# iosefa/obia

Hardware: AMD Instinct MI355X
Metric: Mpixel/s (SLIC+zonal feats) on 16384²×8-band; achieved HBM GB/s fraction (higher is better)
Workload: dtype f32

## Files before the change

### obia_amd/_lib.py

```python
import ctypes
import os
import subprocess

import numpy as np

_CSRC = os.path.join(os.path.dirname(os.path.abspath(__file__)), "csrc")
LIB_PATH = os.environ.get("OBIA_HIP_LIB") or os.path.join(_CSRC, "libobia_hip.so")

OBIA_OK = 0
MASK_SEEDS_CHUNK = 1024
E_INVALID, E_HIP, E_NOMEM, E_UNSUPPORTED, E_EMPTY, E_NONFINITE = -1, -2, -3, -4, -5, -6


class SlicParams(ctypes.Structure):
    _fields_ = [("compactness", ctypes.c_double), ("min_size_factor", ctypes.c_double),
                ("max_size_factor", ctypes.c_double), ("n_segments", ctypes.c_int32),
                ("max_num_iter", ctypes.c_int32), ("convert2lab", ctypes.c_int32),
                ("enforce_connectivity", ctypes.c_int32), ("slic_zero", ctypes.c_int32),
                ("start_label", ctypes.c_int32), ("normalize_bands", ctypes.c_int32),
                ("exit_on_fixed_point", ctypes.c_int32), ("reserved", ctypes.c_int32),
                ("sigma_zyx", ctypes.c_double * 3), ("spacing_zyx", ctypes.c_double * 3)]


class SlicSeeds(ctypes.Structure):
# ... 43 lines not shown
    "obia_slic_f32_dev": (_I, [_P, _P, _I, _I, _I, _P, ctypes.POINTER(SlicParams), _P, ctypes.POINTER(_I)]),
    "obia_slic_assign_only_f32_dev": (_I, [_P, _P, _I, _I, _I, _P, ctypes.POINTER(SlicParams), _P, ctypes.POINTER(_I)]),
    "obia_slic_seeded_f32_dev": (_I, [_P, _P, _I, _I, _I, _P, ctypes.POINTER(SlicParams), ctypes.POINTER(SlicSeeds), _I, _P,
                                      ctypes.POINTER(_I)]),
    "obia_mask_centroids_dev": (_I, [_P, _P, _I, _I, _P, ctypes.c_int32, _P, ctypes.c_int64, _I, _P, _P]),
    "obia_slic_stages_f32_dev": (_I, [_P, _P, _I, _I, _I, _P, ctypes.POINTER(SlicParams), ctypes.POINTER(SlicSeeds),
                                      ctypes.POINTER(SlicStages)]),
    "obia_enforce_connectivity_i32_dev": (_I, [_P, _P, _I, _I, _I, _I, _I, _P, ctypes.POINTER(_I)]),
    "obia_zonal_stats_f32": (_I, [_P, _P, _P, _I, _I, _I, _P, _I, _I, _I, _P, _P, _P, _P, _P]),
    "obia_zonal_stats_f32_dev": (_I, [_P, _P, _P, _I, _I, _I, _P, _I, _I, _I, _P, _P, _P, _P, _P]),
    "obia_zonal_moments_f32_dev": (_I, [_P, _P, _P, _I, _I, _I, _P, _I, _I, _I, _P, _P, _P, _P]),
    "obia_zonal_moments_f32": (_I, [_P, _P, _P, _I, _I, _I, _P, _I, _I, _I, _P, _P, _P]),
    "obia_texture_stats_f32_dev": (_I, [_P, _P, _P, _I, _I, _I, _P, _I, _I, _I, _P]),
    "obia_label_edges_u8_dev": (_I, [_P, _P, _I, _I, _P, _P]),
    "obia_sample_labels_i32_dev": (_I, [_P, _P, _I, _I, _P, _P, ctypes.c_int64, _I, _P]),
    "obia_cost_bands_f32_dev": (_I, [_P, _P, ctypes.c_int64, _P, _P]),
    "obia_cost_ndvi_f32_dev": (_I, [_P, _P, _P, ctypes.c_int64, _P]),
    "obia_cost_sobel_f32_dev": (_I, [_P, _P, _I, _I, _P]),
    "obia_cost_select_dev": (_I, [_P, _P, _I, ctypes.c_int64, ctypes.c_double, ctypes.c_double, _P, _P]),
    "obia_cost_entropy_f32_dev": (_I, [_P, _P, _I, _I, ctypes.c_double, ctypes.c_double, _P, _P]),
    "obia_cost_normalise_dev": (_I, [_P, _P, _I, ctypes.c_int64, ctypes.c_double, ctypes.c_double, _P]),
    "obia_cost_edge_count_dev": (_I, [_P, _P, _I, _I, _P]),
    "obia_cost_combine_dev": (_I, [_P, _P, _P, _P, _P, _I, _I, _P, _P, _P, _P]),
    "obia_seeds_peaks_dev": (_I, [_P, _P, _I, _I, ctypes.c_double, _I, ctypes.c_float, _P, _P, _P, _P]),
    "obia_seeds_peaks_gather_dev": (_I, [_P, _P, _P, _P, _P, _I, _I, ctypes.c_int64, _P, _P, _P, _P]),
    "obia_seeds_pair_link_dev": (_I, [_P, _P, _P, _I, _P, _I, _I, _P, ctypes.c_double, ctypes.c_double, _I, _P, ctypes.c_double, _I, _P,
                                      ctypes.POINTER(_I)]),
    "obia_seeds_pair_stats_dev": (_I, [_P, _P, _P, _I, _P, _I, _I, _P, ctypes.c_double, ctypes.c_double, _I, _P, _P, _P]),
    "obia_seeds_pair_matrix_dev": (_I, [_P, _P, _P, _I, _P, _I, _I, _P, ctypes.c_double, ctypes.c_double, _I, _P, _P]),
    "obia_polygon_count_i32_dev": (_I, [_P, _P, _I, _I, _I, _P, _P]),
    "obia_polygon_rings_i32_dev": (_I, [_P, _P, _I, _I, _I, ctypes.c_int64, ctypes.c_int64, _P, _P, _P, _P, _P, _P]),
    "obia_rasterize_polygons_dev": (_I, [_P, _P, _P, ctypes.c_int64, _P, _P, ctypes.c_int64, _I, _I, ctypes.c_int32, _P]),
    "obia_rasterize_info": (_I, [ctypes.POINTER(ctypes.c_int64)]),
    "obia_quickshift_f32": (_I, [_P, _P, _I, _I, _I, ctypes.c_double, ctypes.c_double, ctypes.c_double, ctypes.c_double, _I, _P, _I, _P, ctypes.POINTER(_I)]),
    "obia_quickshift_f32_dev": (_I, [_P, _P, _I, _I, _I, ctypes.c_double, ctypes.c_double, ctypes.c_double, ctypes.c_double, _I, _P, _I, _P, ctypes.POINTER(_I)]),
    "obia_quickshift_stages_f32_dev": (_I, [_P, _P, _I, _I, _I, ctypes.c_double, ctypes.c_double, ctypes.c_double, ctypes.c_double, _I, _P, _I, _P,
                                            ctypes.POINTER(_I), _P, _P, _P, _P, _P, _P]),
    "obia_tiled_slic_f32_dev": (_I, [_P, _P, _P, _I, _I, _I, ctypes.POINTER(TilingParams), ctypes.POINTER(SlicParams), _P,
                                     ctypes.POINTER(ctypes.c_int64)]),
    "obia_tiled_slic_f32": (_I, [_P, _P, _P, _I, _I, _I, ctypes.POINTER(TilingParams), ctypes.POINTER(SlicParams), _P,
                                 ctypes.POINTER(ctypes.c_int64)]),
    "obia_tiled_slic_seeded_f32_dev": (_I, [_P, _P, _P, _I, _I, _I, ctypes.POINTER(TilingParams), ctypes.POINTER(SlicParams), _I, PickFn, _P,
                                            _P, ctypes.POINTER(ctypes.c_int64)]),
    "obia_tiled_slic_seeded_f32": (_I, [_P, _P, _P, _I, _I, _I, ctypes.POINTER(TilingParams), ctypes.POINTER(SlicParams), _I, PickFn, _P,
                                        _P, ctypes.POINTER(ctypes.c_int64)]),
    "obia_tiler_set_seeding": (_I, [_P, _I, PickFn, _P]),
    "obia_tiler_create": (_P, [_P, _P, _P, _I, _I, _I, _I, _I, ctypes.POINTER(TilingParams), ctypes.POINTER(SlicParams), _P, _I]),
    "obia_tiler_destroy": (None, [_P]),
    "obia_tiler_run": (_I, [_P, _I, _I, _I, _I]),
    "obia_tiler_next_id": (_I, [_P]),
    "obia_tiler_set_segments": (_I, [_P, _I, _I, _P]),
    "obia_tiler_get_alive": (_I, [_P, _P, _I]),
    "obia_tiler_set_alive": (_I, [_P, _P, _I]),
    "obia_tiler_finalize": (_I, [_P, ctypes.POINTER(ctypes.c_int64)]),
    "obia_tiler_import_seam": (_I, [_P, _P, _I, _I, _I, _P, _I, _P, _P, ctypes.POINTER(ctypes.c_int), ctypes.POINTER(ctypes.c_int),
                                    ctypes.POINTER(ctypes.c_int)]),
    "obia_table_scale_dev": (_I, [_P, _P, ctypes.c_int64, _I, _P, _P, _P]),
    "obia_forest_predict_dev": (_I, [_P, _P, ctypes.c_int64, _I, ctypes.POINTER(Forest), _P, _P, _P, _P]),
    "obia_mlp_predict_dev": (_I, [_P, _P, ctypes.c_int64, _I, ctypes.POINTER(Mlp), _P, _P, _P, _P, _P]),
    "obia_table_scale_f64_dev": (_I, [_P, _P, ctypes.c_int64, _I, _P, _P, _P]),
    "obia_forest_shap_dev": (_I, [_P, _P, ctypes.c_int64, _I, ctypes.POINTER(Forest), _P, _P, _P]),
    "obia_mlp_coalition_dev": (_I, [_P, _P, ctypes.c_int64, _I, ctypes.POINTER(Mlp), _P, ctypes.c_int64, _P, ctypes.c_int64, _P]),
    "obia_shapley_combine_dev": (_I, [_P, _P, ctypes.c_int64, _I, _I, _P, _P]),
    "obia_set_profiling": (_I, [_P, _I]),
    "obia_last_timing": (ctypes.c_double, [_P, _I]),
}
EXPORTED_SYMBOLS = tuple(_SIGNATURES)
_IMAGE_SIGNATURES = {
    "obia_image_stretch_u8_dev": (_I, [_P, _P, _I, ctypes.c_int64, ctypes.c_double, ctypes.c_double, _P]),
    "obia_image_gray_hist_dev": (_I, [_P, _P, _I, ctypes.c_int64, _P, _P]),
    "obia_image_lut_u8_dev": (_I, [_P, _P, ctypes.c_int64, _P, _I, _P]),
    "obia_image_clahe_u8_dev": (_I, [_P, _P, _I, _I, _I, _I, _P]),
    "obia_image_boundaries_dev": (_I, [_P, _P, _I, _I, _P]),
    "obia_image_mark_u8_dev": (_I, [_P, _P, _I, _P, _I, _I, _P, _P, _P]),
}
SHARP_MAX_WIN = 65536
_SHARPNESS_SIGNATURES = {
    "obia_sharp_gray_lap_dev": (_I, [_P, _P, _I, _I, _I, ctypes.POINTER(ctypes.c_int32), _P, _P]),
    "obia_sharp_laplacian_dev": (_I, [_P, _P, _I, _I, _P, _P]),
    "obia_sharp_box_dev": (_I, [_P, _P, _I, _I, _I, _P, _P, _P]),
    "obia_sharp_variance_dev": (_I, [_P, _P, _I, _I, _I, _P, _P]),
    "obia_sharp_stretch_f32_dev": (_I, [_P, _P, ctypes.c_int64, ctypes.c_double, ctypes.c_double, _P]),
}

_lib = None


def build(force=False):
    args = ["make", "-C", _CSRC, "-j8"]
    if force:
        args.append("-B")
    subprocess.check_call(args, stdout=subprocess.DEVNULL)
    return LIB_PATH


def load():
    global _lib
    if _lib is None:
        if not os.path.exists(LIB_PATH):
            raise ImportError(f"{LIB_PATH} not found: build it with `python -c 'import __graft_entry__ as g; g.build()'` "
                              "(hipcc, gfx950). obia_amd has no CPU fallback.")
        lib = ctypes.CDLL(LIB_PATH)
        for name, (res, args) in list(_SIGNATURES.items()) + list(_IMAGE_SIGNATURES.items()) + list(_SHARPNESS_SIGNATURES.items()):
            try:
                fn = getattr(lib, name)
            except AttributeError:
                if os.environ.get("OBIA_HIP_LIB"):
                    continue
                raise
            fn.restype = res
            fn.argtypes = args
        _lib = lib
    return _lib


def last_error():
    return load().obia_last_error().decode("utf-8", "replace")


def check(rc):
    if rc == OBIA_OK:
        return
    msg = last_error()
    if rc in (E_INVALID, E_EMPTY, E_NONFINITE):
        raise ValueError(msg)
    if rc == E_UNSUPPORTED:
        raise NotImplementedError(msg)
    if rc == E_NOMEM:
        raise MemoryError(msg)
    raise RuntimeError(f"obia_hip error {rc}: {msg}")


class Context:

    def __init__(self, device=0, stream=None):
        lib = load()
        if stream is None:
            self._h = lib.obia_create(int(device))
        else:
            self._h = lib.obia_create_on_stream(int(device), ctypes.c_void_p(int(stream)))
        if not self._h:
            raise RuntimeError(f"obia_create failed: {last_error()} (obia_amd needs an AMD GPU; there is no CPU path)")
        self.device = int(device)

    @property
    def handle(self):
        return self._h

    def close(self):
        if getattr(self, "_h", None):
            load().obia_destroy(self._h)
            self._h = None

    def __del__(self):
        try:
            self.close()
        except Exception:
            pass

    def set_profiling(self, on):
        check(load().obia_set_profiling(self._h, int(on)))

    def timing(self):
        lib = load()
        names = ["assign_ms", "sweeps", "features_ms", "connectivity_ms", "zonal_ms", "total_ms", "prepass_ms", "assign_px",
                 "prepass_px", "assign_store_px", "assign_busy_ms", "prepass_busy_ms", "batch_repeats",
                 "prepass_shared_px", "feature_fused_px", "prepass_group_launches"]
        return {n: lib.obia_last_timing(self._h, i) for i, n in enumerate(names)}

    def workspace_bytes(self):
        return int(load().obia_workspace_bytes(self._h))


_default_ctx = {}


def default_context(device=0):
    ctx = _default_ctx.get(device)
    if ctx is None:
        ctx = _default_ctx[device] = Context(device)
    return ctx


def np_ptr(a):
    return None if a is None else ctypes.c_void_p(a.ctypes.data)


def mask_bytes(mask, device=None):
    import torch
    m = torch.as_tensor(mask, device=device)
    if m.dtype == torch.bool:
        m = m.contiguous().view(torch.uint8)
    elif m.dtype != torch.uint8:
        m = (m != 0).view(torch.uint8)
    return m.contiguous()
```

### obia_amd/csrc/api.cpp

```cpp
#include "slic.hpp"

#include <cmath>

using namespace obia;

namespace {

int check_slic_args(const float *img, int H, int W, int C, const obia_slic_params *p) {
    if (!img || !p) { set_error("null image or params"); return OBIA_E_INVALID; }
    if (H <= 0 || W <= 0 || C <= 0) { set_error("bad image shape (%d,%d,%d)", H, W, C); return OBIA_E_INVALID; }
    if ((long long)H * W > 0x7fffffffLL) { set_error("rasters above 2^31 pixels must go through the tiled driver"); return OBIA_E_INVALID; }
    if (C > 16) { set_error("more than 16 bands not supported (got %d)", C); return OBIA_E_UNSUPPORTED; }
    if (p->start_label != 0 && p->start_label != 1) { set_error("start_label should be 0 or 1."); return OBIA_E_INVALID; }
    if (p->convert2lab == 1 && C != 3) { set_error("Lab colorspace conversion requires a RGB image."); return OBIA_E_INVALID; }
    if (!(p->compactness > 0.0)) { set_error("compactness must be positive"); return OBIA_E_INVALID; }
    if (p->n_segments <= 0) { set_error("n_segments must be positive"); return OBIA_E_INVALID; }
    if (p->max_num_iter < 0) { set_error("max_num_iter must be >= 0"); return OBIA_E_INVALID; }
    for (int i = 0; i < 3; ++i) {
        if (!(p->sigma_zyx[i] >= 0.0)) { set_error("sigma must be >= 0"); return OBIA_E_INVALID; }
        if (!(p->spacing_zyx[i] > 0.0) || !(p->spacing_zyx[i] < 1.0e30)) { set_error("spacing must be positive and finite"); return OBIA_E_INVALID; }
    }
    return OBIA_OK;
}

int slic_single(obia_ctx *ctx, const float *img, int H, int W, int C, const uint8_t *mask,
                const obia_slic_params *p, SlicBatch &b, const ExternalSeeds *ext = nullptr, bool prepass_only = false,
                int prepass_iters = 0) {
    Arena &A = ctx->arena;
    slic_batch_settings(b, *p, C, p->normalize_bands, mask != nullptr);
    b.prepass_only = prepass_only && b.masked;
    b.prepass_iter = b.masked ? prepass_iters : 0;
    b.windows.assign(1, SrcWindow{0, 0, H, W, 0, 0, 0});
    OBIA_TRY(slic_batch_layout(b));
    b.d_windows = A.get<SrcWindow>(1);
    b.d_feat = A.get<float>(4 * (size_t)b.total_feat_f4);
    b.d_labels = A.get<int32_t>((size_t)b.total_pix);
    if (!b.d_windows || !b.d_feat || !b.d_labels) return OBIA_E_NOMEM;
    OBIA_HIP_TRY(hipMemcpyAsync(b.d_windows, b.windows.data(), sizeof(SrcWindow), hipMemcpyHostToDevice, ctx->stream));
    b.d_mask = const_cast<uint8_t *>(mask);
    if (b.col_lb) {
        b.d_fbox = A.get<float>((size_t)b.total_boxes * 2 * b.CP);
        if (!b.d_fbox) return OBIA_E_NOMEM;
    }
    OBIA_TRY(slic_prepare_features(ctx, b, img, W));
    std::vector<int> nseg(1, p->n_segments);
    OBIA_TRY(slic_plan_and_seed(ctx, b, nseg, nullptr, ext));
    if (b.probs[0].K <= 0) {
        set_error("mask is empty: nothing to segment");
        return OBIA_E_EMPTY;
    }
    const Arena::Mark sweeps_mk = A.mark();
    OBIA_TRY(slic_run_sweeps(ctx, b));
    OBIA_HIP_TRY(hipStreamSynchronize(ctx->stream));
    bool repeat = false;
    OBIA_TRY(slic_sweeps_settle(ctx, &repeat));
    if (repeat) {
        A.rewind(sweeps_mk);
        b.d_mask4 = nullptr;
        OBIA_TRY(slic_rerun_storing(ctx, b));
    }
    return OBIA_OK;
}

}

extern "C" {

static int check_seeds(const obia_slic_seeds *seeds, int H, int W, ExternalSeeds &ext) {
    if (!seeds) { set_error("null seeds"); return OBIA_E_INVALID; }
    if (!seeds->yx || seeds->n < 1) { set_error("seeds: need at least one (y, x) pair"); return OBIA_E_INVALID; }
    for (int i = 0; i < seeds->n; ++i) {
        const double y = seeds->yx[2 * (size_t)i], x = seeds->yx[2 * (size_t)i + 1];
        if (!(y >= 0.0 && y <= (double)(H - 1) && x >= 0.0 && x <= (double)(W - 1))) {
            set_error("seed %d = (%g, %g) lies outside the (%d, %d) raster", i, y, x, H, W);
            return OBIA_E_INVALID;
        }
    }
    double st = seeds->steps_zyx[0];
    if (seeds->steps_zyx[1] > st) st = seeds->steps_zyx[1];
    if (seeds->steps_zyx[2] > st) st = seeds->steps_zyx[2];
    if (!(st > 0.0) || !(st < 1e9)) { set_error("seeds: steps must be positive and finite"); return OBIA_E_INVALID; }
    ext.yx = seeds->yx; ext.n = seeds->n; ext.step = st;
    return OBIA_OK;
}

static int slic_stages_impl(obia_ctx *ctx, const float *img, int H, int W, int C, const uint8_t *mask,
                            const obia_slic_params *params, const ExternalSeeds *ext, obia_slic_stages *st) {
    OBIA_TRY(check_slic_args(img, H, W, C, params));
    if (!st) { set_error("null output"); return OBIA_E_INVALID; }
    if (st->prepass_iters < 0) { set_error("prepass_iters must be >= 0"); return OBIA_E_INVALID; }
    if (st->centroids && params->max_num_iter < 1) { set_error("centroids: no sweep ran (max_num_iter = 0)"); return OBIA_E_INVALID; }
    SlicBatch b;
    OBIA_TRY(call_frame(ctx, FRAME_TOTAL, [&] {
        int rc = slic_single(ctx, img, H, W, C, mask, params, b, ext, st->prepass_only != 0, st->prepass_iters);
        if (rc == OBIA_OK && (st->seeds_yx || st->centroids) && b.probs[0].K > st->centroid_capacity) {
            set_error("%d centroids, room for %d", b.probs[0].K, st->centroid_capacity);
            rc = OBIA_E_INVALID;
        }
        if (rc == OBIA_OK && st->labels_pre) {
            hipError_t e = hipMemcpyAsync(st->labels_pre, b.d_labels, sizeof(int32_t) * (size_t)H * W, hipMemcpyDeviceToDevice, ctx->stream);
            if (e != hipSuccess) { set_error("copy failed: %s", hipGetErrorString(e)); rc = OBIA_E_HIP; }
        }
        if (rc == OBIA_OK && (st->features || st->seeds_yx || st->centroids))
            rc = slic_stage_outputs(ctx, b, st->features, st->seeds_yx, st->centroids);
        return rc;
    }));
    st->K = b.probs[0].K;
    st->step = (double)b.step[0];
    st->prescale = (double)b.prescale;
    st->fscale = b.fscale * (double)b.prescale;
    return OBIA_OK;
}

static int slic_assign_only_impl(obia_ctx *ctx, const float *img, int H, int W, int C, const uint8_t *mask,
                                 const obia_slic_params *params, const ExternalSeeds *ext, int32_t *labels_pre_out,
                                 int *n_centroids_out) {
    if (!labels_pre_out) { set_error("null output"); return OBIA_E_INVALID; }
    obia_slic_stages st{};
    st.labels_pre = labels_pre_out;
    OBIA_TRY(slic_stages_impl(ctx, img, H, W, C, mask, params, ext, &st));
    if (n_centroids_out) *n_centroids_out = st.K;
    return OBIA_OK;
}

static int slic_full_impl(obia_ctx *ctx, const float *img, int H, int W, int C, const uint8_t *mask,
                          const obia_slic_params *params, const ExternalSeeds *ext, int32_t *labels_out, int *n_labels_out) {
    OBIA_TRY(check_slic_args(img, H, W, C, params));
    if (!labels_out) { set_error("null output"); return OBIA_E_INVALID; }
    SlicBatch b;
    int n_labels = 0;
    OBIA_TRY(call_frame(ctx, FRAME_TOTAL, [&]() -> int {
        OBIA_TRY(slic_single(ctx, img, H, W, C, mask, params, b, ext));
        if (params->enforce_connectivity) {
            const auto [min_size, max_size] = slic_cc_sizes(params->min_size_factor, params->max_size_factor, b.probs[0].n_valid, b.probs[0].K);
            return enforce_connectivity_dev(ctx, b.d_labels, H, W, min_size, max_size, params->start_label, labels_out, &n_labels);
        }
        hipError_t e = hipMemcpyAsync(labels_out, b.d_labels, sizeof(int32_t) * (size_t)H * W, hipMemcpyDeviceToDevice, ctx->stream);
        if (e != hipSuccess) { set_error("copy failed: %s", hipGetErrorString(e)); return OBIA_E_HIP; }
        n_labels = b.probs[0].K;
        return OBIA_OK;
    }));
    if (n_labels_out) *n_labels_out = n_labels;
// ... 160 lines not shown
```

### obia_amd/csrc/cc.hip

```cpp
#include "slic.hpp"

#include <cstdlib>

namespace obia {

__device__ __forceinline__ int find_prob(const CcProblem *__restrict__ probs, int nprob, long long g) {
    int lo = 0, hi = nprob - 1;
    while (lo < hi) {
        const int mid = (lo + hi + 1) >> 1;
        if (probs[mid].pix_off <= g) lo = mid; else hi = mid - 1;
    }
    return lo;
}

__device__ __forceinline__ int ld_agent(const int *p) {
    return __hip_atomic_load(p, __ATOMIC_RELAXED, __HIP_MEMORY_SCOPE_AGENT);
}

__device__ __forceinline__ int find_root(const int *parent, int i) {
    int p;
    while ((p = ld_agent(&parent[i])) != i) i = p;
    return i;
}

// ... 642 lines not shown
        n = ccur[s];
        if (o + n > cap) n = cap - o;
    }
    if (n > 0 && n <= SETTLE_COOP) {
        int m = T_NEVER;
        for (int e = 0; e < n; ++e) m = min(m, settle_entry_min(px_cn[o + e], settle));
        int t = T_NEVER;
        if (m != T_NEVER)
            for (int e = 0; e < n; ++e) { const int g = px_g[o + e]; if (g > m && g < t) t = g; }
        if (settle[s] != t) {
            settle[s] = t;
            for (int e = 0; e < n; ++e) push_neighbours(px_cn[o + e]);
        }
    }
    unsigned long long coop = __ballot(n > SETTLE_COOP);
    while (coop) {
        const int src = __builtin_ctzll(coop);
        coop &= coop - 1;
        const int sb = __shfl(s, src), ob = __shfl(o, src), nb = __shfl(n, src);
        int m = T_NEVER;
        for (int e = lane; e < nb; e += 64) m = min(m, settle_entry_min(px_cn[ob + e], settle));
        m = wave_min_i32(m);
        int t = T_NEVER;
        if (m != T_NEVER)
            for (int e = lane; e < nb; e += 64) { const int g = px_g[ob + e]; if (g > m && g < t) t = g; }
        t = wave_min_i32(t);
        const int old = settle[sb];
        if (old != t) {
            if (lane == 0) settle[sb] = t;
            for (int e = lane; e < nb; e += 64) push_neighbours(px_cn[ob + e]);
        }
    }
    int inc = npush;
#pragma unroll
    for (int off = 1; off < 64; off <<= 1) { const int v = __shfl_up(inc, off); if ((int)threadIdx.x >= off) inc += v; }
    const int total = __shfl(inc, 63);
    if (total == 0) return;
    int base_slot = 0;
    if (threadIdx.x == 63) base_slot = atomicAdd(work_cnt, total);
    base_slot = __shfl(base_slot, 63);
    for (int j = 0; j < npush; ++j) work_out[base_slot + inc - npush + j] = s_push[threadIdx.x][j];
}
__global__ __launch_bounds__(64) void cc_small_target_kernel(const CcProblem *__restrict__ probs, int nprob, const int *__restrict__ code,
                                                             const int *__restrict__ newlab, const int *__restrict__ small_list,
                                                             const int *__restrict__ small_qoff, const int *__restrict__ settle,
                                                             int *__restrict__ queue, int32_t *__restrict__ out, int *__restrict__ target, int n_small) {
    const int s = blockIdx.x * blockDim.x + threadIdx.x;
    if (s >= n_small) return;
    const int st = settle[s];
    if (st == T_NEVER) { target[s] = -1; return; }
    const CcProblem P = probs[find_prob(probs, nprob, small_list[s])];
    int *q = queue + small_qoff[s];
    int csize = 0, ms = 0;
    const int adjacent = replay_bfs<true>(code, newlab, settle, -(s + 2), st, P.H, P.W, (int)P.pix_off, q, out, &csize, &ms, nullptr);
    for (int i = 0; i < csize; ++i) out[q[i]] = 0;
    target[s] = adjacent;
}

__global__ void cc_settle_init_kernel(const int *__restrict__ small_list, int n_small, int *__restrict__ settle, int from_above) {
    const int s = blockIdx.x * blockDim.x + threadIdx.x;
    if (s < n_small) settle[s] = from_above ? 0x7fffffff : small_list[s];
}

__global__ void cc_small_final_kernel(const int *__restrict__ parent, const int *__restrict__ newlab, const int *__restrict__ target,
                                      int n_small, int max_hops, int *__restrict__ small_final) {
    const int s = blockIdx.x * blockDim.x + threadIdx.x;
    if (s >= n_small) return;
    int nl = -(s + 2), hops = 0;
    while (nl < 0) {
        const int t = target[-nl - 2];
        if (t < 0 || ++hops > max_hops) { nl = -1; break; }
        nl = newlab[parent[parent[t]]];
    }
    small_final[s] = nl;
}

__global__ __launch_bounds__(256) void cc_relabel_kernel(const CcResolve R, long long n, int32_t *__restrict__ out) {
    for (long long i = (long long)blockIdx.x * blockDim.x + threadIdx.x; i < n; i += (long long)gridDim.x * blockDim.x)
        out[i] = cc_resolve_label(R, i);
}

int enforce_connectivity_batch(obia_ctx *ctx, const std::vector<CcProblem> &probs, const int32_t *labels_in,
                               long long total_pix, int start_label, int32_t *labels_out, int *h_n_labels_out,
                               CcResolve *deferred) {
    ScopedSpan span(ctx, T_CC);
    Arena &A = ctx->arena;
    const long long n = total_pix;
    const int np = (int)probs.size();
    if (np <= 0 || n <= 0 || n > 0x7fffffffLL) { set_error("label batch of %lld pixels not supported", n); return OBIA_E_INVALID; }
    const int mask_label = start_label - 1;
    CcProblem *d_probs = A.get<CcProblem>(np);
    int *parent = A.get<int>(n), *size = A.get<int>(n), *newlab = A.get<int>(n);
    const int nb = cdiv(n, SCAN_CHUNK);
    int *block_sums = A.get<int>(3 * (size_t)nb);
    unsigned long long *rootbits = A.get<unsigned long long>((size_t)((n + 63) / 64));
    if (!rootbits) return OBIA_E_NOMEM;
    unsigned long long *lrbits_block = A.get<unsigned long long>((size_t)((n + 63) / 64) + 4);
    if (!lrbits_block) return OBIA_E_NOMEM;
    unsigned long long *lrbits = lrbits_block + 4;
    const unsigned long long *rb = rootbits;
    int *counters = reinterpret_cast<int *>(lrbits_block);
    if (!d_probs || !parent || !size || !newlab || !block_sums) return OBIA_E_NOMEM;
    OBIA_TRY(upload_async(ctx, d_probs, probs.data(), sizeof(CcProblem) * np));
    OBIA_HIP_TRY(hipMemsetAsync(lrbits_block, 0, sizeof(unsigned long long) * ((size_t)((n + 63) / 64) + 4), ctx->stream));
    int gs = cdiv(n, 256 * 4);
    if (gs > 65535 * 4) gs = 65535 * 4;
    {
        int max_tiles = 1;
        long long max_seam = 1;
        for (auto &P : probs) {
            const int t = cdiv(P.W, CT_W) * cdiv(P.H, CT_H);
            if (t > max_tiles) max_tiles = t;
            const long long sm = (long long)((P.H - 1) / CT_H) * P.W + (long long)((P.W - 1) / CT_W) * P.H;
            if (sm > max_seam) max_seam = sm;
        }
        hipLaunchKernelGGL(cc_tile_kernel, dim3(max_tiles, np), dim3(256), 0, ctx->stream, d_probs, labels_in, parent, size, mask_label, lrbits);
        int sg = cdiv(max_seam, 256);
        if (sg > 65535) sg = 65535;
        hipLaunchKernelGGL(cc_seam_kernel, dim3(sg, np), dim3(256), 0, ctx->stream, d_probs, labels_in, parent, mask_label);
    }
    debug_sync(ctx, "cc: tile + seam");
    hipLaunchKernelGGL(cc_roots_kernel, dim3(cdiv((n + 63) / 64, 64)), dim3(64), 0, ctx->stream, parent, size, n, lrbits, rootbits);
    debug_sync(ctx, "cc: roots");
    hipLaunchKernelGGL(cc_rank_blocksum_bits_kernel, dim3(nb), dim3(64), 0, ctx->stream, d_probs, np, size, n, block_sums, counters, rootbits);
    hipLaunchKernelGGL(cc_rank_scan_kernel, dim3(3), dim3(1024), 0, ctx->stream, block_sums, nb, counters);
    int hc[8];
    OBIA_TRY(read_back(ctx, hc, counters, sizeof(hc)));
    if (hc[6] > 0) {
        const int n_big = hc[6];
        int *big_root = A.get<int>(n_big), *big_qoff = A.get<int>(n_big), *big_box = A.get<int>(4 * (size_t)n_big);
        if (!big_root || !big_qoff || !big_box) return OBIA_E_NOMEM;
        OBIA_HIP_TRY(hipMemsetAsync(counters, 0, sizeof(int) * 8, ctx->stream));
        hipLaunchKernelGGL(cc_flatten_all_kernel, dim3(gs), dim3(256), 0, ctx->stream, parent, n);
        hipLaunchKernelGGL(cc_big_list_kernel, dim3(cdiv(n, 256)), dim3(256), 0, ctx->stream, d_probs, np, parent, size, n, newlab,
                           big_root, big_qoff, big_box, counters);
        int hb[8];
        OBIA_TRY(read_back(ctx, hb, counters, sizeof(hb)));
        int *bqueue = A.get<int>(hb[7] > 0 ? hb[7] : 1);
        if (!bqueue) return OBIA_E_NOMEM;
        hipLaunchKernelGGL(cc_big_mark_kernel, dim3(cdiv(n, 256)), dim3(256), 0, ctx->stream, d_probs, np, parent, size, n, newlab, big_box);
        hipLaunchKernelGGL(cc_split_kernel, dim3(cdiv(n_big, 64)), dim3(64), 0, ctx->stream, d_probs, np, parent, size, big_root, big_qoff,
                           big_box, n_big, bqueue);
        OBIA_HIP_TRY(hipMemsetAsync(counters, 0, sizeof(int) * 8, ctx->stream));
        rb = nullptr;
        hipLaunchKernelGGL(cc_rank_blocksum_kernel, dim3(nb), dim3(SCAN_NT), 0, ctx->stream, d_probs, np, parent, size, n, block_sums, counters, rb);
        hipLaunchKernelGGL(cc_rank_scan_kernel, dim3(3), dim3(1024), 0, ctx->stream, block_sums, nb, counters);
        OBIA_TRY(read_back(ctx, hc, counters, sizeof(hc)));
    }
    const int n_small = hc[0], small_px = hc[1], n_surv = hc[2];
    int *small_list = A.get<int>(n_small > 0 ? n_small : 1);
    int *small_qoff = A.get<int>(n_small > 0 ? n_small : 1);
    int *target = A.get<int>(n_small > 0 ? n_small : 1);
    int *queue = A.get<int>(small_px > 0 ? small_px : 1);
    if (!small_list || !small_qoff || !target || !queue) return OBIA_E_NOMEM;
    debug_sync(ctx, "cc: rank counts");
    if (rb)
        hipLaunchKernelGGL(cc_rank_apply_bits_kernel, dim3(nb), dim3(64), 0, ctx->stream, d_probs, np, size, n, block_sums, newlab,
                           small_list, small_qoff, rb);
    else
        hipLaunchKernelGGL(cc_rank_apply_kernel, dim3(nb), dim3(SCAN_NT), 0, ctx->stream, d_probs, np, parent, size, n, block_sums,
                           newlab, small_list, small_qoff, counters, rb);
    int *settle_arr = nullptr;
    int32_t *visited = nullptr;
    if (n_small > 0) {
        int *settle = settle_arr = A.get<int>(n_small), *work_a = A.get<int>(n_small), *work_b = A.get<int>(n_small), *tag = A.get<int>(n_small);
        static const long long code_div = std::getenv("OBIA_CC_CODE_DIV") ? atoll(std::getenv("OBIA_CC_CODE_DIV")) : 64;
        const bool use_code = (long long)n_small * code_div >= n;
        constexpr int RING = 64;
        int *ring = A.get<int>(RING);
        if (!ring) return OBIA_E_NOMEM;
        OBIA_HIP_TRY(hipMemsetAsync(ring, 0, sizeof(int) * RING, ctx->stream));
        long long ring_pos = 0;
        int *code = use_code ? A.get<int>(n) : parent;
        if (!settle || !work_a || !work_b || !tag || !code) return OBIA_E_NOMEM;
        if ((size_t)n > ctx->cc_visited_px || ctx->cc_visited_dirty) {
            if ((size_t)n > ctx->cc_visited_px) {
                OBIA_HIP_TRY(hipStreamSynchronize(ctx->stream));
                if (ctx->cc_visited) (void)hipFree(ctx->cc_visited);
                ctx->cc_visited = nullptr; ctx->cc_visited_px = 0;
                const size_t want = (size_t)n + (size_t)n / 8;
                if (hipMalloc(&ctx->cc_visited, want * sizeof(int32_t)) != hipSuccess) { (void)hipGetLastError(); set_error("out of device memory (visited map of %zu pixels)", want); return OBIA_E_NOMEM; }
                ctx->cc_visited_px = want;
            }
            OBIA_HIP_TRY(hipMemsetAsync(ctx->cc_visited, 0, sizeof(int32_t) * ctx->cc_visited_px, ctx->stream));
        }
        ctx->cc_visited_dirty = true;
        visited = ctx->cc_visited;
        if (use_code) hipLaunchKernelGGL(cc_code_kernel, dim3(gs), dim3(256), 0, ctx->stream, parent, newlab, n, code);
        constexpr int ROUNDS_FROM_BELOW = 5;
        bool converged = false;
        const bool dense = use_code && start_label == 1 && !std::getenv("OBIA_CC_WORKLIST");
        if (dense) {
            int *px_g = A.get<int>(small_px), *ccur = A.get<int>(n_small);
            int4 *px_cn = A.get<int4>(small_px);
            if (!px_g || !ccur || !px_cn) return OBIA_E_NOMEM;
            int maxh = 1;
            for (auto &P : probs) maxh = std::max(maxh, P.H);
            OBIA_HIP_TRY(hipMemsetAsync(ccur, 0, sizeof(int) * (size_t)n_small, ctx->stream));
            hipLaunchKernelGGL(cc_small_pixels_kernel, dim3(maxh, np), dim3(256), 0, ctx->stream, d_probs, code, small_qoff, ccur, px_g, px_cn, small_px);
            for (int side = (n_small > 8 * (long long)n_surv ? 1 : 0); side < 2 && !converged; ++side) {
                OBIA_HIP_TRY(hipMemsetAsync(tag, 0, sizeof(int) * (size_t)n_small, ctx->stream));
                hipLaunchKernelGGL(cc_settle_init_kernel, dim3(cdiv(n_small, 256)), dim3(256), 0, ctx->stream, small_list, n_small, settle, side);
                int n_items = n_small;
                const int *work_in = nullptr;
                const long long max_rounds = side == 0 ? ROUNDS_FROM_BELOW : (long long)small_px + 2;
                for (long long round = 0; round <= max_rounds; ++round) {
                    if (std::getenv("OBIA_DEBUG_CC")) fprintf(stderr, "[obia cc]   (lists) side %d round %lld: %d items\n", side, round, n_items);
                    int *cnt = ring + (ring_pos++ % RING);
                    if (ring_pos > RING && (ring_pos - 1) % RING == 0) OBIA_HIP_TRY(hipMemsetAsync(ring, 0, sizeof(int) * RING, ctx->stream));
                    hipLaunchKernelGGL(cc_settle_eval_kernel, dim3(cdiv(n_items, 64)), dim3(64), 0, ctx->stream, small_qoff, ccur, px_g, px_cn, small_px,
                                       settle, work_in, n_items, work_a, cnt, tag, (int)(round & 0x3fffffff));
                    int n_next = 0;
                    OBIA_TRY(read_back(ctx, &n_next, cnt, sizeof(int)));
                    if (n_next == 0) { converged = true; break; }
                    work_in = work_a;
                    std::swap(work_a, work_b);
                    n_items = n_next;
                }
            }
            if (converged)
                hipLaunchKernelGGL(cc_small_target_kernel, dim3(cdiv(n_small, 64)), dim3(64), 0, ctx->stream, d_probs, np, code, newlab, small_list,
                                   small_qoff, settle, queue, visited, target, n_small);
        }
        for (int side = (n_small > 8 * (long long)n_surv ? 1 : 0); !dense && side < 2 && !converged; ++side) {
            OBIA_HIP_TRY(hipMemsetAsync(tag, 0, sizeof(int) * (size_t)n_small, ctx->stream));
            hipLaunchKernelGGL(cc_settle_init_kernel, dim3(cdiv(n_small, 256)), dim3(256), 0, ctx->stream, small_list, n_small, settle, side);
            int n_items = n_small;
            const int *work_in = nullptr;
            const long long max_rounds = side == 0 ? ROUNDS_FROM_BELOW : (long long)small_px + 2;
            for (long long round = 0; round <= max_rounds; ++round) {
                if (std::getenv("OBIA_DEBUG_CC")) fprintf(stderr, "[obia cc]   side %d round %lld: %d items\n", side, round, n_items);
                int *cnt = ring + (ring_pos++ % RING);
                if (ring_pos > RING && (ring_pos - 1) % RING == 0) OBIA_HIP_TRY(hipMemsetAsync(ring, 0, sizeof(int) * RING, ctx->stream));
                if (use_code)
                    hipLaunchKernelGGL(HIP_KERNEL_NAME(cc_small_bfs_kernel<true>), dim3(cdiv(n_items, 64)), dim3(64), 0, ctx->stream, d_probs, np, code,
                                       newlab, small_list, small_qoff, start_label, settle, queue, visited, target, work_in, n_items, work_a,
                                       cnt, tag, (int)(round & 0x3fffffff));
                else
                    hipLaunchKernelGGL(HIP_KERNEL_NAME(cc_small_bfs_kernel<false>), dim3(cdiv(n_items, 64)), dim3(64), 0, ctx->stream, d_probs, np, code,
                                       newlab, small_list, small_qoff, start_label, settle, queue, visited, target, work_in, n_items, work_a,
                                       cnt, tag, (int)(round & 0x3fffffff));
                int n_next = 0;
                OBIA_TRY(read_back(ctx, &n_next, cnt, sizeof(int)));
                if (n_next == 0) { converged = true; break; }
                work_in = work_a;
                std::swap(work_a, work_b);
                n_items = n_next;
            }
        }
        if (!converged) { set_error("connectivity enforcement: settle rounds did not converge (%d small components)", n_small); return OBIA_E_INVALID; }
        ctx->cc_visited_dirty = false;
    }
    if (std::getenv("OBIA_DEBUG_CC"))
        fprintf(stderr, "[obia cc] %lld px, %d problems: %d surviving, %d small components (%d px)\n", n, np, n_surv, n_small, small_px);
    debug_sync(ctx, "cc: rank apply + small components");
    if (n_small > 0)
        hipLaunchKernelGGL(cc_small_final_kernel, dim3(cdiv(n_small, 256)), dim3(256), 0, ctx->stream, parent, newlab, target, n_small, n_small + 1, settle_arr);
    const CcResolve R{parent, newlab, settle_arr, start_label, mask_label};
    if (deferred) *deferred = R;
    else hipLaunchKernelGGL(cc_relabel_kernel, dim3(gs), dim3(256), 0, ctx->stream, R, n, labels_out);
    OBIA_HIP_TRY(hipGetLastError());
    if (h_n_labels_out) *h_n_labels_out = n_surv;
    return OBIA_OK;
}

int enforce_connectivity_dev(obia_ctx *ctx, const int32_t *labels_in, int H, int W, int min_size, int max_size,
                             int start_label, int32_t *labels_out, int *h_n_labels_out) {
    std::vector<CcProblem> probs(1, CcProblem{H, W, 0, min_size, max_size > 0 ? max_size : 1});
    return enforce_connectivity_batch(ctx, probs, labels_in, (long long)H * W, start_label, labels_out, h_n_labels_out);
}

}
```

### obia_amd/csrc/common.hpp

```cpp
#pragma once
#include <hip/hip_runtime.h>
#include <algorithm>
#include <cstdint>
#include <cstdio>
#include <cstring>
#include <string>
#include <vector>

#include "../../include/obia_hip.h"

namespace obia {

void set_error(const char *fmt, ...);

#define OBIA_HIP_TRY(expr)                                                                       \
    do {                                                                                         \
        hipError_t e__ = (expr);                                                                 \
        if (e__ != hipSuccess) {                                                                 \
            obia::set_error("%s:%d: %s -> %s", __FILE__, __LINE__, #expr, hipGetErrorString(e__)); \
            return OBIA_E_HIP;                                                                   \
        }                                                                                        \
    } while (0)

#define OBIA_TRY(expr)            \
    do {                          \
        int rc__ = (expr);        \
        if (rc__ != OBIA_OK) return rc__; \
    } while (0)

class Arena {
  public:
    ~Arena() { release(); }
    void *alloc(size_t bytes);
    template <typename T> T *get(size_t n) { return static_cast<T *>(alloc(n * sizeof(T))); }
    void reset();
    void release();
    struct Mark { size_t block, used, total; };
    Mark mark() const;
    void rewind(const Mark &m);
    size_t capacity() const;
    bool failed() const { return failed_; }

  private:
    struct Block { char *p; size_t size; size_t used; };
    std::vector<Block> blocks_;
    size_t high_water_ = 0, cur_total_ = 0, cur_ = 0;
    bool failed_ = false;
};

struct Timing {
    double assign_ms = 0, prepass_ms = 0, feat_ms = 0, cc_ms = 0, zonal_ms = 0, total_ms = 0;
    double assign_px = 0, prepass_px = 0;
    double prepass_shared_px = 0;
    double assign_store_px = 0;
    double feat_fused_px = 0;
    int sweeps = 0;
    int prepass_group_launches = 0;
    int batch_repeats = 0;
    double assign_busy_ms = 0, prepass_busy_ms = 0;
};

}

struct obia_ctx {
    int device = 0;
    hipStream_t stream = nullptr;
    bool own_stream = false;
    obia::Arena arena;
    void *pinned = nullptr;
    size_t pinned_bytes = 0;
    unsigned long long *defer_buf = nullptr;
    bool defer_pending = false;
    double defer_shared_px = 0;
    int32_t *cc_visited = nullptr;
    size_t cc_visited_px = 0;
    bool cc_visited_dirty = false;
    char *up_buf = nullptr;
    size_t up_bytes = 0, up_used = 0;
    int profiling = 0;
    obia::Timing timing;
    struct Span { int kind; hipEvent_t a, b; };
    std::vector<Span> spans;
    std::vector<hipEvent_t> event_pool;
    size_t events_used = 0;
    hipStream_t side = nullptr;
    hipEvent_t aux_fork = nullptr, aux_join = nullptr;
    hipEvent_t grp_fork = nullptr, grp_join = nullptr;
    int spatial_residency[4] = {0, 0, 0, 0};
};

namespace obia {

enum TimeKind { T_ASSIGN = 0, T_FEAT = 2, T_CC = 3, T_ZONAL = 4, T_TOTAL = 5, T_PREPASS = 6 };

struct ScopedSpan {
    obia_ctx *ctx; bool on; size_t idx;
    ScopedSpan(obia_ctx *c, int kind);
    ~ScopedSpan();
};
struct KernelSpan {
    hipEvent_t a = nullptr, b = nullptr;
    KernelSpan(obia_ctx *c, int kind);
};
void begin_timing(obia_ctx *ctx);
void resolve_timing(obia_ctx *ctx);

int read_back(obia_ctx *ctx, void *host_dst, const void *dev_src, size_t bytes);
int upload_async(obia_ctx *ctx, void *dev_dst, const void *host_src, size_t bytes);
int side_stream(obia_ctx *ctx);
void debug_sync(obia_ctx *ctx, const char *stage);

static inline int cdiv(long long a, long long b) { return (int)((a + b - 1) / b); }
static inline unsigned flat_grid(long long n) { return (unsigned)std::max<long long>(1, std::min<long long>(cdiv(n, 256), 8192)); }


int enter(obia_ctx *ctx);

int quiesce(obia_ctx *ctx, int rc);

enum FrameOpts : unsigned { FRAME_PLAIN = 0, FRAME_TIMING = 1, FRAME_TOTAL = 2 | FRAME_TIMING };
void frame_begin(obia_ctx *ctx, unsigned opts);
int frame_end(obia_ctx *ctx, unsigned opts, int rc);
template <typename Body> int call_frame(obia_ctx *ctx, unsigned opts, Body &&body) {
    frame_begin(ctx, opts);
    int rc;
    if ((opts & FRAME_TOTAL) == FRAME_TOTAL) {
        ScopedSpan total(ctx, T_TOTAL);
        rc = body();
    } else {
        rc = body();
    }
    return frame_end(ctx, opts, rc);
}

class Staging {
  public:
    explicit Staging(obia_ctx *ctx) : ctx_(ctx) {}
    ~Staging() { (void)finish(); }
    Staging(const Staging &) = delete;
    Staging &operator=(const Staging &) = delete;
    template <typename T> T *in(const T *host, size_t n) { return static_cast<T *>(upload(host, n * sizeof(T))); }
    template <typename T> T *out(size_t n) { return static_cast<T *>(alloc(n * sizeof(T))); }
    template <typename T> void fetch(T *host, const T *dev, size_t n) { download(host, dev, n * sizeof(T)); }
    bool ok() const { return rc_ == OBIA_OK; }
    template <typename Call> void run(Call &&call) { if (ok()) rc_ = call(); }
    int finish();
  private:
    void *alloc(size_t bytes);
    void *upload(const void *host, size_t bytes);
    void download(void *host, const void *dev, size_t bytes);
    obia_ctx *ctx_;
    int rc_ = OBIA_OK;
    bool open_ = true;
    std::vector<void *> bufs_;
};

#if defined(__HIPCC__)
typedef float obia_v4f __attribute__((ext_vector_type(4)));
__device__ __forceinline__ float4 ld_stream_f4(const void *p) {
    const obia_v4f t = __builtin_nontemporal_load(reinterpret_cast<const obia_v4f *>(p));
    return make_float4(t.x, t.y, t.z, t.w);
}
#endif

}
```

### obia_amd/csrc/context.cpp

```cpp
#include "common.hpp"

#include <algorithm>
#include <cstdlib>
#include <utility>

#include <cstdarg>

namespace obia {

static thread_local std::string g_last_error;

void set_error(const char *fmt, ...) {
    char buf[1024];
    va_list ap;
    va_start(ap, fmt);
    vsnprintf(buf, sizeof(buf), fmt, ap);
    va_end(ap);
    g_last_error = buf;
}

void *Arena::alloc(size_t bytes) {
    bytes = (bytes + 255) & ~size_t(255);
    if (bytes == 0) bytes = 256;
    for (; cur_ < blocks_.size(); ++cur_) {
        Block &b = blocks_[cur_];
        if (b.size - b.used >= bytes) {
            void *p = b.p + b.used;
            b.used += bytes;
            cur_total_ += bytes;
            if (cur_total_ > high_water_) high_water_ = cur_total_;
            return p;
        }
    }
    size_t want = bytes;
    size_t grow = blocks_.empty() ? (size_t(64) << 20) : 2 * blocks_.back().size;
    if (grow > (size_t(4) << 30)) grow = size_t(4) << 30;
    if (want < grow) want = grow;
    void *p = nullptr;
    if (hipMalloc(&p, want) != hipSuccess) {
        if (want == bytes || hipMalloc(&p, bytes) != hipSuccess) {
            failed_ = true;
            set_error("workspace hipMalloc of %zu bytes failed", bytes);
            return nullptr;
        }
        want = bytes;
    }
    blocks_.push_back(Block{static_cast<char *>(p), want, bytes});
    cur_ = blocks_.size() - 1;
    cur_total_ += bytes;
    if (cur_total_ > high_water_) high_water_ = cur_total_;
    return p;
}

Arena::Mark Arena::mark() const {
    Mark m;
    m.block = cur_ < blocks_.size() ? cur_ : blocks_.size();
    m.used = m.block < blocks_.size() ? blocks_[m.block].used : 0;
    m.total = cur_total_;
    return m;
}

void Arena::rewind(const Mark &m) {
    for (size_t i = m.block + 1; i < blocks_.size(); ++i) blocks_[i].used = 0;
    if (m.block < blocks_.size()) blocks_[m.block].used = m.used;
    cur_ = m.block;
    cur_total_ = m.total;
}

void Arena::reset() {
    failed_ = false;
    cur_total_ = 0;
    cur_ = 0;
    if (blocks_.size() > 1) {
        size_t total = 0;
        for (auto &b : blocks_) total += b.size;
        for (auto &b : blocks_) (void)hipFree(b.p);
        blocks_.clear();
        void *p = nullptr;
        if (hipMalloc(&p, high_water_ + (high_water_ >> 3)) == hipSuccess) blocks_.push_back(Block{static_cast<char *>(p), high_water_ + (high_water_ >> 3), 0});
        (void)total;
    } else if (!blocks_.empty()) {
        blocks_[0].used = 0;
    }
// ... 17 lines not shown
        ctx->event_pool.push_back(e);
    }
    return ctx->event_pool[ctx->events_used++];
}

ScopedSpan::ScopedSpan(obia_ctx *c, int kind) : ctx(c), on(c->profiling == 1 || (c->profiling == 2 && kind == T_ASSIGN)), idx(0) {
    if (!on) return;
    obia_ctx::Span s{kind, get_event(ctx), get_event(ctx)};
    (void)hipEventRecord(s.a, ctx->stream);
    idx = ctx->spans.size();
    ctx->spans.push_back(s);
}
ScopedSpan::~ScopedSpan() {
    if (on) (void)hipEventRecord(ctx->spans[idx].b, ctx->stream);
}

int side_stream(obia_ctx *ctx) {
    if (!ctx->aux_fork) OBIA_HIP_TRY(hipEventCreateWithFlags(&ctx->aux_fork, hipEventDisableTiming));
    if (!ctx->aux_join) OBIA_HIP_TRY(hipEventCreateWithFlags(&ctx->aux_join, hipEventDisableTiming));
    if (!ctx->grp_fork) OBIA_HIP_TRY(hipEventCreateWithFlags(&ctx->grp_fork, hipEventDisableTiming));
    if (!ctx->grp_join) OBIA_HIP_TRY(hipEventCreateWithFlags(&ctx->grp_join, hipEventDisableTiming));
    if (!ctx->side) OBIA_HIP_TRY(hipStreamCreateWithFlags(&ctx->side, hipStreamNonBlocking));
    return OBIA_OK;
}

KernelSpan::KernelSpan(obia_ctx *c, int kind) {
    if (!(c->profiling == 1 || (c->profiling == 2 && kind == T_ASSIGN))) return;
    a = get_event(c);
    b = get_event(c);
    c->spans.push_back(obia_ctx::Span{kind, a, b});
}

void begin_timing(obia_ctx *ctx) {
    ctx->spans.clear();
    ctx->events_used = 0;
    ctx->timing = Timing();
}

void resolve_timing(obia_ctx *ctx) {
    if (!ctx->profiling) return;
    (void)hipStreamSynchronize(ctx->stream);
    std::vector<std::pair<double, double>> iv[2];
    hipEvent_t ref = nullptr;
    for (auto &s : ctx->spans) {
        float ms = 0;
        if (hipEventElapsedTime(&ms, s.a, s.b) != hipSuccess) { (void)hipGetLastError(); continue; }
        if (s.kind == T_ASSIGN || s.kind == T_PREPASS) {
            if (!ref) ref = s.a;
            float end = 0;
            if (hipEventElapsedTime(&end, ref, s.b) == hipSuccess) iv[s.kind == T_ASSIGN ? 0 : 1].emplace_back((double)end - ms, (double)end);
            else (void)hipGetLastError();
        }
        switch (s.kind) {
            case T_ASSIGN: ctx->timing.assign_ms += ms; ctx->timing.sweeps += 1; break;
            case T_FEAT: ctx->timing.feat_ms += ms; break;
            case T_CC: ctx->timing.cc_ms += ms; break;
            case T_ZONAL: ctx->timing.zonal_ms += ms; break;
            case T_TOTAL: ctx->timing.total_ms += ms; break;
            case T_PREPASS: ctx->timing.prepass_ms += ms; break;
            default: break;
        }
    }
    for (int c = 0; c < 2; ++c) {
        std::sort(iv[c].begin(), iv[c].end());
        double busy = 0, lo = 0, hi = -1;
        for (auto &x : iv[c]) {
            if (hi < lo || x.first > hi) { if (hi > lo) busy += hi - lo; lo = x.first; hi = x.second; }
            else if (x.second > hi) hi = x.second;
        }
        if (hi > lo) busy += hi - lo;
        (c == 0 ? ctx->timing.assign_busy_ms : ctx->timing.prepass_busy_ms) += busy;
    }
    ctx->spans.clear();
}

int read_back(obia_ctx *ctx, void *host_dst, const void *dev_src, size_t bytes) {
    if (bytes > ctx->pinned_bytes) {
        if (ctx->pinned) (void)hipHostFree(ctx->pinned);
        ctx->pinned = nullptr;
        size_t want = bytes < 4096 ? 4096 : bytes;
        OBIA_HIP_TRY(hipHostMalloc(&ctx->pinned, want, hipHostMallocDefault));
        ctx->pinned_bytes = want;
    }
    OBIA_HIP_TRY(hipMemcpyAsync(ctx->pinned, dev_src, bytes, hipMemcpyDeviceToHost, ctx->stream));
    OBIA_HIP_TRY(hipStreamSynchronize(ctx->stream));
    ctx->up_used = 0;
    memcpy(host_dst, ctx->pinned, bytes);
    return OBIA_OK;
}

void debug_sync(obia_ctx *ctx, const char *stage) {
    static const bool on = std::getenv("OBIA_DEBUG_SYNC") != nullptr;
    if (!on) return;
    const hipError_t e = hipStreamSynchronize(ctx->stream);
    fprintf(stderr, "[obia debug] %s: %s\n", stage, e == hipSuccess ? "ok" : hipGetErrorString(e));
    fflush(stderr);
}

int upload_async(obia_ctx *ctx, void *dev_dst, const void *host_src, size_t bytes) {
    if (bytes == 0) return OBIA_OK;
    constexpr size_t RING = 8u << 20;
    if (!ctx->up_buf) {
        void *p = nullptr;
        OBIA_HIP_TRY(hipHostMalloc(&p, RING, hipHostMallocDefault));
        ctx->up_buf = static_cast<char *>(p);
        ctx->up_bytes = RING;
        ctx->up_used = 0;
    }
    if (bytes > ctx->up_bytes) {
        OBIA_HIP_TRY(hipMemcpyAsync(dev_dst, host_src, bytes, hipMemcpyHostToDevice, ctx->stream));
        OBIA_HIP_TRY(hipStreamSynchronize(ctx->stream));
        ctx->up_used = 0;
        return OBIA_OK;
    }
    if (ctx->up_used + bytes > ctx->up_bytes) {
        OBIA_HIP_TRY(hipStreamSynchronize(ctx->stream));
        ctx->up_used = 0;
    }
    char *slot = ctx->up_buf + ctx->up_used;
    memcpy(slot, host_src, bytes);
    OBIA_HIP_TRY(hipMemcpyAsync(dev_dst, slot, bytes, hipMemcpyHostToDevice, ctx->stream));
    ctx->up_used += (bytes + 63) & ~(size_t)63;
    return OBIA_OK;
}

int enter(obia_ctx *ctx) {
    if (!ctx) { set_error("null context"); return OBIA_E_INVALID; }
    if (hipSetDevice(ctx->device) != hipSuccess) { set_error("hipSetDevice(%d) failed", ctx->device); return OBIA_E_HIP; }
    return OBIA_OK;
}

int quiesce(obia_ctx *ctx, int rc) {
    (void)hipStreamSynchronize(ctx->stream);
    if (ctx->side) (void)hipStreamSynchronize(ctx->side);
    return rc;
}

void frame_begin(obia_ctx *ctx, unsigned opts) {
    ctx->arena.reset();
    if (opts & FRAME_TIMING) begin_timing(ctx);
}

int frame_end(obia_ctx *ctx, unsigned opts, int rc) {
    if (rc != OBIA_OK) return quiesce(ctx, rc);
    OBIA_HIP_TRY(hipStreamSynchronize(ctx->stream));
    if (opts & FRAME_TIMING) resolve_timing(ctx);
    return OBIA_OK;
}

void *Staging::alloc(size_t bytes) {
    if (!ok()) return nullptr;
    void *p = nullptr;
    if (hipMalloc(&p, bytes) != hipSuccess) {
        set_error("device allocation for host-pointer call failed");
        rc_ = OBIA_E_NOMEM;
        return nullptr;
    }
    bufs_.push_back(p);
    return p;
}

void *Staging::upload(const void *host, size_t bytes) {
    if (!host) return nullptr;
    void *p = alloc(bytes);
    if (p && hipMemcpyAsync(p, host, bytes, hipMemcpyHostToDevice, ctx_->stream) != hipSuccess) {
        set_error("host->device copy failed in a host-pointer call");
        rc_ = OBIA_E_HIP;
    }
    return p;
}

void Staging::download(void *host, const void *dev, size_t bytes) {
    if (ok() && hipMemcpyAsync(host, dev, bytes, hipMemcpyDeviceToHost, ctx_->stream) != hipSuccess) {
        set_error("device->host copy failed in a host-pointer call");
        rc_ = OBIA_E_HIP;
    }
}

int Staging::finish() {
    if (open_) {
        open_ = false;
        (void)hipStreamSynchronize(ctx_->stream);
        for (void *p : bufs_) (void)hipFree(p);
        bufs_.clear();
    }
    return rc_;
}

}

using namespace obia;

extern "C" {

int obia_abi_version(void) { return OBIA_ABI_VERSION; }

const char *obia_last_error(void) { return g_last_error.c_str(); }

static obia_ctx *create_impl(int device_id, void *stream, bool own) {
    int n = 0;
    if (hipGetDeviceCount(&n) != hipSuccess || n <= 0) {
        set_error("no HIP device available");
        return nullptr;
    }
    if (device_id < 0 || device_id >= n) {
        set_error("device_id %d out of range (%d devices)", device_id, n);
        return nullptr;
    }
    if (hipSetDevice(device_id) != hipSuccess) {
        set_error("hipSetDevice(%d) failed", device_id);
        return nullptr;
    }
    obia_ctx *ctx = new obia_ctx();
    ctx->device = device_id;
    if (own) {
        if (hipStreamCreateWithFlags(&ctx->stream, hipStreamNonBlocking) != hipSuccess) {
            set_error("hipStreamCreate failed");
            delete ctx;
            return nullptr;
        }
        ctx->own_stream = true;
    } else {
        ctx->stream = static_cast<hipStream_t>(stream);
    }
    return ctx;
}

obia_ctx *obia_create(int device_id) { return create_impl(device_id, nullptr, true); }
obia_ctx *obia_create_on_stream(int device_id, void *hip_stream) { return create_impl(device_id, hip_stream, false); }

void obia_destroy(obia_ctx *ctx) {
    if (!ctx) return;
    (void)hipSetDevice(ctx->device);
    (void)hipStreamSynchronize(ctx->stream);
    ctx->arena.release();
    if (ctx->up_buf) (void)hipHostFree(ctx->up_buf);
    if (ctx->pinned) (void)hipHostFree(ctx->pinned);
    if (ctx->defer_buf) (void)hipHostFree(ctx->defer_buf);
    if (ctx->cc_visited) (void)hipFree(ctx->cc_visited);
    for (auto e : ctx->event_pool) (void)hipEventDestroy(e);
    if (ctx->side) (void)hipStreamDestroy(ctx->side);
    if (ctx->aux_fork) (void)hipEventDestroy(ctx->aux_fork);
    if (ctx->aux_join) (void)hipEventDestroy(ctx->aux_join);
    if (ctx->grp_fork) (void)hipEventDestroy(ctx->grp_fork);
    if (ctx->grp_join) (void)hipEventDestroy(ctx->grp_join);
    if (ctx->own_stream) (void)hipStreamDestroy(ctx->stream);
    delete ctx;
}

int obia_synchronize(obia_ctx *ctx) {
    if (!ctx) { set_error("null context"); return OBIA_E_INVALID; }
    OBIA_HIP_TRY(hipStreamSynchronize(ctx->stream));
    return OBIA_OK;
}

int64_t obia_workspace_bytes(obia_ctx *ctx) { return ctx ? (int64_t)ctx->arena.capacity() : 0; }

void obia_slic_default_params(obia_slic_params *p) {
    if (!p) return;
    p->n_segments = 100;
    p->compactness = 10.0;
    p->max_num_iter = 10;
    p->convert2lab = -1;
    p->enforce_connectivity = 1;
    p->min_size_factor = 0.5;
    p->max_size_factor = 3.0;
    p->slic_zero = 0;
    p->start_label = 1;
    p->normalize_bands = 0;
    p->exit_on_fixed_point = 0;
    p->reserved = 0;
    p->sigma_zyx[0] = p->sigma_zyx[1] = p->sigma_zyx[2] = 0.0;
    p->spacing_zyx[0] = p->spacing_zyx[1] = p->spacing_zyx[2] = 1.0;
}

int obia_set_profiling(obia_ctx *ctx, int enabled) {
    if (!ctx) { set_error("null context"); return OBIA_E_INVALID; }
    ctx->profiling = enabled < 0 ? 0 : (enabled > 2 ? 1 : enabled);
    return OBIA_OK;
}

double obia_last_timing(obia_ctx *ctx, int what) {
    if (!ctx) return -1.0;
    switch (what) {
        case 0: return ctx->timing.assign_ms;
        case 1: return (double)ctx->timing.sweeps;
        case 2: return ctx->timing.feat_ms;
        case 3: return ctx->timing.cc_ms;
        case 4: return ctx->timing.zonal_ms;
        case 5: return ctx->timing.total_ms;
        case 6: return ctx->timing.prepass_ms;
        case 7: return ctx->timing.assign_px;
        case 8: return ctx->timing.prepass_px;
        case 9: return ctx->timing.assign_store_px;
        case 10: return ctx->timing.assign_busy_ms;
        case 11: return ctx->timing.prepass_busy_ms;
        case 12: return (double)ctx->timing.batch_repeats;
        case 13: return ctx->timing.prepass_shared_px;
        case 14: return ctx->timing.feat_fused_px;
        case 15: return (double)ctx->timing.prepass_group_launches;
        default: return -1.0;
    }
}

}
```

### obia_amd/csrc/slic.hip

```cpp
#include "slic.hpp"
#include "slic_features.hpp"

#include <cmath>
#include <cstdlib>

namespace obia {

void regular_grid_hw(long long H, long long W, long long n, long long out[4]) {
    long long dims[3] = {1, H, W};
    int order[3] = {0, 1, 2};
    for (int i = 0; i < 3; ++i)
        for (int j = i + 1; j < 3; ++j)
            if (dims[order[j]] < dims[order[i]]) std::swap(order[i], order[j]);
    double sd[3];
    for (int i = 0; i < 3; ++i) sd[i] = (double)dims[order[i]];
    double space = sd[0] * sd[1] * sd[2];
    if (space <= (double)n) { out[0] = out[1] = out[2] = out[3] = 0; return; }
    double st[3];
    for (int i = 0; i < 3; ++i) st[i] = std::pow(space / (double)n, 1.0 / 3.0);
    auto all_ge = [&]() { return sd[0] >= st[0] && sd[1] >= st[1] && sd[2] >= st[2]; };
    if (!all_ge()) {
        for (int d = 0; d < 3; ++d) {
            st[d] = sd[d];
            double sp = 1.0;
// ... 612 lines not shown
            bal[u] = __ballot(keep[u]);
            if (lane == 0) s_wave[it & 1][u][wv] = __popcll(bal[u]);
        }
        __syncthreads();
        int run = base;
#pragma unroll
        for (int u = 0; u < U; ++u) {
            int before = 0, total = 0;
#pragma unroll
            for (int w = 0; w < 4; ++w) { const int c = s_wave[it & 1][u][w]; total += c; if (w < wv) before += c; }
            if (keep[u]) {
                const int rank = run + before + __popcll(bal[u] & ((1ull << lane) - 1ull));
                seed[2 * (size_t)(g.cent_off + rank)] = (float)y[u];
                seed[2 * (size_t)(g.cent_off + rank) + 1] = (float)x[u];
                cent_prob[g.cent_off + rank] = p;
            }
            run += total;
        }
        base = run;
    }
    __syncthreads();
    int K = base;
    if (K == 0 && g.slots > 0) {
        const long long npix = (long long)P.H * P.W;
        unsigned long long best = ~0ull;
        for (long long i = tid; i < npix; i += 256)
            if (mask[P.pix_off + i]) { best = (unsigned long long)i; break; }
        atomicMin(&s_first, best);
        __syncthreads();
        if (tid == 0 && s_first != ~0ull) {
            seed[2 * (size_t)g.cent_off] = (float)(s_first / P.W);
            seed[2 * (size_t)g.cent_off + 1] = (float)(s_first % P.W);
            cent_prob[g.cent_off] = p;
        }
        K = (s_first != ~0ull) ? 1 : 0;
    }
    if (tid == 0) K_out[p] = K;
}

__global__ __launch_bounds__(256) void count_valid_kernel(const SlicProblem *__restrict__ probs,
                                                          const uint8_t *__restrict__ mask, int *__restrict__ out) {
    const int p = blockIdx.y;
    const SlicProblem P = probs[p];
    const long long npix = (long long)P.H * P.W;
    const uint8_t *m = mask + P.pix_off;
    int c = 0;
    const long long head = ((16 - (reinterpret_cast<uintptr_t>(m) & 15)) & 15);
    const long long h0 = head < npix ? head : npix;
    const long long nvec = (npix - h0) / 16;
    const uint4 *mv = reinterpret_cast<const uint4 *>(m + h0);
    auto popnz = [](const uint4 &t) {
        int n = 0;
        const unsigned wds[4] = {t.x, t.y, t.z, t.w};
#pragma unroll
        for (int q = 0; q < 4; ++q) {
            unsigned nz = wds[q] | (wds[q] >> 4);
            nz |= nz >> 2; nz |= nz >> 1;
            n += __popc(nz & 0x01010101u);
        }
        return n;
    };
    const long long stride = (long long)gridDim.x * blockDim.x;
    long long i = (long long)blockIdx.x * blockDim.x + threadIdx.x;
    for (; i + 3 * stride < nvec; i += 4 * stride) {
        const uint4 t0 = mv[i], t1 = mv[i + stride], t2 = mv[i + 2 * stride], t3 = mv[i + 3 * stride];
        c += popnz(t0) + popnz(t1) + popnz(t2) + popnz(t3);
    }
    for (; i < nvec; i += stride) c += popnz(mv[i]);
    if (blockIdx.x == 0) {
        for (long long j = threadIdx.x; j < h0; j += blockDim.x) c += m[j] != 0;
        for (long long j = h0 + nvec * 16 + threadIdx.x; j < npix; j += blockDim.x) c += m[j] != 0;
    }
    __shared__ int s_c[4];
#pragma unroll
    for (int off = 32; off > 0; off >>= 1) c += __shfl_xor(c, off);
    if ((threadIdx.x & 63) == 0) s_c[threadIdx.x >> 6] = c;
    __syncthreads();
    if (threadIdx.x == 0) {
        const int tot = s_c[0] + s_c[1] + s_c[2] + s_c[3];
        if (tot) atomicAdd(&out[p], tot);
    }
}

int slic_count_valid(obia_ctx *ctx, SlicBatch &b, std::vector<int> &nvalid) {
    const int np = b.nprob;
    Arena &A = ctx->arena;
    nvalid.assign(np, 0);
    if (!b.d_probs) b.d_probs = A.get<SlicProblem>(np);
    if (!b.d_probs) return OBIA_E_NOMEM;
    if (b.masked) {
        OBIA_TRY(upload_async(ctx, b.d_probs, b.probs.data(), sizeof(SlicProblem) * np));
        int *d_cnt = A.get<int>(np);
        if (!d_cnt) return OBIA_E_NOMEM;
        OBIA_HIP_TRY(hipMemsetAsync(d_cnt, 0, sizeof(int) * np, ctx->stream));
        int blocks = cdiv(b.maxpix, 256 * 16 * 32);
        if (blocks < 1) blocks = 1;
        hipLaunchKernelGGL(count_valid_kernel, dim3(blocks, np), dim3(256), 0, ctx->stream, b.d_probs, b.d_mask, d_cnt);
        OBIA_TRY(read_back(ctx, nvalid.data(), d_cnt, sizeof(int) * np));
    } else {
        for (int p = 0; p < np; ++p) nvalid[p] = b.probs[p].H * b.probs[p].W;
    }
    return OBIA_OK;
}

int slic_plan_and_seed(obia_ctx *ctx, SlicBatch &b, const std::vector<int> &n_segments, const std::vector<int> *nvalid_in,
                       const ExternalSeeds *ext) {
    const int np = b.nprob;
    if (ext)
        for (int p = 0; p < np; ++p)
            if (ext[p].n < 0 || (ext[p].n > 0 && !ext[p].yx && !ext[p].d_yx)) { set_error("external seeds of problem %d: bad set", p); return OBIA_E_INVALID; }
    Arena &A = ctx->arena;
    if (!b.d_probs) b.d_probs = A.get<SlicProblem>(np);
    if (!b.d_probs) return OBIA_E_NOMEM;
    std::vector<int> nvalid;
    if (nvalid_in) nvalid = *nvalid_in;
    else OBIA_TRY(slic_count_valid(ctx, b, nvalid));
    if (ext && np == 1 && ext->n > 0 && nvalid[0] <= 0) { set_error("the mask has no valid pixel"); return OBIA_E_EMPTY; }
    std::vector<SeedGrid> grids(np);
    std::vector<double> stepmax(np);
    b.step.assign(np, 1.0f);
    b.grid_n.assign(np, 0);
    int cent_off = 0;
    for (int p = 0; p < np; ++p) {
        SlicProblem &P = b.probs[p];
        P.n_valid = nvalid[p];
        SeedGrid &g = grids[p];
        g.cent_off = cent_off; g.slots = 0;
        if (ext && ext[p].n > 0 && nvalid[p] > 0) {
            if ((long long)cent_off + ext[p].n > 0x7fff0000LL) { set_error("too many centroids in one batch"); return OBIA_E_INVALID; }
            g.start_y = g.start_x = 0; g.step_y = g.step_x = 1; g.ny = 1; g.nx = ext[p].n;
            stepmax[p] = ext[p].step < 1.0 ? 1.0 : ext[p].step;
            P.cent_off = cent_off;
            cent_off += ext[p].n;
            continue;
        }
        if (ext || nvalid[p] <= 0 || n_segments[p] <= 0) {
            g.start_y = g.start_x = 0; g.step_y = g.step_x = 1; g.ny = g.nx = 0;
            stepmax[p] = 1.0;
            P.cent_off = cent_off;
            continue;
        }
        long long n_eff = n_segments[p];
        if (b.masked) {
            double ne = std::nearbyint((double)n_segments[p] * ((double)P.H * (double)P.W) / (double)nvalid[p]);
            n_eff = ne < 1.0 ? 1 : (long long)ne;
        }
        b.grid_n[p] = n_eff;
        long long gr[4];
        regular_grid_hw(P.H, P.W, n_eff, gr);
        g.start_y = (int)gr[0]; g.step_y = gr[1] ? (int)gr[1] : 1; g.ny = (int)slice_len(P.H, gr[0], gr[1]);
        g.start_x = (int)gr[2]; g.step_x = gr[3] ? (int)gr[3] : 1; g.nx = (int)slice_len(P.W, gr[2], gr[3]);
        double sy = gr[1] ? (double)gr[1] : 1.0, sx = gr[3] ? (double)gr[3] : 1.0;
        stepmax[p] = sy > sx ? sy : sx;
        if (stepmax[p] < 1.0) stepmax[p] = 1.0;
        P.cent_off = cent_off;
        long long Kg = (long long)g.ny * g.nx;
        if (Kg < 1) Kg = 1;
        if (cent_off + Kg > 0x7fff0000LL) { set_error("too many centroids in one batch"); return OBIA_E_INVALID; }
        g.slots = (int)Kg;
        cent_off += (int)Kg;
    }
    b.total_cent = cent_off > 0 ? cent_off : 1;
    b.d_seed = A.get<float>((size_t)b.total_cent * 2);
    b.d_cent_prob = A.get<int>(b.total_cent);
    SeedGrid *d_grids = A.get<SeedGrid>(np);
    if (!b.d_seed || !b.d_cent_prob || !d_grids) return OBIA_E_NOMEM;
    OBIA_HIP_TRY(hipMemsetAsync(b.d_cent_prob, 0xff, sizeof(int) * b.total_cent, ctx->stream));
    OBIA_TRY(upload_async(ctx, d_grids, grids.data(), sizeof(SeedGrid) * np));
    std::vector<int> K(np);
    if (ext) {
        std::vector<int> hp((size_t)b.total_cent, 0);
        std::vector<float> hs;
        for (int p = 0; p < np; ++p) {
            K[p] = grids[p].ny * grids[p].nx;
            if (K[p] <= 0) continue;
            float *dst = b.d_seed + 2 * (size_t)grids[p].cent_off;
            for (int k = 0; k < K[p]; ++k) hp[(size_t)grids[p].cent_off + k] = p;
            if (ext[p].d_yx) {
                OBIA_HIP_TRY(hipMemcpyAsync(dst, ext[p].d_yx, sizeof(float) * 2 * (size_t)K[p], hipMemcpyDeviceToDevice, ctx->stream));
            } else {
                hs.resize((size_t)K[p] * 2);
                for (size_t i = 0; i < hs.size(); ++i) hs[i] = (float)ext[p].yx[i];
                OBIA_TRY(upload_async(ctx, dst, hs.data(), sizeof(float) * hs.size()));
            }
        }
        OBIA_TRY(upload_async(ctx, b.d_cent_prob, hp.data(), sizeof(int) * hp.size()));
    } else if (b.masked) {
        int *d_K = A.get<int>(np);
        if (!d_K) return OBIA_E_NOMEM;
        hipLaunchKernelGGL(seed_masked_kernel, dim3(np), dim3(256), 0, ctx->stream, d_grids, b.d_probs, b.d_mask,
                           b.d_seed, b.d_cent_prob, d_K);
        OBIA_TRY(read_back(ctx, K.data(), d_K, sizeof(int) * np));
        for (int p = 0; p < np; ++p) if (nvalid[p] <= 0 || n_segments[p] <= 0) K[p] = 0;
    } else {
        int maxK = 1;
        for (int p = 0; p < np; ++p) { K[p] = grids[p].ny * grids[p].nx; if (K[p] > maxK) maxK = K[p]; }
        hipLaunchKernelGGL(seed_grid_kernel, dim3(cdiv(maxK, 256), np), dim3(256), 0, ctx->stream, d_grids, np,
                           b.d_seed, b.d_cent_prob);
    }
    int cell_off = 0, tile_max = 0;
    long long tiles_all = 0;
    for (int p = 0; p < np; ++p) {
        SlicProblem &P = b.probs[p];
        P.K = K[p];
        long long gr[4] = {0, 0, 0, 0};
        if (P.K > 0) regular_grid_hw(P.H, P.W, P.K, gr);
        P.sy = gr[1] ? (int)gr[1] : 1;
        P.sx = gr[3] ? (int)gr[3] : 1;
        P.ncy = cdiv(P.H, P.sy);
        P.ncx = cdiv(P.W, P.sx);
        const float stepf = (float)stepmax[p];
        b.step[p] = stepf;
        P.spatial_w = (float)(1.0 / ((double)stepf * (double)stepf)) * (b.prescale * b.prescale);
        P.sp_y = (float)b.spacing[1]; P.sp_x = (float)b.spacing[2];
        P.direct = b.direct ? 1 : 0;
        P.cell_off = cell_off;
        long long nc = (long long)P.ncy * P.ncx;
        if (cell_off + nc > 0x7fff0000LL) { set_error("too many bins in one batch"); return OBIA_E_INVALID; }
        cell_off += (int)nc;
        P.tiles_x = cdiv(P.W, SWEEP_TW);
        P.tiles_y = cdiv(P.H, SWEEP_TH);
        const int nt = P.tiles_x * P.tiles_y;
        P.tile_off = (int)tiles_all;
        tiles_all += nt;
        if (nt > tile_max) tile_max = nt;
    }
    b.total_tiles_all = tiles_all > 0 ? tiles_all : 1;
    {
        std::vector<int> tp((size_t)b.total_tiles_all, 0);
        for (int p = 0; p < np; ++p)
            for (int t = 0; t < b.probs[p].tiles_x * b.probs[p].tiles_y; ++t) tp[(size_t)b.probs[p].tile_off + t] = p;
        b.d_tile_prob = A.get<int>(tp.size());
        if (!b.d_tile_prob) return OBIA_E_NOMEM;
        OBIA_TRY(upload_async(ctx, b.d_tile_prob, tp.data(), sizeof(int) * tp.size()));
    }
    b.total_cells = cell_off > 0 ? cell_off : 1;
    b.total_tiles = tile_max;
    OBIA_TRY(upload_async(ctx, b.d_probs, b.probs.data(), sizeof(SlicProblem) * np));
    const int RS = CENT_REC + b.CP;
    b.d_cent = A.get<float>((size_t)b.total_cent * RS);
    b.d_head = A.get<int>((size_t)b.total_cells * 2);
    const size_t acc_q = (size_t)b.total_cent * acc_record_qwords(b.CP);
    b.d_acc = A.get<unsigned long long>(acc_q);
    if (!b.d_cent || !b.d_head || !b.d_acc) return OBIA_E_NOMEM;
    OBIA_HIP_TRY(hipMemsetAsync(b.d_acc, 0, sizeof(unsigned long long) * acc_q, ctx->stream));
    return OBIA_OK;
}

__global__ __launch_bounds__(256) void stage_features_kernel(const float *__restrict__ feat, SlicProblem P, int C, int CP, float inv_prescale,
                                                             float *__restrict__ out) {
    const long long n = (long long)P.H * P.W * C;
    for (long long i = (long long)blockIdx.x * blockDim.x + threadIdx.x; i < n; i += (long long)gridDim.x * blockDim.x) {
        const int c = (int)(i % C);
        const long long pix = i / C;
        const int y = (int)(pix / P.W), x = (int)(pix % P.W);
        const long long f4 = P.feat_off + (((long long)(y >> 2) * P.XB + (x >> 4)) * CP + c) * 16 + (x & 15);
        out[i] = feat[4 * f4 + (y & 3)] * inv_prescale;
    }
}

__global__ void stage_centroids_kernel(const float *__restrict__ cent, int cent_off, int K, int C, int CP, float inv_prescale,
                                       float *__restrict__ out) {
    const long long i = (long long)blockIdx.x * blockDim.x + threadIdx.x;
    if (i >= (long long)K * (2 + C)) return;
    const int k = (int)(i / (2 + C)), f = (int)(i % (2 + C));
    const float *rec = cent + (size_t)(cent_off + k) * (CENT_REC + CP);
    out[i] = f < 2 ? rec[f] : rec[CENT_REC + f - 2] * inv_prescale;
}

int slic_stage_outputs(obia_ctx *ctx, const SlicBatch &b, float *features, float *seeds_yx, float *centroids) {
    if (b.nprob != 1 || !b.feat_planes) { set_error("stage outputs: one raster in the plane layout"); return OBIA_E_INVALID; }
    const SlicProblem &P = b.probs[0];
    const float inv_prescale = 1.0f / b.prescale;
    if (features) {
        const long long n = (long long)P.H * P.W * b.C;
        long long blocks = (n + 255) / 256;
        if (blocks > 65535) blocks = 65535;
        hipLaunchKernelGGL(stage_features_kernel, dim3((unsigned)blocks), dim3(256), 0, ctx->stream, b.d_feat, P, b.C, b.CP, inv_prescale, features);
    }
    if (seeds_yx && P.K > 0)
        OBIA_HIP_TRY(hipMemcpyAsync(seeds_yx, b.d_seed + 2 * (size_t)P.cent_off, sizeof(float) * 2 * (size_t)P.K, hipMemcpyDeviceToDevice, ctx->stream));
    if (centroids && P.K > 0)
        hipLaunchKernelGGL(stage_centroids_kernel, dim3(cdiv((long long)P.K * (2 + b.C), 256)), dim3(256), 0, ctx->stream, b.d_cent, P.cent_off,
                           P.K, b.C, b.CP, inv_prescale, centroids);
    OBIA_HIP_TRY(hipGetLastError());
    return OBIA_OK;
}

}
```

### obia_amd/csrc/slic.hpp

```cpp
#pragma once
#include "common.hpp"

namespace obia {

struct SlicProblem {
    int H, W;
    int K;
    int sy, sx;
    int ncy, ncx;
    float spatial_w;
    int cent_off;
    int cell_off;
    int tile_off;
    int tiles_x, tiles_y;
    long long pix_off;
    long long feat_off;
    int XB;
    int n_valid;
    long long fb_off;
    float sp_y, sp_x;
    int direct;
    int m4_off;
};

// ... 51 lines not shown
    double sigma[3] = {0.0, 0.0, 0.0};
    double spacing[3] = {1.0, 1.0, 1.0};
    long long total_feat_f4 = 0;
    uint8_t *d_mask = nullptr;
    unsigned *d_mask4 = nullptr;
    long long total_m4 = 0;
    int32_t *d_labels = nullptr;
    float *d_seed = nullptr;
    int *d_cent_prob = nullptr;
    int *d_tile_prob = nullptr;
    float *d_cent = nullptr;
    int *d_head = nullptr;
    int *d_head_cur = nullptr;
    unsigned long long *d_acc = nullptr;
    int *d_tl_k = nullptr;
    unsigned *d_tl_fp = nullptr;
    int *d_tl_meta = nullptr;
    int *d_tl_req = nullptr;
    float *d_ref = nullptr;
    double fscale = 1.0;
    float prescale = 1.0f;
    bool exit_on_fixed_point = false;
    bool slic_zero = false;
    bool prepass_only = false;
    int prepass_iter = 0;
    std::vector<float> step;
    std::vector<long long> grid_n;
};

inline int slic_prepass_classes(const std::vector<SlicProblem> &probs, const std::vector<long long> &grid_n, std::vector<int> &rep) {
    const int np = (int)probs.size();
    rep.resize(np);
    std::vector<int> reps;
    int members = 0;
    for (int p = 0; p < np; ++p) {
        const SlicProblem &P = probs[p];
        rep[p] = p;
        if ((int)grid_n.size() != np || grid_n[p] <= 0 || P.K <= 0 || P.direct) continue;
        if ((long long)P.n_valid != (long long)P.H * (long long)P.W) continue;
        bool found = false;
        for (int r : reps) {
            const SlicProblem &R = probs[r];
            if (R.H == P.H && R.W == P.W && R.K == P.K && grid_n[r] == grid_n[p] && R.sy == P.sy && R.sx == P.sx && R.ncy == P.ncy &&
                R.ncx == P.ncx && R.tiles_x == P.tiles_x && R.tiles_y == P.tiles_y && R.spatial_w == P.spatial_w && R.sp_y == P.sp_y &&
                R.sp_x == P.sp_x) {
                rep[p] = r; ++members; found = true;
                break;
            }
        }
        if (!found) reps.push_back(p);
    }
    return members;
}

struct SmoothSpec {
    double sigma[3] = {0.0, 0.0, 0.0};
    float *tmp_a = nullptr, *tmp_b = nullptr;
    double *d_w[3] = {nullptr, nullptr, nullptr};
    int radius[3] = {0, 0, 0};
    unsigned *d_scratch = nullptr;
    bool on() const { return sigma[0] > 1e-15 || sigma[1] > 1e-15 || sigma[2] > 1e-15; }
};
int smooth_prepare(obia_ctx *ctx, SmoothSpec &sm, long long total_pix, int CP, int np);
int gaussian_weights_host(double sigma, bool sigma_is_f32, std::vector<double> &w);
int slic_features_launch(hipStream_t stream, const SlicBatch &b, const float *src, int Ws, unsigned *d_keys, const SmoothSpec *smooth = nullptr,
                         bool minmax_only = false);
bool slic_fuse_features(const SlicBatch &b, const float *src, int Ws);
double slic_fscale(float maxabs);
int slic_features_finish(SlicBatch &b, const unsigned *keys, const unsigned *nonfinite, const unsigned *maxabs_bits, std::vector<int> *skip);
int slic_prepare_features(obia_ctx *ctx, SlicBatch &b, const float *src, int Ws, std::vector<int> *skip = nullptr);
float slic_prescale(float ratio, int normalize, int to_lab, bool slic_zero);
bool slic_use_colour_bound(float ratio, bool to_lab = false);
void slic_batch_settings(SlicBatch &b, const obia_slic_params &p, int C, int normalize_bands, bool masked);
int slic_batch_layout(SlicBatch &b);
inline std::pair<int, int> slic_cc_sizes(double min_size_factor, double max_size_factor, int n_valid, int K) {
    const double segment_size = K > 0 ? (double)n_valid / (double)K : 1.0;
    const double mxd = max_size_factor * segment_size;
    return {(int)(min_size_factor * segment_size), mxd >= 2147483647.0 ? 2147483647 : (mxd >= 1.0 ? (int)mxd : 1)};
}

struct ExternalSeeds { const double *yx; int n; double step; const float *d_yx = nullptr; };
int slic_plan_and_seed(obia_ctx *ctx, SlicBatch &b, const std::vector<int> &n_segments,
                       const std::vector<int> *nvalid = nullptr, const ExternalSeeds *ext = nullptr);
int slic_count_valid(obia_ctx *ctx, SlicBatch &b, std::vector<int> &nvalid);

int slic_run_sweeps(obia_ctx *ctx, SlicBatch &b);
int slic_sweeps_settle(obia_ctx *ctx, bool *repeat);
int slic_rerun_storing(obia_ctx *ctx, SlicBatch &b);

int slic_stage_outputs(obia_ctx *ctx, const SlicBatch &b, float *features, float *seeds_yx, float *centroids);

int mask_centroids_dev(obia_ctx *ctx, const uint8_t *mask, int H, int W, const int64_t *picks, int K, const int64_t *dense, long long n_dense,
                       int iters, double *centroids_yx_out, double *steps_zyx_out);
int mask_centroids_queue(obia_ctx *ctx, const uint8_t *mask, int h, int w, long long n_valid, const int64_t *picks, int K, const int64_t *dense,
                         long long n_dense, int iters, float *seeds_out_dev, double *steps_out_dev);

struct CcProblem { int H, W; long long pix_off; int min_size; int max_size; };
struct CcResolve { const int *parent; const int *newlab; const int *small_final; int start_label; int mask_label; };
#if defined(__HIPCC__)
__device__ __forceinline__ int cc_resolve_label(const CcResolve &R, long long i) {
    const int p = R.parent[i];
    if (p < 0) return R.mask_label;
    const int r = R.parent[p];
    int nl = R.newlab[r];
    if (nl < 0) nl = R.small_final[-nl - 2];
    return (nl >= 0) ? nl + R.start_label : 0;
}
#endif
int enforce_connectivity_batch(obia_ctx *ctx, const std::vector<CcProblem> &probs, const int32_t *labels_in,
                               long long total_pix, int start_label, int32_t *labels_out, int *h_n_labels_out,
                               CcResolve *deferred = nullptr);

int enforce_connectivity_dev(obia_ctx *ctx, const int32_t *labels_in, int H, int W, int min_size,
                             int max_size, int start_label, int32_t *labels_out, int *d_n_labels_out);

int zonal_stats_dev(obia_ctx *ctx, const float *raw, const int32_t *labels, int H, int W, int C,
                    const int32_t *bands_host, int n_bands, int n_labels, int start_label,
                    int64_t *count, double *mean, double *var, float *mn, float *mx);
int zonal_moments_dev(obia_ctx *ctx, const float *raw, const int32_t *labels, int H, int W, int C,
                      const int32_t *bands_host, int n_bands, int n_labels, int start_label, const double *mean,
                      double *skew, double *kurt, double *var );

}
```

### obia_amd/csrc/slic_sweep.hip

```cpp
#include "slic.hpp"
#include "slic_features.hpp"

#include <type_traits>
#include <hip/hip_ext.h>

#include <cstdlib>

namespace obia {

#ifdef OBIA_STAMP
__device__ unsigned long long g_tl[65536 * 4 * 24];
#define STAMP_DECL unsigned long long st_t = clock64(), st_t0 = st_t, st_r0 = __builtin_amdgcn_s_memrealtime(), st_acc[12] = {0, 0, 0, 0, 0, 0, 0, 0, 0, 0, 0, 0}, st_cnt[6] = {0, 0, 0, 0, 0, 0};
#define STAMP_COUNT(i, v) st_cnt[i] += (v);
#define STAMP(i) { const unsigned long long st_n = clock64(); st_acc[i] += st_n - st_t; st_t = st_n; }
#ifndef OBIA_STAMP_KIND
#define OBIA_STAMP_KIND 0
#endif
#define STAMP_FLUSH if (accumulate && (LEAN ? 1 : 0) == OBIA_STAMP_KIND && (threadIdx.x & 63) == 0 && gtile < 65536) { unsigned long long *st_o = g_tl + ((size_t)gtile * 4 + (threadIdx.x >> 6)) * 24; for (int st_i = 0; st_i < 12; ++st_i) st_o[st_i] = st_acc[st_i]; st_o[12] = st_t0; st_o[13] = clock64(); st_o[14] = st_r0; st_o[15] = __builtin_amdgcn_s_memrealtime(); for (int st_i = 0; st_i < 6; ++st_i) st_o[16 + st_i] = st_cnt[st_i]; }
#else
#define STAMP_DECL
#define STAMP(i)
#define STAMP_COUNT(i, v)
#define STAMP_FLUSH
#endif
// ... 1247 lines not shown
                for (int j = 0; j < 4; ++j) {
                    const int y = 4 * q + j;
                    if (y < P.H) w |= (unsigned)(mb[(long long)y * W + x] != 0) << (8 * j);
                }
                out[(long long)q * W + x] = w;
            }
        }
    }
}

__global__ void fill_i32_kernel(int32_t *p, long long n, int32_t v) {
    for (long long i = (long long)blockIdx.x * blockDim.x + threadIdx.x; i < n; i += (long long)gridDim.x * blockDim.x) p[i] = v;
}

static void fill_labels(obia_ctx *ctx, SlicBatch &b) {
    const long long n = b.total_pix;
    int blocks = cdiv(n, 256 * 8);
    if (blocks > 65535) blocks = 65535;
    if (blocks < 1) blocks = 1;
    hipLaunchKernelGGL(fill_i32_kernel, dim3(blocks), dim3(256), 0, ctx->stream, b.d_labels, n, b.start_label - 1);
}

static void fold_counters(obia_ctx *ctx, const unsigned long long *h, double shared_px) {
    if (ctx->profiling) {
        for (int i = 0; i < 256; ++i) { ctx->timing.assign_px += (double)h[i]; ctx->timing.prepass_px += (double)h[256 + i]; }
        ctx->timing.prepass_px += shared_px;
        ctx->timing.prepass_shared_px += shared_px;
    }
}

static int spatial_residency(obia_ctx *ctx, int CP) {
    int &r = ctx->spatial_residency[CP / 4 - 1];
    if (r > 0) return r;
    int per_cu = 0, cus = 0;
    hipError_t e = hipErrorInvalidValue;
    switch (CP) {
        case 8: e = hipOccupancyMaxActiveBlocksPerMultiprocessor(&per_cu, slic_spatial_kernel<8>, NT, 0); break;
#ifndef OBIA_ONLY_CP8
        case 4: e = hipOccupancyMaxActiveBlocksPerMultiprocessor(&per_cu, slic_spatial_kernel<4>, NT, 0); break;
        case 12: e = hipOccupancyMaxActiveBlocksPerMultiprocessor(&per_cu, slic_spatial_kernel<12>, NT, 0); break;
        case 16: e = hipOccupancyMaxActiveBlocksPerMultiprocessor(&per_cu, slic_spatial_kernel<16>, NT, 0); break;
#endif
        default: break;
    }
    if (e == hipSuccess) e = hipDeviceGetAttribute(&cus, hipDeviceAttributeMultiprocessorCount, ctx->device);
    if (e != hipSuccess || per_cu <= 0 || cus <= 0) { (void)hipGetLastError(); return 0x7fffffff; }
    r = per_cu * cus;
    return r;
}

static int queue_sweeps(obia_ctx *ctx, SlicBatch &b, bool repeat, unsigned long long **d_px_out, double *shared_px_out) {
    *d_px_out = nullptr;
    *shared_px_out = 0.0;
    if (std::getenv("OBIA_DEBUG_SYNC"))
        for (size_t p = 0; p < b.probs.size(); ++p) {
            const SlicProblem &P = b.probs[p];
            fprintf(stderr, "[obia debug]   problem %zu: %dx%d K %d steps %d %d bins %dx%d cell_off %d cent_off %d tiles %dx%d tile_off %d n_valid %d (total_cent %d total_cells %d tiles_all %lld)\n",
                    p, P.H, P.W, P.K, P.sy, P.sx, P.ncy, P.ncx, P.cell_off, P.cent_off, P.tiles_y, P.tiles_x, P.tile_off, P.n_valid,
                    b.total_cent, b.total_cells, b.total_tiles_all);
        }
    if (b.total_tiles <= 0 || b.max_iter <= 0) { fill_labels(ctx, b); return OBIA_OK; }
    for (auto &P : b.probs)
        if (P.W >= (1 << 22)) { set_error("rasters / tile windows wider than 4194303 pixels are not supported (got %d)", P.W); return OBIA_E_UNSUPPORTED; }
    const int passes = (b.masked && !b.prepass_only) ? 2 : 1;
    if (b.fuse_features && (!b.masked || b.exit_on_fixed_point || b.slic_zero || b.direct || b.col_lb || b.C != b.CP || b.CP > 12 || !b.raw_src || !b.d_keys)) {
        set_error("fused feature pass on a batch that cannot take it");
        return OBIA_E_INVALID;
    }
    const int pre_iter = (b.masked && b.prepass_iter > 0) ? b.prepass_iter : b.max_iter;
    const int total_sweeps = b.masked ? pre_iter + (passes - 1) * b.max_iter : b.max_iter;
    const int RQ = acc_record_qwords(b.CP);
    Arena &A = ctx->arena;
    unsigned long long *d_px = A.get<unsigned long long>(513);
    if (!d_px) return OBIA_E_NOMEM;
    int *d_orphan = reinterpret_cast<int *>(d_px + 512);
    FixedPointState fp;
    if (b.exit_on_fixed_point) {
        const size_t nt = (size_t)b.total_tiles_all;
        fp.bin_stamp = A.get<int>((size_t)b.total_cells);
        fp.tile_lp = A.get<int>(nt);
        fp.cache_k = A.get<int>(nt * (MAXC + 1));
        fp.cache_q = A.get<unsigned long long>(nt * MAXC * (size_t)(b.CP + 3));
        if (!fp.bin_stamp || !fp.tile_lp || !fp.cache_k || !fp.cache_q) return OBIA_E_NOMEM;
        OBIA_HIP_TRY(hipMemsetAsync(fp.bin_stamp, 0, sizeof(int) * (size_t)b.total_cells, ctx->stream));
        OBIA_HIP_TRY(hipMemsetAsync(fp.tile_lp, 0, sizeof(int) * nt, ctx->stream));
    }
    {
        const size_t nt = (size_t)b.total_tiles_all;
        b.d_tl_k = A.get<int>(nt * MAXC);
        b.d_tl_fp = A.get<unsigned>(nt * NT);
        b.d_tl_meta = A.get<int>(nt * 3);
        b.d_tl_req = b.d_tl_meta ? b.d_tl_meta + nt * 2 : nullptr;
        b.d_ref = A.get<float>((size_t)b.total_cent * 2);
        if (!b.d_tl_k || !b.d_tl_fp || !b.d_tl_meta || !b.d_tl_req || !b.d_ref) return OBIA_E_NOMEM;
    }
    int maxh_z = 1, kmax = 1;
    for (auto &P : b.probs) { if (P.H > maxh_z) maxh_z = P.H; if (P.K > kmax) kmax = P.K; }
    if (b.masked && b.d_mask && !b.d_mask4) {
        b.d_mask4 = A.get<unsigned>((size_t)b.total_m4);
        if (!b.d_mask4) return OBIA_E_NOMEM;
        int gq = (maxh_z + 3) / 4;
        if (gq > 16384) gq = 16384;
        hipLaunchKernelGGL(mask_pack4_kernel, dim3(gq, b.nprob), dim3(256), 0, ctx->stream, b.d_probs, b.d_mask, b.d_mask4);
    }
    if (maxh_z > 4096) maxh_z = 4096;

    const bool store_all = repeat || b.exit_on_fixed_point || b.slic_zero;
    if (store_all || total_sweeps <= 1) {
        fill_labels(ctx, b);
        debug_sync(ctx, "sweeps: label fill");
    }
    if (repeat) OBIA_HIP_TRY(hipMemsetAsync(b.d_acc, 0, sizeof(unsigned long long) * (size_t)b.total_cent * RQ, ctx->stream));
    const bool prep_grouped = std::getenv("OBIA_PREP_GROUPED") != nullptr;
    const bool prepass_visits = std::getenv("OBIA_PREPASS_VISITS") != nullptr;
    std::vector<int> share_rep;
    int n_shared = 0;
    {
        const char *e = std::getenv("OBIA_PREPASS_SHARE");
        const bool off = e && e[0] == '0';
        if (!off && b.masked && passes == 2 && pre_iter >= 2 && b.prepass_iter <= 0 && !store_all && !b.direct && !prep_grouped)
            n_shared = slic_prepass_classes(b.probs, b.grid_n, share_rep);
    }
    TileSubset act_tiles;
    const int *d_act_probs = nullptr;
    const int *d_member_rep = nullptr;
    int act_p_base = 0, n_act = b.nprob, kmax_act = kmax, kmax_mem = 1;
    if (n_shared > 0) {
        std::vector<int> ap, at, mr;
        double spx = 0.0;
        kmax_act = 1;
        for (int p = 0; p < b.nprob; ++p) {
            const SlicProblem &P = b.probs[p];
            if (share_rep[p] == p) {
                ap.push_back(p);
                for (int t = 0; t < P.tiles_x * P.tiles_y; ++t) at.push_back(P.tile_off + t);
                if (P.K > kmax_act) kmax_act = P.K;
            } else {
                mr.push_back(p); mr.push_back(share_rep[p]);
                if (P.K > kmax_mem) kmax_mem = P.K;
                spx += (double)P.H * (double)P.W * (double)(pre_iter - 1);
            }
        }
        n_act = (int)ap.size();
        act_p_base = ap.front();
        const bool span = ap.back() - ap.front() + 1 == n_act;
        int *d_mr = A.get<int>(mr.size());
        if (!d_mr) return OBIA_E_NOMEM;
        OBIA_TRY(upload_async(ctx, d_mr, mr.data(), sizeof(int) * mr.size()));
        d_member_rep = d_mr;
        if (span) {
            act_tiles.base = b.probs[ap.front()].tile_off;
            act_tiles.end = b.probs[ap.back()].tile_off + b.probs[ap.back()].tiles_x * b.probs[ap.back()].tiles_y;
        } else {
            int *d_ap = A.get<int>(ap.size()), *d_at = A.get<int>(at.size() ? at.size() : 1);
            if (!d_ap || !d_at) return OBIA_E_NOMEM;
            OBIA_TRY(upload_async(ctx, d_ap, ap.data(), sizeof(int) * ap.size()));
            if (!at.empty()) OBIA_TRY(upload_async(ctx, d_at, at.data(), sizeof(int) * at.size()));
            d_act_probs = d_ap;
            act_tiles.table = d_at; act_tiles.base = 0; act_tiles.end = (int)at.size();
        }
        *shared_px_out = spx;
    }
    int grp_split = 0;
    {
        const char *e = std::getenv("OBIA_PREPASS_GROUPS");
        const int mode = !e ? 1 : (e[0] == '0' ? 0 : (e[0] == '2' ? 2 : 1));
        if (mode != 0 && n_shared == 0 && b.masked && pre_iter >= 2 && !store_all && !prepass_visits && !prep_grouped && !b.direct &&
            b.nprob >= 2 && !std::getenv("OBIA_DEBUG_SYNC")) {
            long long best = -1;
            for (int p = 1; p < b.nprob; ++p) {
                const long long t0 = b.probs[p].tile_off, t1 = b.total_tiles_all - t0, d = t0 > t1 ? t0 - t1 : t1 - t0;
                if (t0 > 0 && t1 > 0 && (best < 0 || d <= best)) { best = d; grp_split = p; }
            }
            if (grp_split > 0 && mode != 2) {
                const long long t0 = b.probs[grp_split].tile_off, t1 = b.total_tiles_all - t0;
                if ((t0 < t1 ? t0 : t1) < (long long)spatial_residency(ctx, b.CP)) grp_split = 0;
            }
            if (grp_split > 0) OBIA_TRY(side_stream(ctx));
        }
    }
    OBIA_HIP_TRY(hipMemsetAsync(d_px, 0, sizeof(unsigned long long) * 513, ctx->stream));
    OBIA_HIP_TRY(hipMemsetAsync(b.d_head, 0xff, sizeof(int) * (size_t)b.total_cells, ctx->stream));
    OBIA_HIP_TRY(hipMemsetAsync(b.d_tl_meta, 0xff, sizeof(int) * 3 * (size_t)b.total_tiles_all, ctx->stream));
    debug_sync(ctx, "sweeps: memsets");
    bool first = true;
    int sweep_no = 0;
    for (int pass = 0; pass < passes; ++pass) {
        const int ignore_color = (b.masked && pass == 0) ? 1 : 0;
        const bool last_pass = (pass == passes - 1);
        if (pass > 0 && store_all) {
            fill_labels(ctx, b);
            if (fp.tile_lp) OBIA_HIP_TRY(hipMemsetAsync(fp.tile_lp, 0, sizeof(int) * (size_t)b.total_tiles_all, ctx->stream));
        }
        const int iters = ignore_color ? pre_iter : b.max_iter;
        for (int it = 0; it < iters; ++it) {
            int *head_cur = b.d_head + (size_t)(sweep_no & 1) * b.total_cells;
            int *head_nxt = b.d_head + (size_t)((sweep_no + 1) & 1) * b.total_cells;
            ++sweep_no;
            const int zmode = (b.slic_zero && !ignore_color) ? (it == 0 ? 2 : 1) : 0;
            const bool shared_sweep = n_shared > 0 && ignore_color && it < iters - 1;
            if (n_shared > 0 && ignore_color && it == iters - 1) {
                hipLaunchKernelGGL(slic_prepass_broadcast_kernel, dim3(cdiv(kmax_mem, 64), n_shared), dim3(64), 0, ctx->stream, b.d_probs,
                                   d_member_rep, b.CP, RQ, b.d_acc, b.d_cent, b.d_ref);
                debug_sync(ctx, "sweeps: pre-pass broadcast");
            }
            const dim3 prep_grid(cdiv(shared_sweep ? kmax_act : kmax, 64), shared_sweep ? n_act : b.nprob);
            const int prep_base = shared_sweep ? act_p_base : 0;
            const int *prep_table = shared_sweep ? d_act_probs : nullptr;
#define LAUNCH_PREP_LANE(CPV)                                                                                         \
    hipLaunchKernelGGL(HIP_KERNEL_NAME(slic_prep_lane_kernel<CPV>), pgrid, dim3(64), 0, stream, \
                       b.d_probs, p_base, first ? 1 : 0, zmode, b.d_seed, b.d_acc, RQ, 1.0 / b.fscale, b.d_cent, head_cur, head_nxt, \
                       cell_end, fp.bin_stamp, sweep_no, cell_base, b.d_ref, b.d_tl_req, table)
            auto prep_lane = [&](hipStream_t stream, dim3 pgrid, int p_base, const int *table, int cell_base, int cell_end) {
                switch (b.CP) {
                    case 4: LAUNCH_PREP_LANE(4); break;
                    case 8: LAUNCH_PREP_LANE(8); break;
                    case 12: LAUNCH_PREP_LANE(12); break;
                    default: LAUNCH_PREP_LANE(16); break;
                }
            };
#undef LAUNCH_PREP_LANE
            if (grp_split > 0 && ignore_color && it < iters - 1) {
                hipError_t he = hipSuccess;
                if (it == 0) {
                    he = hipEventRecord(ctx->grp_fork, ctx->stream);
                    if (he == hipSuccess) he = hipStreamWaitEvent(ctx->side, ctx->grp_fork, 0);
                }
                for (int g = 0; g < 2 && he == hipSuccess; ++g) {
                    const int p0 = g ? grp_split : 0, p1 = g ? b.nprob : grp_split;
                    int kmax_g = 1;
                    for (int p = p0; p < p1; ++p) if (b.probs[p].K > kmax_g) kmax_g = b.probs[p].K;
                    const hipStream_t st = g ? ctx->side : ctx->stream;
                    prep_lane(st, dim3(cdiv(kmax_g, 64), p1 - p0), p0, nullptr, b.probs[p0].cell_off, g ? b.total_cells : b.probs[p1].cell_off);
                    KernelSpan span(ctx, T_PREPASS);
                    TileSubset sub;
                    sub.base = b.probs[p0].tile_off;
                    sub.end = g ? (int)b.total_tiles_all : b.probs[p1].tile_off;
                    unsigned long long *pxc = ctx->profiling ? d_px + 256 : nullptr;
                    switch (b.CP) {
                        case 8: launch_assign<8>(ctx, b, 1, 1, 0, 0, d_orphan, fp, sweep_no, 1, pxc, span, head_cur, false, sub, false, &st); break;
#ifndef OBIA_ONLY_CP8
                        case 4: launch_assign<4>(ctx, b, 1, 1, 0, 0, d_orphan, fp, sweep_no, 1, pxc, span, head_cur, false, sub, false, &st); break;
                        case 12: launch_assign<12>(ctx, b, 1, 1, 0, 0, d_orphan, fp, sweep_no, 1, pxc, span, head_cur, false, sub, false, &st); break;
                        case 16: launch_assign<16>(ctx, b, 1, 1, 0, 0, d_orphan, fp, sweep_no, 1, pxc, span, head_cur, false, sub, false, &st); break;
#endif
                        default: he = hipErrorInvalidValue; break;
                    }
                    ctx->timing.prepass_group_launches += 1;
                }
                if (he == hipSuccess && it == iters - 2) {
                    he = hipEventRecord(ctx->grp_join, ctx->side);
                    if (he == hipSuccess) he = hipStreamWaitEvent(ctx->stream, ctx->grp_join, 0);
                }
                if (he != hipSuccess) {
                    (void)hipStreamSynchronize(ctx->side);
                    set_error("grouped pre-pass: %s", hipGetErrorString(he));
                    return OBIA_E_HIP;
                }
                b.d_head_cur = head_cur;
                first = false;
                continue;
            }
            if (!prep_grouped) prep_lane(ctx->stream, prep_grid, prep_base, prep_table, 0, b.total_cells);
            else if (RQ == 16)
                hipLaunchKernelGGL(HIP_KERNEL_NAME(slic_prep_kernel<16>), dim3(cdiv(b.total_cent * 16LL, 256)), dim3(256), 0,
                                   ctx->stream, b.d_probs, b.d_cent_prob, b.total_cent, b.CP, first ? 1 : 0, zmode, b.d_seed, b.d_acc,
                                   1.0 / b.fscale, b.d_cent, head_cur, head_nxt, b.total_cells, fp.bin_stamp, sweep_no, 0, 0, b.d_ref, b.d_tl_req);
            else
                hipLaunchKernelGGL(HIP_KERNEL_NAME(slic_prep_kernel<32>), dim3(cdiv(b.total_cent * 32LL, 256)), dim3(256), 0,
                                   ctx->stream, b.d_probs, b.d_cent_prob, b.total_cent, b.CP, first ? 1 : 0, zmode, b.d_seed, b.d_acc,
                                   1.0 / b.fscale, b.d_cent, head_cur, head_nxt, b.total_cells, fp.bin_stamp, sweep_no, 0, 0, b.d_ref, b.d_tl_req);
            b.d_head_cur = head_cur;
            debug_sync(ctx, "sweeps: prep");
            first = false;
            if (zmode == 1) {
                dim3 zg(maxh_z, b.nprob);
#define LAUNCH_MAXDIST(CPV)                                                                                           \
    do {                                                                                                              \
        if (b.masked) hipLaunchKernelGGL(HIP_KERNEL_NAME(slic_maxdist_kernel<CPV, true>), zg, dim3(256), 0, ctx->stream, b.d_probs, \
                                         b.d_feat, b.d_mask, b.d_labels, b.d_cent, b.start_label, b.C);            \
        else hipLaunchKernelGGL(HIP_KERNEL_NAME(slic_maxdist_kernel<CPV, false>), zg, dim3(256), 0, ctx->stream, b.d_probs, \
                                b.d_feat, b.d_mask, b.d_labels, b.d_cent, b.start_label, b.C);                     \
    } while (0)
                switch (b.CP) {
                    case 4: LAUNCH_MAXDIST(4); break;
                    case 8: LAUNCH_MAXDIST(8); break;
                    case 12: LAUNCH_MAXDIST(12); break;
                    default: LAUNCH_MAXDIST(16); break;
                }
#undef LAUNCH_MAXDIST
            }
            const bool very_last = last_pass && it == iters - 1;
            const int accumulate = very_last ? 0 : 1;
            const int accum_color = (!ignore_color || it == iters - 1) ? 1 : 0;
            const int store_labels = store_all ? 2 : (very_last ? 1 : 0);
            const int use_cache = (ignore_color && it == iters - 1) ? 0 : 1;
            const bool rawin = b.fuse_features && !repeat && ignore_color && it == iters - 1;
            {
                KernelSpan span(ctx, ignore_color ? T_PREPASS : T_ASSIGN);
                const TileSubset sub = shared_sweep ? act_tiles : TileSubset();
                unsigned long long *pxc = ctx->profiling ? d_px + (ignore_color ? 256 : 0) : nullptr;
                if (ctx->profiling && !ignore_color && store_labels) ctx->timing.assign_store_px += (double)b.total_pix;
                switch (b.CP) {
                    case 8: launch_assign<8>(ctx, b, ignore_color, accumulate, accum_color, store_labels, d_orphan, fp, sweep_no, use_cache, pxc, span, head_cur, prepass_visits, sub, rawin); break;
#ifndef OBIA_ONLY_CP8
                    case 4: launch_assign<4>(ctx, b, ignore_color, accumulate, accum_color, store_labels, d_orphan, fp, sweep_no, use_cache, pxc, span, head_cur, prepass_visits, sub, rawin); break;
                    case 12: launch_assign<12>(ctx, b, ignore_color, accumulate, accum_color, store_labels, d_orphan, fp, sweep_no, use_cache, pxc, span, head_cur, prepass_visits, sub, rawin); break;
                    case 16: launch_assign<16>(ctx, b, ignore_color, accumulate, accum_color, store_labels, d_orphan, fp, sweep_no, use_cache, pxc, span, head_cur, prepass_visits, sub); break;
#endif
                    default: set_error("bad CP"); return OBIA_E_INVALID;
                }
            }
            debug_sync(ctx, ignore_color ? "sweeps: pre-pass sweep" : "sweeps: colour sweep");
        }
    }
    OBIA_HIP_TRY(hipGetLastError());
    *d_px_out = d_px;
    return OBIA_OK;
}

int slic_run_sweeps(obia_ctx *ctx, SlicBatch &b) {
    ctx->defer_pending = false;
    unsigned long long *d_px = nullptr;
    ctx->defer_shared_px = 0.0;
    OBIA_TRY(queue_sweeps(ctx, b, false, &d_px, &ctx->defer_shared_px));
    if (!d_px) return OBIA_OK;
    if (!ctx->defer_buf) OBIA_HIP_TRY(hipHostMalloc(reinterpret_cast<void **>(&ctx->defer_buf), sizeof(unsigned long long) * 513, hipHostMallocDefault));
    OBIA_HIP_TRY(hipMemcpyAsync(ctx->defer_buf, d_px, sizeof(unsigned long long) * 513, hipMemcpyDeviceToHost, ctx->stream));
    ctx->defer_pending = true;
    return OBIA_OK;
}

int slic_sweeps_settle(obia_ctx *ctx, bool *repeat) {
    *repeat = false;
    if (!ctx->defer_pending) return OBIA_OK;
    ctx->defer_pending = false;
    const unsigned long long *h = ctx->defer_buf;
    if ((h[512] & 0xffffffffull) != 0ull) { *repeat = true; return OBIA_OK; }
    fold_counters(ctx, h, ctx->defer_shared_px);
    return OBIA_OK;
}

int slic_rerun_storing(obia_ctx *ctx, SlicBatch &b) {
    ctx->timing.batch_repeats += 1;
    unsigned long long *d_px = nullptr;
    double shared_px = 0.0;
    OBIA_TRY(queue_sweeps(ctx, b, true, &d_px, &shared_px));
    if (!d_px) return OBIA_OK;
    unsigned long long h[513];
    OBIA_TRY(read_back(ctx, h, d_px, sizeof(h)));
    fold_counters(ctx, h, shared_px);
    return OBIA_OK;
}

}
```

### obia_amd/csrc/tiling.hip

```cpp
#include "slic.hpp"

#include <cmath>
#include <cstdlib>

namespace obia {

struct TileWin { int y0, x0, h, w; long long pix_off; int cly, clx; int cly_in, clx_in, cly_any, clx_any; int m4_off; };

__device__ __forceinline__ void wave_hist_add(unsigned *hist, int key, bool active) {
    bool todo = active;
    while (true) {
        const unsigned long long act = __ballot(todo);
        if (!act) break;
        const int leader = __ffsll((long long)act) - 1;
        const int kk = __shfl(key, leader);
        const unsigned long long same = __ballot(todo && key == kk);
        if ((int)(threadIdx.x & 63) == leader) atomicAdd(&hist[kk], (unsigned)__popcll(same));
        if (key == kk) todo = false;
    }
}

__device__ __forceinline__ bool in_corner(const TileWin &t, int y, int x) {
    return (y >= t.h - t.cly) && (x < t.clx || x >= t.w - t.clx);
}
// ... 217 lines not shown
    for (int q = 0; q < 16; ++q)
        if (i0 + q < n_ids) { if (f[q]) { run += 1; newid[i0 + q] = run; } else newid[i0 + q] = 0; }
    if (blockIdx.x == gridDim.x - 1 && tid == 1023) *total = before + inc;
}

__global__ __launch_bounds__(256) void ids_apply_kernel(int32_t *__restrict__ G, long long n, const int *__restrict__ newid) {
    const long long n4 = ((reinterpret_cast<uintptr_t>(G) & 15) == 0) ? n / 4 : 0;
    int4 *G4 = reinterpret_cast<int4 *>(G);
    for (long long i = (long long)blockIdx.x * blockDim.x + threadIdx.x; i < n4; i += (long long)gridDim.x * blockDim.x) {
        int4 g = G4[i];
        g.x = g.x > 0 ? newid[g.x] : 0;
        g.y = g.y > 0 ? newid[g.y] : 0;
        g.z = g.z > 0 ? newid[g.z] : 0;
        g.w = g.w > 0 ? newid[g.w] : 0;
        G4[i] = g;
    }
    for (long long i = n4 * 4 + (long long)blockIdx.x * blockDim.x + threadIdx.x; i < n; i += (long long)gridDim.x * blockDim.x) {
        const int g = G[i];
        G[i] = g > 0 ? newid[g] : 0;
    }
}

struct TileState {
    int H, W, C;
    int Hg, row0;
    const float *img;
    const uint8_t *inmask;
    int32_t *G;
    unsigned *seg_size, *inside;
    uint8_t *alive;
    int *newid;
    long long *d_total;
    int id_cap, next_id;
    int clx, cly, clx_in, cly_in, clx_any, cly_any;
    obia_tiling_params tp;
    obia_slic_params sp;
    SlicBatch settings;
    int seeding = OBIA_SEEDING_GRID;
    obia_pick_fn pick_fn = nullptr;
    void *pick_user = nullptr;
    struct PreFeat {
        bool ready = false;
        bool planned = false;
        bool fused = false;
        SlicBatch b;
        std::vector<unsigned> host;
        unsigned *d_keys = nullptr;
        bool launched = false;
        bool on_side = false;
        size_t cursor = 0;
    } pf;
};


static int grid_rows(const std::vector<TileWin> &wins) {
    int g = 1;
    for (auto &t : wins) if (t.h > g) g = t.h;
    return g > 8192 ? 8192 : g;
}

#ifndef OBIA_PREFETCH_BESIDE
#define OBIA_PREFETCH_BESIDE 0
#endif
static int prefetch_white_launch(obia_ctx *ctx, TileState &S, bool beside = false);

static int seed_tiles_skimage(obia_ctx *ctx, TileState &S, const SlicBatch &b, const std::vector<int> &nvalid, std::vector<int> &nseg,
                              std::vector<ExternalSeeds> &ext) {
    const int np = b.nprob;
    if (!S.pick_fn) { set_error("seeding = skimage needs a pick function"); return OBIA_E_INVALID; }
    Arena &A = ctx->arena;
    ext.assign(np, ExternalSeeds{nullptr, 0, 1.0, nullptr});
    std::vector<long long> off(np, 0);
    long long total = 0;
    for (int p = 0; p < np; ++p) {
        if (nseg[p] < 2 || nvalid[p] < 2) { nseg[p] = 0; continue; }
        off[p] = total;
        total += std::min(nseg[p], nvalid[p]);
    }
    if (total == 0) return OBIA_OK;
    if (total > 0x7fff0000LL) { set_error("too many centroids in one batch"); return OBIA_E_INVALID; }
    float *d_seeds = A.get<float>(2 * (size_t)total);
    double *d_steps = A.get<double>(2 * (size_t)np);
    if (!d_seeds || !d_steps) return OBIA_E_NOMEM;
    OBIA_HIP_TRY(hipMemsetAsync(d_steps, 0, sizeof(double) * 2 * (size_t)np, ctx->stream));
    auto ascending_below = [](const int64_t *v, long long n, long long bound) {
        if (v[0] < 0 || v[n - 1] >= bound) return false;
        for (long long i = 1; i < n; ++i) if (v[i] <= v[i - 1]) return false;
        return true;
    };
    for (int p = 0; p < np; ++p) {
        if (nseg[p] == 0) continue;
        const int K = std::min(nseg[p], nvalid[p]);
        const int64_t *idx = nullptr, *dense = nullptr;
        int32_t n_idx = 0;
        int64_t n_dense = 0;
        if (S.pick_fn(S.pick_user, (int64_t)nvalid[p], (int32_t)nseg[p], &idx, &n_idx, &dense, &n_dense) != 0) {
            set_error("the pick function failed for a tile with %d valid pixels and n_segments = %d", nvalid[p], nseg[p]);
            return OBIA_E_INVALID;
        }
        if (!idx || n_idx != K || !ascending_below(idx, K, nvalid[p]) ||
            (dense && (n_dense < 1 || n_dense > nvalid[p] || !ascending_below(dense, n_dense, nvalid[p])))) {
            set_error("the pick function returned bad picks for a tile with %d valid pixels and n_segments = %d: %d strictly ascending ranks below the "
                      "valid count are needed", nvalid[p], nseg[p], K);
            return OBIA_E_INVALID;
        }
        const SlicProblem &P = b.probs[p];
        OBIA_TRY(mask_centroids_queue(ctx, b.d_mask + P.pix_off, P.H, P.W, nvalid[p], idx, K, dense, dense ? (long long)n_dense : 0, 5,
                                      d_seeds + 2 * off[p], d_steps + 2 * (size_t)p));
        ext[p].n = K;
        ext[p].d_yx = d_seeds + 2 * off[p];
    }
    std::vector<double> steps(2 * (size_t)np);
    OBIA_TRY(read_back(ctx, steps.data(), d_steps, sizeof(double) * steps.size()));
    for (int p = 0; p < np; ++p) {
        if (ext[p].n == 0) continue;
        const double st = std::max(steps[2 * (size_t)p], steps[2 * (size_t)p + 1]);
        if (!(st >= 0.0) || !(st < 1e9)) { set_error("tile seeding: steps are not finite"); return OBIA_E_INVALID; }
        ext[p].step = st;
    }
    return OBIA_OK;
}

static int run_tile_batch(obia_ctx *ctx, TileState &S, std::vector<TileWin> &wins, bool white) {
    const int np = (int)wins.size();
    if (np == 0) return OBIA_OK;
    Arena &A = ctx->arena;
    const Arena::Mark mk = A.mark();
    SlicBatch b = S.settings;
    for (auto &t : wins) b.windows.push_back(SrcWindow{t.y0, t.x0, t.h, t.w, 0, 0, 0});
    OBIA_TRY(slic_batch_layout(b));
    for (int p = 0; p < np; ++p) { wins[p].pix_off = b.probs[p].pix_off; wins[p].m4_off = b.probs[p].m4_off; }
    TileWin *d_wins = A.get<TileWin>(np);
    b.d_windows = A.get<SrcWindow>(np);
    b.d_mask = A.get<uint8_t>((size_t)b.total_pix);
    unsigned *d_mask4 = A.get<unsigned>((size_t)b.total_m4);
    if (!d_mask4) return OBIA_E_NOMEM;
    const bool pre = white && S.pf.ready;
    if (pre) {
        const SlicBatch &pb = S.pf.b;
        if (S.pf.cursor + np > pb.windows.size()) { set_error("white batch beyond the prefetched windows"); return OBIA_E_INVALID; }
        const SrcWindow *a = &pb.windows[S.pf.cursor];
        for (int p = 0; p < np; ++p)
            if (a[p].y0 != wins[p].y0 || a[p].x0 != wins[p].x0 || a[p].h != wins[p].h || a[p].w != wins[p].w) { set_error("white batch does not match the prefetched windows"); return OBIA_E_INVALID; }
        if (S.pf.fused) {
            b.d_feat = A.get<float>(4 * (size_t)b.total_feat_f4);
            b.fuse_features = true;
            b.raw_src = S.img; b.raw_ws = S.W;
            b.d_keys = S.pf.d_keys + S.pf.cursor * (size_t)S.C * 2;
        } else {
            b.d_feat = pb.d_feat + 4 * (size_t)a[0].feat_off;
            if (b.col_lb) b.d_fbox = pb.d_fbox + (size_t)a[0].fb_off * 2 * b.CP;
        }
    } else {
        b.d_feat = A.get<float>(4 * (size_t)b.total_feat_f4);
        if (b.col_lb) {
            b.d_fbox = A.get<float>((size_t)b.total_boxes * 2 * b.CP);
            if (!b.d_fbox) return OBIA_E_NOMEM;
        }
    }
    b.d_labels = A.get<int32_t>((size_t)b.total_pix);
    if (!d_wins || !b.d_windows || !b.d_mask || !b.d_feat || !b.d_labels) return OBIA_E_NOMEM;
    OBIA_TRY(upload_async(ctx, d_wins, wins.data(), sizeof(TileWin) * np));
    OBIA_TRY(upload_async(ctx, b.d_windows, b.windows.data(), sizeof(SrcWindow) * np));
    int *d_tile_any = A.get<int>(np);
    if (!d_tile_any) return OBIA_E_NOMEM;
    if (white) {
        OBIA_HIP_TRY(hipMemsetAsync(S.inside, 0, sizeof(unsigned) * (size_t)S.next_id, ctx->stream));
        OBIA_HIP_TRY(hipMemsetAsync(d_tile_any, 0, sizeof(int) * (size_t)np, ctx->stream));
        hipLaunchKernelGGL(tile_count_inside_kernel, dim3(grid_rows(wins), np), dim3(256), 0, ctx->stream, d_wins, S.G, S.W, S.inside, d_tile_any);
    }
    {
        bool vec4 = (S.W % 4 == 0) && (reinterpret_cast<uintptr_t>(S.inmask) % 4 == 0) && (reinterpret_cast<uintptr_t>(S.G) % 16 == 0) &&
                    (reinterpret_cast<uintptr_t>(b.d_mask) % 4 == 0) && (reinterpret_cast<uintptr_t>(d_mask4) % 16 == 0);
        for (auto &t : wins) vec4 = vec4 && (t.x0 % 4 == 0) && (t.w % 4 == 0) && (t.pix_off % 4 == 0);
        if (vec4) {
            hipLaunchKernelGGL(HIP_KERNEL_NAME(tile_mask_kernel<true>), dim3((grid_rows(wins) + 3) / 4, np), dim3(256), 0, ctx->stream, d_wins, S.inmask,
                               S.G, S.W, white ? 1 : 0, S.inside, S.seg_size, S.alive, b.d_mask, d_tile_any, d_mask4);
            b.d_mask4 = d_mask4;
        } else {
            hipLaunchKernelGGL(HIP_KERNEL_NAME(tile_mask_kernel<false>), dim3(grid_rows(wins), np), dim3(256), 0, ctx->stream, d_wins, S.inmask,
                               S.G, S.W, white ? 1 : 0, S.inside, S.seg_size, S.alive, b.d_mask, d_tile_any, d_mask4);
        }
    }
    std::vector<int> skip;
    if (pre) {
        const size_t NP = S.pf.b.windows.size(), nkeys = NP * (size_t)S.C * 2;
        const unsigned *h = S.pf.host.data();
        OBIA_TRY(slic_features_finish(b, h + S.pf.cursor * (size_t)S.C * 2, h + nkeys + S.pf.cursor, h + nkeys + NP + S.pf.cursor, &skip));
        S.pf.cursor += np;
    } else {
        OBIA_TRY(slic_prepare_features(ctx, b, S.img, S.W, &skip));
    }
    std::vector<int> nvalid;
    debug_sync(ctx, "tiler: mask + features");
    OBIA_TRY(slic_count_valid(ctx, b, nvalid));
    debug_sync(ctx, "tiler: count_valid");
    std::vector<int> nseg(np);
    const double pixel_area = S.tp.pixel_width * S.tp.pixel_height;
    const double crown_area = M_PI * S.tp.crown_radius * S.tp.crown_radius;
    for (int p = 0; p < np; ++p) {
        double n;
        if (S.sp.n_segments > 0)
            n = std::nearbyint((double)S.sp.n_segments * (double)nvalid[p] / ((double)S.tp.tile_size * S.tp.tile_size));
        else
            n = std::nearbyint((double)nvalid[p] * pixel_area / crown_area);
        nseg[p] = (skip[p] || n < 1.0) ? 0 : (n > 2.0e9 ? 2000000000 : (int)n);
    }
    std::vector<ExternalSeeds> ext;
    if (S.seeding == OBIA_SEEDING_SKIMAGE) OBIA_TRY(seed_tiles_skimage(ctx, S, b, nvalid, nseg, ext));
    OBIA_TRY(slic_plan_and_seed(ctx, b, nseg, &nvalid, ext.empty() ? nullptr : ext.data()));
    debug_sync(ctx, "tiler: plan_and_seed");
    if (!white && S.pf.planned && !S.pf.launched)
        OBIA_TRY(prefetch_white_launch(ctx, S, OBIA_PREFETCH_BESIDE != 0 || b.exit_on_fixed_point || b.slic_zero));
    const Arena::Mark sweeps_mk = A.mark();
    unsigned *const mask4 = b.d_mask4;
    OBIA_TRY(slic_run_sweeps(ctx, b));
    debug_sync(ctx, "tiler: sweeps");
    int n_new = 0;
    CcResolve resolve{};
    if (S.sp.enforce_connectivity) {
        std::vector<CcProblem> cps(np);
        for (int p = 0; p < np; ++p) {
            const SlicProblem &P = b.probs[p];
            const auto [min_size, max_size] = slic_cc_sizes(S.sp.min_size_factor, S.sp.max_size_factor, P.n_valid, P.K);
            cps[p] = CcProblem{P.H, P.W, P.pix_off, min_size, max_size};
        }
        OBIA_TRY(enforce_connectivity_batch(ctx, cps, b.d_labels, b.total_pix, 1, nullptr, &n_new, &resolve));
        bool repeat = false;
        OBIA_TRY(slic_sweeps_settle(ctx, &repeat));
        if (repeat) {
            A.rewind(sweeps_mk);
            b.d_mask4 = mask4;
            OBIA_TRY(slic_rerun_storing(ctx, b));
            OBIA_TRY(enforce_connectivity_batch(ctx, cps, b.d_labels, b.total_pix, 1, nullptr, &n_new, &resolve));
        }
        debug_sync(ctx, "tiler: connectivity");
    } else {
        set_error("the tiled driver needs enforce_connectivity=True (segments must be connected pixel sets)");
        return OBIA_E_UNSUPPORTED;
    }
    if (S.next_id + n_new > S.id_cap) { set_error("segment id capacity exceeded (%d + %d > %d)", S.next_id, n_new, S.id_cap); return OBIA_E_NOMEM; }
    if (n_new > 0) {
        int sblocks = 1;
        for (auto &t : wins) sblocks = std::max(sblocks, cdiv(t.w, 64) * cdiv(t.h, 64));
        hipLaunchKernelGGL(tile_scatter_kernel, dim3(sblocks, np), dim3(64), 0, ctx->stream, d_wins, resolve, S.G, S.W,
                           S.next_id - 1, S.seg_size);
        OBIA_HIP_TRY(hipMemsetAsync(S.alive + S.next_id, 1, (size_t)n_new, ctx->stream));
        S.next_id += n_new;
    }
    OBIA_HIP_TRY(hipGetLastError());
    A.rewind(mk);
    return OBIA_OK;
}

__global__ __launch_bounds__(256) void seam_mark_kernel(const int32_t *__restrict__ codes, int n, int me, int owner, int32_t *__restrict__ fmap,
                                                        int cap, int *__restrict__ new_list, int *__restrict__ ctr, int32_t *__restrict__ ids) {
    int tmax = 0;
    for (int i = blockIdx.x * blockDim.x + threadIdx.x; i < n; i += gridDim.x * blockDim.x) {
        const int c = codes[i];
        int id = 0;
        if (c > 0) {
            const int o = (c >> 24) - 1, t = c & 0xffffff;
            if (o == me) id = t;
            else if (o == owner) {
                tmax = max(tmax, t);
                if (t > 0 && t < cap) {
                    const int f = fmap[t];
                    if (f > 0) id = f;
                    else if (f == 0 && atomicCAS(&fmap[t], 0, -1) == 0) new_list[atomicAdd(&ctr[0], 1)] = t;
                }
            }
        }
        ids[i] = id;
    }
    for (int off = 32; off > 0; off >>= 1) tmax = max(tmax, __shfl_xor(tmax, off));
    if ((threadIdx.x & 63) == 0 && tmax > 0) atomicMax(&ctr[1], tmax);
}
constexpr int SEAM_SORT = 16384;
__global__ __launch_bounds__(1024) void seam_assign_sort_kernel(int *__restrict__ new_list, int m, int first, int owner,
                                                                int32_t *__restrict__ fmap, int32_t *__restrict__ code_of) {
    __shared__ int s[SEAM_SORT];
    int np2 = 1;
    while (np2 < m) np2 <<= 1;
    for (int i = threadIdx.x; i < np2; i += 1024) s[i] = i < m ? new_list[i] : 0x7fffffff;
    __syncthreads();
    for (int k = 2; k <= np2; k <<= 1)
        for (int j = k >> 1; j > 0; j >>= 1) {
            for (int i = threadIdx.x; i < np2; i += 1024) {
                const int ixj = i ^ j;
                if (ixj > i) {
                    const int a = s[i], b = s[ixj];
                    if (((i & k) == 0) ? (a > b) : (a < b)) { s[i] = b; s[ixj] = a; }
                }
            }
            __syncthreads();
        }
    for (int i = threadIdx.x; i < m; i += 1024) {
        const int t = s[i];
        fmap[t] = first + i;
        code_of[first + i] = t | ((owner + 1) << 24);
    }
}
__global__ __launch_bounds__(256) void seam_assign_count_kernel(const int *__restrict__ new_list, int m, int first, int owner,
                                                                int32_t *__restrict__ fmap, int32_t *__restrict__ code_of) {
    for (int i = blockIdx.x * blockDim.x + threadIdx.x; i < m; i += gridDim.x * blockDim.x) {
        const int t = new_list[i];
        int rank = 0;
        for (int j = 0; j < m; ++j) rank += new_list[j] < t;
        fmap[t] = first + rank;
        code_of[first + rank] = t | ((owner + 1) << 24);
    }
}
__global__ __launch_bounds__(256) void seam_translate_kernel(const int32_t *__restrict__ codes, int n, int owner,
                                                             const int32_t *__restrict__ fmap, int cap, int32_t *__restrict__ ids) {
    for (int i = blockIdx.x * blockDim.x + threadIdx.x; i < n; i += gridDim.x * blockDim.x) {
        if (ids[i] != 0) continue;
        const int c = codes[i];
        if (c <= 0 || (c >> 24) - 1 != owner) continue;
        const int t = c & 0xffffff;
        if (t > 0 && t < cap) ids[i] = fmap[t];
    }
}
__global__ void seam_register_kernel(unsigned *__restrict__ seg_size, uint8_t *__restrict__ alive, int first, int count) {
    const int i = blockIdx.x * blockDim.x + threadIdx.x;
    if (i < count) { seg_size[first + i] = 0xffffffffu; alive[first + i] = 1; }
}

static int tiler_check(const float *img, int H, int W, int C, int Hg, int row0, const obia_tiling_params *tp,
                       const obia_slic_params *sp, const int32_t *labels) {
    if (!img || !tp || !sp || !labels) { set_error("null argument"); return OBIA_E_INVALID; }
    if (H <= 0 || W <= 0 || C <= 0 || C > 16) { set_error("bad raster shape (%d,%d,%d)", H, W, C); return OBIA_E_INVALID; }
    if (row0 < 0 || row0 + H > Hg) { set_error("local rows [%d,%d) outside the global raster of %d rows", row0, row0 + H, Hg); return OBIA_E_INVALID; }
    if ((long long)H * W > 0x7fffffffLL) { set_error("raster above 2^31 pixels: shard it across GPUs"); return OBIA_E_INVALID; }
    if (tp->tile_size <= 0 || tp->buffer < 0) { set_error("tile_size must be positive and buffer non-negative"); return OBIA_E_INVALID; }
    if (!(sp->compactness > 0.0) || sp->max_num_iter < 0) { set_error("bad SLIC parameters"); return OBIA_E_INVALID; }
    for (int i = 0; i < 3; ++i) {
        if (!(sp->sigma_zyx[i] >= 0.0)) { set_error("sigma must be >= 0"); return OBIA_E_INVALID; }
        if (!(sp->spacing_zyx[i] > 0.0) || !(sp->spacing_zyx[i] < 1.0e30)) { set_error("spacing must be positive and finite"); return OBIA_E_INVALID; }
    }
    if (!sp->enforce_connectivity) { set_error("the tiled driver needs enforce_connectivity=True (segments must be connected pixel sets)"); return OBIA_E_UNSUPPORTED; }
    if (sp->n_segments <= 0 && !(tp->crown_radius > 0.0 && tp->pixel_width > 0.0 && tp->pixel_height > 0.0)) {
        set_error("crown_radius and pixel size must be positive when n_segments is not given");
        return OBIA_E_INVALID;
    }
    return OBIA_OK;
}

static int tiler_init(obia_ctx *ctx, TileState &S, const float *img, const uint8_t *mask, int H, int W, int C, int Hg,
                      int row0, const obia_tiling_params *tp, const obia_slic_params *sp, int32_t *labels, int extra_ids) {
    OBIA_TRY(tiler_check(img, H, W, C, Hg, row0, tp, sp, labels));
    const int T = tp->tile_size, B = tp->buffer;
    Arena &A = ctx->arena;
    const int ntx = cdiv(W, T), nty = cdiv(H, T) + 2;
    const double pixel_area = tp->pixel_width * tp->pixel_height;
    const double crown_area = M_PI * tp->crown_radius * tp->crown_radius;
    const long long wh = (long long)(T + 2 * B) * (T + 2 * B);
    double n = sp->n_segments > 0 ? (double)sp->n_segments * (double)wh / ((double)T * T) : (double)wh * pixel_area / crown_area;
    if (n < 1) n = 1;
    long long cap = (long long)(n * 1.5 + 64.0) * (long long)ntx * nty + 16 + extra_ids;
    if (cap > 0x7ffffff0LL) { set_error("too many segments for int32 ids"); return OBIA_E_INVALID; }
    S.H = H; S.W = W; S.C = C; S.Hg = Hg; S.row0 = row0; S.img = img; S.inmask = mask; S.G = labels; S.tp = *tp; S.sp = *sp;
    S.id_cap = (int)cap; S.next_id = 1;
    slic_batch_settings(S.settings, *sp, C, 1, true);
    S.settings.start_label = 1;
    S.seg_size = A.get<unsigned>((size_t)cap);
    S.inside = A.get<unsigned>((size_t)cap);
    S.alive = A.get<uint8_t>((size_t)cap);
    S.newid = A.get<int>((size_t)cap);
    S.d_total = A.get<long long>(1);
    if (!S.seg_size || !S.inside || !S.alive || !S.newid || !S.d_total) return OBIA_E_NOMEM;
    OBIA_HIP_TRY(hipMemsetAsync(S.seg_size, 0, sizeof(unsigned) * (size_t)cap, ctx->stream));
    OBIA_HIP_TRY(hipMemsetAsync(S.alive, 0, (size_t)cap, ctx->stream));
    S.clx = S.cly = S.clx_in = S.cly_in = S.clx_any = S.cly_any = 0;
    if (B > 0) {
        const double cl = (double)B / 2.0;
        auto count = [](double px, double cl, int kind) {
            if (!(px > 0.0)) px = 1.0;
            long long k = (long long)std::floor(cl / px) + 2;
            if (k < 0) k = 0;
            auto holds = [&](long long i) { return kind == 0 ? (i + 0.5) * px < cl : (kind == 1 ? (i + 1.0) * px <= cl : i * px < cl); };
            while (k > 0 && !holds(k - 1)) --k;
            return (int)std::min<long long>(k, 0x3fffffff);
        };
        S.clx = count(tp->pixel_width, cl, 0);  S.cly = count(tp->pixel_height, cl, 0);
        S.clx_in = count(tp->pixel_width, cl, 1);  S.cly_in = count(tp->pixel_height, cl, 1);
        S.clx_any = count(tp->pixel_width, cl, 2);  S.cly_any = count(tp->pixel_height, cl, 2);
    }
    return OBIA_OK;
}

static TileWin white_window(const TileState &S, int tj, int ti) {
    const int T = S.tp.tile_size, B = S.tp.buffer;
    const int y0 = std::max(0, tj * T - B), y1 = std::min(S.Hg, tj * T + T + B);
    const int x0 = std::max(0, ti * T - B), x1 = std::min(S.W, ti * T + T + B);
    const int h = y1 - y0, w = x1 - x0;
    return TileWin{y0 - S.row0, x0, h, w, 0, std::min(S.cly, h), std::min(S.clx, w), std::min(S.cly_in, h), std::min(S.clx_in, w),
                   std::min(S.cly_any, h), std::min(S.clx_any, w), 0};
}

static int prefetch_white_plan(obia_ctx *ctx, TileState &S, int white_order) {
    const int T = S.tp.tile_size;
    const int ntx = cdiv(S.W, T), nty = cdiv(S.Hg, T);
    TileState::PreFeat &pf = S.pf;
    pf = TileState::PreFeat();
    if (S.sp.sigma_zyx[0] > 0.0 || S.sp.sigma_zyx[1] > 0.0 || S.sp.sigma_zyx[2] > 0.0) return OBIA_OK;
    SlicBatch b = S.settings;
    for (int cls = 0; cls < (white_order == 1 ? 2 : 1); ++cls)
        for (int tj = 0; tj < nty; ++tj) {
            if (white_order == 1 && (tj & 1) != cls) continue;
            for (int ti = 0; ti < ntx; ++ti) {
                if ((ti + tj) % 2 == 0) continue;
                const TileWin t = white_window(S, tj, ti);
                if (t.h <= 0 || t.w <= 0) continue;
                if (t.y0 < 0 || t.y0 + t.h > S.H) return OBIA_OK;
                b.windows.push_back(SrcWindow{t.y0, t.x0, t.h, t.w, 0, 0, 0});
            }
        }
    const size_t NP = b.windows.size();
    if (NP == 0) return OBIA_OK;
    if (slic_batch_layout(b) != OBIA_OK) return OBIA_OK;
    pf.fused = slic_fuse_features(b, S.img, S.W);
    if (!pf.fused && (double)b.total_feat_f4 * 16.0 > 32.0 * 1024 * 1024 * 1024) return OBIA_OK;
    Arena &A = ctx->arena;
    const size_t ntot = NP * (size_t)S.C * 2 + 2 * NP;
    b.d_windows = A.get<SrcWindow>(NP);
    pf.d_keys = A.get<unsigned>(ntot);
    if (!pf.fused) b.d_feat = A.get<float>(4 * (size_t)b.total_feat_f4);
    if (!b.d_windows || !pf.d_keys || (!pf.fused && !b.d_feat)) return OBIA_E_NOMEM;
    if (b.col_lb) {
        b.d_fbox = A.get<float>((size_t)b.total_boxes * 2 * b.CP);
        if (!b.d_fbox) return OBIA_E_NOMEM;
    }
    pf.host.resize(ntot);
    pf.b = std::move(b);
    pf.planned = true;
    return OBIA_OK;
}

static int prefetch_white_launch(obia_ctx *ctx, TileState &S, bool beside) {
    TileState::PreFeat &pf = S.pf;
    if (pf.launched || !pf.planned) return OBIA_OK;
    pf.launched = true;
    if (pf.fused) beside = false;
    OBIA_TRY(upload_async(ctx, pf.b.d_windows, pf.b.windows.data(), sizeof(SrcWindow) * pf.b.windows.size()));
    if (beside) {
        OBIA_TRY(side_stream(ctx));
        hipStream_t side = ctx->side;
        OBIA_HIP_TRY(hipEventRecord(ctx->aux_fork, ctx->stream));
        OBIA_HIP_TRY(hipStreamWaitEvent(side, ctx->aux_fork, 0));
        OBIA_TRY(slic_features_launch(side, pf.b, S.img, S.W, pf.d_keys, nullptr, false));
        OBIA_HIP_TRY(hipEventRecord(ctx->aux_join, side));
        pf.on_side = true;
        return OBIA_OK;
    }
    ScopedSpan span(ctx, T_FEAT);
    OBIA_TRY(slic_features_launch(ctx->stream, pf.b, S.img, S.W, pf.d_keys, nullptr, pf.fused));
    return OBIA_OK;
}

static int prefetch_white_fetch(obia_ctx *ctx, TileState &S) {
    if (!S.pf.planned) return OBIA_OK;
    OBIA_TRY(prefetch_white_launch(ctx, S));
    if (S.pf.on_side) { OBIA_HIP_TRY(hipStreamWaitEvent(ctx->stream, ctx->aux_join, 0)); S.pf.on_side = false; }
    OBIA_TRY(read_back(ctx, S.pf.host.data(), S.pf.d_keys, S.pf.host.size() * sizeof(unsigned)));
    S.pf.ready = true;
    S.pf.cursor = 0;
    return OBIA_OK;
}

static int tiler_run(obia_ctx *ctx, TileState &S, bool white, int tr_lo, int tr_hi, int parity) {
    const int T = S.tp.tile_size, B = S.tp.buffer;
    const int ntx = cdiv(S.W, T), nty = cdiv(S.Hg, T);
    if (tr_lo < 0) tr_lo = 0;
    if (tr_hi > nty) tr_hi = nty;
    const bool per_row = !(parity >= 0 && T > 2 * B);
    const bool per_tile = white && T <= 2 * B;
    std::vector<TileWin> wins;
    auto flush = [&]() -> int {
        for (auto &t : wins)
            if (t.y0 < 0 || t.y0 + t.h > S.H) { set_error("tile window rows [%d,%d) (local) outside the %d local rows: halo too small", t.y0, t.y0 + t.h, S.H); return OBIA_E_INVALID; }
        int rc = run_tile_batch(ctx, S, wins, white);
        wins.clear();
        return rc;
    };
    for (int tj = tr_lo; tj < tr_hi; ++tj) {
        if (parity >= 0 && (tj & 1) != parity) continue;
        for (int ti = 0; ti < ntx; ++ti) {
            const bool is_white = (ti + tj) % 2 != 0;
            if (is_white != white) continue;
            if (!white) {
                TileWin t{tj * T - S.row0, ti * T, std::min(T, S.Hg - tj * T), std::min(T, S.W - ti * T), 0, 0, 0, 0, 0, 0, 0, 0};
                if (t.h > 0 && t.w > 0) wins.push_back(t);
            } else {
                const TileWin t = white_window(S, tj, ti);
                if (t.h > 0 && t.w > 0) wins.push_back(t);
                if (per_tile && !wins.empty()) OBIA_TRY(flush());
            }
        }
        if (white && per_row) OBIA_TRY(flush());
    }
    if (!wins.empty()) OBIA_TRY(flush());
    return OBIA_OK;
}

static int tiler_finalize(obia_ctx *ctx, TileState &S, int64_t *n_segments_out) {
    const int nchunks = cdiv(S.next_id, IDS_CHUNK);
    int *d_partial = ctx->arena.get<int>((size_t)nchunks);
    if (!d_partial) return OBIA_E_NOMEM;
    hipLaunchKernelGGL(ids_count_kernel, dim3(nchunks), dim3(1024), 0, ctx->stream, S.alive, S.next_id, d_partial);
    hipLaunchKernelGGL(ids_scan_kernel, dim3(nchunks), dim3(1024), 0, ctx->stream, S.alive, S.next_id, d_partial, S.newid, S.d_total);
    int g = cdiv((long long)S.H * S.W, 256 * 16);
    if (g > 65535) g = 65535;
    hipLaunchKernelGGL(ids_apply_kernel, dim3(g), dim3(256), 0, ctx->stream, S.G, (long long)S.H * S.W, S.newid);
    OBIA_HIP_TRY(hipGetLastError());
    long long total = 0;
    OBIA_TRY(read_back(ctx, &total, S.d_total, sizeof(long long)));
    if (n_segments_out) *n_segments_out = total;
    return OBIA_OK;
}

static int check_seeding(int seeding, obia_pick_fn picks) {
    if (seeding != OBIA_SEEDING_GRID && seeding != OBIA_SEEDING_SKIMAGE) { set_error("seeding must be OBIA_SEEDING_GRID or OBIA_SEEDING_SKIMAGE (got %d)", seeding); return OBIA_E_INVALID; }
    if (seeding == OBIA_SEEDING_SKIMAGE && !picks) { set_error("seeding = skimage needs a pick function"); return OBIA_E_INVALID; }
    return OBIA_OK;
}

static int tiled_slic_dev(obia_ctx *ctx, const float *img, const uint8_t *mask, int H, int W, int C,
                          const obia_tiling_params *tp, const obia_slic_params *sp, int seeding, obia_pick_fn picks, void *picks_user,
                          int32_t *labels_out, int64_t *n_segments_out) {
    TileState S;
    OBIA_TRY(check_seeding(seeding, picks));
    OBIA_TRY(tiler_init(ctx, S, img, mask, H, W, C, H, 0, tp, sp, labels_out, 0));
    S.seeding = seeding; S.pick_fn = picks; S.pick_user = picks_user;
    OBIA_HIP_TRY(hipMemsetAsync(labels_out, 0, sizeof(int32_t) * (size_t)H * W, ctx->stream));
    const int nty = cdiv(H, tp->tile_size);
    OBIA_TRY(prefetch_white_plan(ctx, S, tp->white_order));
    OBIA_TRY(tiler_run(ctx, S, false, 0, nty, -1));
    if (std::getenv("OBIA_DEBUG_FAIL_AFTER_BLACK")) {
        set_error("debug: forced failure after the black pass");
        return OBIA_E_INVALID;
    }
    OBIA_TRY(prefetch_white_fetch(ctx, S));
    if (tp->white_order == 1) {
        OBIA_TRY(tiler_run(ctx, S, true, 0, nty, 0));
        OBIA_TRY(tiler_run(ctx, S, true, 0, nty, 1));
    } else {
        OBIA_TRY(tiler_run(ctx, S, true, 0, nty, -1));
    }
    return tiler_finalize(ctx, S, n_segments_out);
}

}

struct obia_tiler {
    obia_ctx *ctx;
    obia::TileState S;
    int *seam_buf = nullptr;
    size_t seam_cap = 0;
};

using namespace obia;

static int enter(obia_tiler *t) {
    if (!t) { set_error("null tiler"); return OBIA_E_INVALID; }
    return enter(t->ctx);
}

extern "C" {

obia_tiler *obia_tiler_create(obia_ctx *ctx, const float *img_local, const uint8_t *mask_local, int H_local, int W, int C,
                              int H_global, int row0, const obia_tiling_params *tiling, const obia_slic_params *params,
                              int32_t *labels_local, int extra_ids) {
    if (enter(ctx) != OBIA_OK) return nullptr;
    frame_begin(ctx, FRAME_TIMING);
    obia_tiler *t = new obia_tiler();
    t->ctx = ctx;
    if (tiler_init(ctx, t->S, img_local, mask_local, H_local, W, C, H_global, row0, tiling, params, labels_local,
                   extra_ids < 0 ? 0 : extra_ids) != OBIA_OK) { delete t; return nullptr; }
    return t;
}

void obia_tiler_destroy(obia_tiler *t) {
    if (!t) return;
    (void)enter(t->ctx);
    (void)quiesce(t->ctx, 0);
    if (t->seam_buf) (void)hipFree(t->seam_buf);
    resolve_timing(t->ctx);
    delete t;
}

int obia_tiler_run(obia_tiler *t, int white, int tile_row_lo, int tile_row_hi, int row_parity) {
    OBIA_TRY(enter(t));
    const int rc = tiler_run(t->ctx, t->S, white != 0, tile_row_lo, tile_row_hi, row_parity);
    if (rc != OBIA_OK) return quiesce(t->ctx, rc);
    OBIA_HIP_TRY(hipStreamSynchronize(t->ctx->stream));
    return OBIA_OK;
}

int obia_tiler_next_id(obia_tiler *t) { return t ? t->S.next_id : -1; }

int obia_tiler_set_seeding(obia_tiler *t, int seeding, obia_pick_fn picks, void *picks_user) {
    OBIA_TRY(enter(t));
    OBIA_TRY(check_seeding(seeding, picks));
    t->S.seeding = seeding; t->S.pick_fn = picks; t->S.pick_user = picks_user;
    return OBIA_OK;
}

int obia_tiler_set_segments(obia_tiler *t, int first_id, int count, const uint32_t *sizes_dev) {
    OBIA_TRY(enter(t));
    if (!sizes_dev || first_id < 1 || count < 0) { set_error("bad arguments"); return OBIA_E_INVALID; }
    if (first_id + count > t->S.id_cap) { set_error("segment id capacity exceeded (%d + %d > %d)", first_id, count, t->S.id_cap); return OBIA_E_NOMEM; }
    if (count == 0) return OBIA_OK;
    OBIA_HIP_TRY(hipMemcpyAsync(t->S.seg_size + first_id, sizes_dev, sizeof(uint32_t) * (size_t)count, hipMemcpyDeviceToDevice, t->ctx->stream));
    OBIA_HIP_TRY(hipMemsetAsync(t->S.alive + first_id, 1, (size_t)count, t->ctx->stream));
    if (first_id + count > t->S.next_id) t->S.next_id = first_id + count;
    OBIA_HIP_TRY(hipStreamSynchronize(t->ctx->stream));
    return OBIA_OK;
}

int obia_tiler_get_alive(obia_tiler *t, uint8_t *alive_out_dev, int count) {
    OBIA_TRY(enter(t));
    if (!alive_out_dev || count < 0 || count > t->S.id_cap) { set_error("bad arguments"); return OBIA_E_INVALID; }
    OBIA_HIP_TRY(hipMemcpyAsync(alive_out_dev, t->S.alive, (size_t)count, hipMemcpyDeviceToDevice, t->ctx->stream));
    OBIA_HIP_TRY(hipStreamSynchronize(t->ctx->stream));
    return OBIA_OK;
}

int obia_tiler_set_alive(obia_tiler *t, const uint8_t *alive_in_dev, int count) {
    OBIA_TRY(enter(t));
    if (!alive_in_dev || count < 0 || count > t->S.id_cap) { set_error("bad arguments"); return OBIA_E_INVALID; }
    OBIA_HIP_TRY(hipMemcpyAsync(t->S.alive, alive_in_dev, (size_t)count, hipMemcpyDeviceToDevice, t->ctx->stream));
    OBIA_HIP_TRY(hipStreamSynchronize(t->ctx->stream));
    return OBIA_OK;
}

int obia_tiler_import_seam(obia_tiler *t, const int32_t *codes_dev, int n, int my_rank, int owner_rank,
                           int32_t *fmap_dev, int fmap_cap, int32_t *code_of_dev, int32_t *ids_out_dev,
                           int *first_new_out, int *n_new_out, int *max_owner_id_out) {
    OBIA_TRY(enter(t));
    if (!codes_dev || !fmap_dev || !code_of_dev || !ids_out_dev || n < 0 || fmap_cap < 1 || my_rank < 0 || owner_rank < 0 ||
        my_rank > 126 || owner_rank > 126 || !first_new_out || !n_new_out || !max_owner_id_out) { set_error("bad arguments"); return OBIA_E_INVALID; }
    obia_ctx *ctx = t->ctx;
    *first_new_out = t->S.next_id; *n_new_out = 0; *max_owner_id_out = 0;
    if (n == 0) return OBIA_OK;
    if (t->seam_cap < (size_t)n + 2) {
        if (t->seam_buf) (void)hipFree(t->seam_buf);
        t->seam_buf = nullptr; t->seam_cap = 0;
        if (hipMalloc(&t->seam_buf, sizeof(int) * ((size_t)n + 2)) != hipSuccess) { set_error("seam scratch allocation failed"); return OBIA_E_NOMEM; }
        t->seam_cap = (size_t)n + 2;
    }
    int *ctr = t->seam_buf, *new_list = t->seam_buf + 2;
    OBIA_HIP_TRY(hipMemsetAsync(ctr, 0, sizeof(int) * 2, ctx->stream));
    const int blocks = std::min(cdiv(n, 256), 2048);
    hipLaunchKernelGGL(seam_mark_kernel, dim3(blocks), dim3(256), 0, ctx->stream, codes_dev, n, my_rank, owner_rank, fmap_dev, fmap_cap, new_list, ctr,
                       ids_out_dev);
    int h[2] = {0, 0};
    OBIA_TRY(read_back(ctx, h, ctr, sizeof(h)));
    *max_owner_id_out = h[1];
    const int n_new = h[0];
    if (t->S.next_id + n_new > t->S.id_cap) { set_error("segment id capacity exceeded (%d + %d > %d)", t->S.next_id, n_new, t->S.id_cap); return OBIA_E_NOMEM; }
    if (n_new > 0) {
        if (n_new <= SEAM_SORT)
            hipLaunchKernelGGL(seam_assign_sort_kernel, dim3(1), dim3(1024), 0, ctx->stream, new_list, n_new, t->S.next_id, owner_rank, fmap_dev, code_of_dev);
        else
            hipLaunchKernelGGL(seam_assign_count_kernel, dim3(256), dim3(256), 0, ctx->stream, new_list, n_new, t->S.next_id, owner_rank, fmap_dev, code_of_dev);
        hipLaunchKernelGGL(seam_translate_kernel, dim3(blocks), dim3(256), 0, ctx->stream, codes_dev, n, owner_rank, fmap_dev, fmap_cap, ids_out_dev);
        hipLaunchKernelGGL(seam_register_kernel, dim3(cdiv(n_new, 256)), dim3(256), 0, ctx->stream, t->S.seg_size, t->S.alive, t->S.next_id, n_new);
        t->S.next_id += n_new;
        OBIA_HIP_TRY(hipStreamSynchronize(ctx->stream));
    }
    *n_new_out = n_new;
    OBIA_HIP_TRY(hipGetLastError());
    return OBIA_OK;
}

int obia_tiler_finalize(obia_tiler *t, int64_t *n_segments_out) {
    OBIA_TRY(enter(t));
    const int rc = tiler_finalize(t->ctx, t->S, n_segments_out);
    return rc == OBIA_OK ? rc : quiesce(t->ctx, rc);
}

int obia_tiled_slic_seeded_f32_dev(obia_ctx *ctx, const float *img, const uint8_t *mask, int H, int W, int C,
                                   const obia_tiling_params *tiling, const obia_slic_params *params, int seeding,
                                   obia_pick_fn picks, void *picks_user, int32_t *labels_out, int64_t *n_segments_out) {
    OBIA_TRY(enter(ctx));
    return call_frame(ctx, FRAME_TOTAL, [&] {
        return tiled_slic_dev(ctx, img, mask, H, W, C, tiling, params, seeding, picks, picks_user, labels_out, n_segments_out);
    });
}

int obia_tiled_slic_f32_dev(obia_ctx *ctx, const float *img, const uint8_t *mask, int H, int W, int C,
                            const obia_tiling_params *tiling, const obia_slic_params *params, int32_t *labels_out,
                            int64_t *n_segments_out) {
    return obia_tiled_slic_seeded_f32_dev(ctx, img, mask, H, W, C, tiling, params, OBIA_SEEDING_GRID, nullptr, nullptr, labels_out, n_segments_out);
}

int obia_tiled_slic_seeded_f32(obia_ctx *ctx, const float *img, const uint8_t *mask, int H, int W, int C,
                               const obia_tiling_params *tiling, const obia_slic_params *params, int seeding,
                               obia_pick_fn picks, void *picks_user, int32_t *labels_out, int64_t *n_segments_out) {
    OBIA_TRY(enter(ctx));
    if (!img || !labels_out || H <= 0 || W <= 0 || C <= 0) { set_error("bad arguments"); return OBIA_E_INVALID; }
    OBIA_TRY(check_seeding(seeding, picks));
    const size_t npix = (size_t)H * W;
    Staging s(ctx);
    const float *d_img = s.in(img, npix * C);
    const uint8_t *d_mask = s.in(mask, npix);
    int32_t *d_lab = s.out<int32_t>(npix);
    s.run([&] {
        return obia_tiled_slic_seeded_f32_dev(ctx, d_img, d_mask, H, W, C, tiling, params, seeding, picks, picks_user, d_lab, n_segments_out);
    });
    s.fetch(labels_out, d_lab, npix);
    return s.finish();
}

int obia_tiled_slic_f32(obia_ctx *ctx, const float *img, const uint8_t *mask, int H, int W, int C,
                        const obia_tiling_params *tiling, const obia_slic_params *params, int32_t *labels_out,
                        int64_t *n_segments_out) {
    return obia_tiled_slic_seeded_f32(ctx, img, mask, H, W, C, tiling, params, OBIA_SEEDING_GRID, nullptr, nullptr, labels_out, n_segments_out);
}

}
```

### obia_amd/csrc/zonal.hip

```cpp
#include "slic.hpp"

namespace obia {

#ifndef ZW
#define ZW 6
#endif
#ifndef ZR
#define ZR 2
#endif
#ifndef ZTW
#define ZTW 128
#endif
#ifndef ZTH
#define ZTH 64
#endif
#ifndef ZSLOTS
#define ZSLOTS 64
#endif
constexpr int Z_MAXB = 16, Z_ROWS = ZR;
constexpr unsigned Z_NOPIV = 0x7fc00001u;

__device__ __forceinline__ float claim_pivot(unsigned *piv, float cand) {
    const unsigned old = atomicCAS(piv, Z_NOPIV, __float_as_uint(cand));
    return old == Z_NOPIV ? cand : __uint_as_float(old);
// ... 363 lines not shown
                if (l != rl) {
                    close_run();
                    rl = l;
#pragma unroll
                    for (int b = 0; b < 4; ++b) {
                        rn[b] = 0; r2[b] = 0.0; r3[b] = 0.0; r4[b] = 0.0;
                        mu[b] = (l >= 0 && b < nbq) ? mean[(size_t)l * nb + 4 * q + b] : 0.0;
                    }
                }
                if (l < 0) continue;
                const float *v = val[half][j];
#pragma unroll
                for (int b = 0; b < 4; ++b) {
                    const bool ok = v[b] == v[b];
                    const double d = ok ? (double)v[b] - mu[b] : 0.0;
                    const double d2 = d * d;
                    rn[b] += ok ? 1u : 0u; r2[b] += d2; r3[b] = fma(d2, d, r3[b]); r4[b] = fma(d2, d2, r4[b]);
                }
            }
        }
    }
    close_run();
    __syncthreads();
    for (int i = tid; i < ZSLOTS * nb; i += NT) {
        const int slot = i / nb, b = i - slot * nb;
        const int l = s_key[slot];
        if (l < 0 || s_n[slot][b] == 0) continue;
        const size_t o = (size_t)l * nb + b;
        atomicAdd(&g_n[o], s_n[slot][b]);
        unsafeAtomicAdd(&g_s2[o], s_s2[slot][b]);
        unsafeAtomicAdd(&g_s3[o], s_s3[slot][b]);
        unsafeAtomicAdd(&g_s4[o], s_s4[slot][b]);
    }
}

__global__ void zonal_moments_finalize_kernel(const unsigned *__restrict__ g_n, const double *__restrict__ g_s2,
                                              const double *__restrict__ g_s3, const double *__restrict__ g_s4,
                                              const double *__restrict__ mean, long long n, double *__restrict__ skew,
                                              double *__restrict__ kurt, double *__restrict__ var) {
    for (long long i = (long long)blockIdx.x * blockDim.x + threadIdx.x; i < n; i += (long long)gridDim.x * blockDim.x) {
        const unsigned c = g_n[i];
        double sk = NAN, ku = NAN;
        if (var && c == 0) var[i] = NAN;
        if (c > 0) {
            const double m2 = g_s2[i] / (double)c, m3 = g_s3[i] / (double)c, m4 = g_s4[i] / (double)c;
            if (var) var[i] = m2;
            const double t = 1.1920928955078125e-07 * mean[i];
            if (!(m2 <= t * t)) {
                sk = m3 / (m2 * sqrt(m2));
                ku = m4 / (m2 * m2) - 3.0;
            }
        }
        skew[i] = sk; kurt[i] = ku;
    }
}

int zonal_moments_dev(obia_ctx *ctx, const float *raw, const int32_t *labels, int H, int W, int C,
                      const int32_t *bands_host, int n_bands, int n_labels, int start_label, const double *mean,
                      double *skew, double *kurt, double *var) {
    ScopedSpan span(ctx, T_ZONAL);
    if (H <= 0 || W <= 0 || C <= 0 || n_labels < 0) { set_error("bad zonal_moments shape"); return OBIA_E_INVALID; }
    BandList bl;
    if (bands_host == nullptr) {
        if (C > Z_MAXB) { set_error("more than %d bands not supported", Z_MAXB); return OBIA_E_UNSUPPORTED; }
        bl.n = C;
        for (int i = 0; i < C; ++i) bl.b[i] = i;
    } else {
        if (n_bands < 1 || n_bands > Z_MAXB) { set_error("n_bands %d out of range (1..%d)", n_bands, Z_MAXB); return OBIA_E_UNSUPPORTED; }
        bl.n = n_bands;
        for (int i = 0; i < n_bands; ++i) {
            if (bands_host[i] < 0 || bands_host[i] >= C) { set_error("band index %d out of range (0..%d)", bands_host[i], C - 1); return OBIA_E_INVALID; }
            bl.b[i] = bands_host[i];
        }
    }
    for (int i = bl.n; i < Z_MAXB; ++i) bl.b[i] = 0;
    bl.identity = 1;
    for (int i = 0; i < bl.n; ++i) if (bl.b[i] != i) bl.identity = 0;
    if (n_labels == 0) return OBIA_OK;
    Arena &A = ctx->arena;
    const size_t nlb = (size_t)n_labels * bl.n;
    unsigned *g_n = A.get<unsigned>(nlb);
    double *g_s2 = A.get<double>(nlb), *g_s3 = A.get<double>(nlb), *g_s4 = A.get<double>(nlb);
    if (!g_n || !g_s2 || !g_s3 || !g_s4) return OBIA_E_NOMEM;
    OBIA_HIP_TRY(hipMemsetAsync(g_n, 0, sizeof(unsigned) * nlb, ctx->stream));
    OBIA_HIP_TRY(hipMemsetAsync(g_s2, 0, sizeof(double) * nlb, ctx->stream));
    OBIA_HIP_TRY(hipMemsetAsync(g_s3, 0, sizeof(double) * nlb, ctx->stream));
    OBIA_HIP_TRY(hipMemsetAsync(g_s4, 0, sizeof(double) * nlb, ctx->stream));
    if ((long long)W * C * 4 >= (1ll << 32)) { set_error("a raster row of %lld bytes is not supported (4 GB at most)", (long long)W * C * 4); return OBIA_E_UNSUPPORTED; }
    const int tiles = cdiv(W, ZTW) * cdiv(H, ZTH);
    const bool ident = bl.identity && bl.n == C;
#define LAUNCH_ZM_MODE(NBPV, MODEV)                                                                                  \
    hipLaunchKernelGGL(HIP_KERNEL_NAME(zonal_moments_kernel<NBPV, MODEV>), dim3(tiles), dim3(ZTW / 4 * NBPV), 0, ctx->stream, raw, \
                       labels, H, W, C, bl, n_labels, start_label, mean, g_n, g_s2, g_s3, g_s4)
#define LAUNCH_ZM(NBPV)                                                                                              \
    do {                                                                                                             \
        if (ident && bl.n == NBPV) LAUNCH_ZM_MODE(NBPV, 0);                                                          \
        else if (ident) LAUNCH_ZM_MODE(NBPV, 1);                                                                     \
        else LAUNCH_ZM_MODE(NBPV, 2);                                                                                \
    } while (0)
    if (bl.n <= 4) LAUNCH_ZM(4);
    else if (bl.n <= 8) LAUNCH_ZM(8);
    else if (bl.n <= 12) LAUNCH_ZM(12);
    else LAUNCH_ZM(16);
#undef LAUNCH_ZM
#undef LAUNCH_ZM_MODE
    int ib = cdiv((long long)nlb, 256);
    if (ib > 4096) ib = 4096;
    hipLaunchKernelGGL(zonal_moments_finalize_kernel, dim3(ib), dim3(256), 0, ctx->stream, g_n, g_s2, g_s3, g_s4, mean,
                       (long long)nlb, skew, kurt, var);
    OBIA_HIP_TRY(hipGetLastError());
    return OBIA_OK;
}

int zonal_stats_dev(obia_ctx *ctx, const float *raw, const int32_t *labels, int H, int W, int C,
                    const int32_t *bands_host, int n_bands, int n_labels, int start_label, int64_t *count,
                    double *mean, double *var, float *mn, float *mx) {
    ScopedSpan span(ctx, T_ZONAL);
    if (H <= 0 || W <= 0 || C <= 0 || n_labels < 0) { set_error("bad zonal_stats shape"); return OBIA_E_INVALID; }
    BandList bl;
    if (bands_host == nullptr) {
        if (C > Z_MAXB) { set_error("more than %d bands not supported", Z_MAXB); return OBIA_E_UNSUPPORTED; }
        bl.n = C;
        for (int i = 0; i < C; ++i) bl.b[i] = i;
    } else {
        if (n_bands < 1 || n_bands > Z_MAXB) { set_error("n_bands %d out of range (1..%d)", n_bands, Z_MAXB); return OBIA_E_UNSUPPORTED; }
        bl.n = n_bands;
        for (int i = 0; i < n_bands; ++i) {
            if (bands_host[i] < 0 || bands_host[i] >= C) { set_error("band index %d out of range (0..%d)", bands_host[i], C - 1); return OBIA_E_INVALID; }
            bl.b[i] = bands_host[i];
        }
    }
    for (int i = bl.n; i < Z_MAXB; ++i) bl.b[i] = 0;
    bl.identity = 1;
    for (int i = 0; i < bl.n; ++i) if (bl.b[i] != i) bl.identity = 0;
    if ((long long)W * C * 4 >= (1ll << 32)) { set_error("a raster row of %lld bytes is not supported (4 GB at most)", (long long)W * C * 4); return OBIA_E_UNSUPPORTED; }
    if (n_labels == 0) return OBIA_OK;
    Arena &A = ctx->arena;
    const size_t nl = (size_t)n_labels, nlb = nl * bl.n;
    unsigned *g_cnt = A.get<unsigned>(nl), *g_bcnt = A.get<unsigned>(nlb);
    double *g_sum = A.get<double>(nlb), *g_sq = A.get<double>(nlb);
    unsigned *g_mn = A.get<unsigned>(nlb), *g_mx = A.get<unsigned>(nlb), *g_piv = A.get<unsigned>(nlb);
    if (!g_cnt || !g_bcnt || !g_sum || !g_sq || !g_mn || !g_mx || !g_piv) return OBIA_E_NOMEM;
    int ib = cdiv((long long)nlb, 256);
    if (ib > 4096) ib = 4096;
    hipLaunchKernelGGL(zonal_init_kernel, dim3(ib), dim3(256), 0, ctx->stream, g_cnt, g_bcnt, g_sum, g_sq, g_mn, g_mx, g_piv, (long long)n_labels, bl.n);
    const int tiles = cdiv(W, ZTW) * cdiv(H, ZTH);
    const bool ident = bl.identity && bl.n == C;
#define LAUNCH_ZONAL_MODE(LPPV, BPLV, MODEV)                                                                        \
    hipLaunchKernelGGL(HIP_KERNEL_NAME(zonal_kernel<LPPV, BPLV, MODEV>), dim3(tiles), dim3(ZTW * LPPV), 0, ctx->stream, raw, labels, H, W, C, \
                       bl, n_labels, start_label, g_cnt, g_bcnt, g_sum, g_sq, g_mn, g_mx, g_piv)
#define LAUNCH_ZONAL(LPPV)                                                                                          \
    do {                                                                                                            \
        if (ident && bl.n == 4 * LPPV) LAUNCH_ZONAL_MODE(LPPV, 4, 0);                                               \
        else if (ident) LAUNCH_ZONAL_MODE(LPPV, 4, 1);                                                              \
        else LAUNCH_ZONAL_MODE(LPPV, 4, 2);                                                                         \
    } while (0)
    if (ident && bl.n == 3) LAUNCH_ZONAL_MODE(1, 3, 0);
    else if (ident && bl.n == 6) LAUNCH_ZONAL_MODE(2, 3, 0);
    else if (ident && bl.n == 9) LAUNCH_ZONAL_MODE(3, 3, 0);
    else if (bl.n <= 4) LAUNCH_ZONAL(1);
    else if (bl.n <= 8) LAUNCH_ZONAL(2);
    else if (bl.n <= 12) LAUNCH_ZONAL(3);
    else LAUNCH_ZONAL(4);
#undef LAUNCH_ZONAL
#undef LAUNCH_ZONAL_MODE
    hipLaunchKernelGGL(zonal_finalize_kernel, dim3(ib), dim3(256), 0, ctx->stream, g_cnt, g_bcnt, g_sum, g_sq, g_mn, g_mx, g_piv,
                       (long long)n_labels, bl.n, count, mean, var, mn, mx);
    OBIA_HIP_TRY(hipGetLastError());
    return OBIA_OK;
}
// ... 3 lines not shown
```

Before: 7452.

## Batch small uploads into a plan blob and coalesce memsets into one clear kernel

Adds a PlanBlob that packs small host-to-device metadata uploads (windows, CC problems, tiles) into one staged transfer flushed before kernels or readbacks. Adds a ClearSet that merges several hipMemsetAsync calls into a single multi-range clear kernel, used for zonal moment accumulators and tiler counters. It also folds the CC ring buffer into an existing zeroed allocation, adds fill/upload/readback counters, and adds a settle sync after rerun. The aim is to cut per-call launch and API overhead, at the cost of added flush-ordering complexity.

```diff
diff --git a/include/obia_testing.h b/include/obia_testing.h
--- /dev/null
+++ b/include/obia_testing.h
@@ -0,0 +1,15 @@
+#ifndef OBIA_TESTING_H
+#define OBIA_TESTING_H
+
+#include "obia_hip.h"
+
+#ifdef __cplusplus
+extern "C" {
+#endif
+
+int obia_test_clear_ranges_dev(obia_ctx *ctx, void *const *dev_ptrs, const int64_t *bytes, const int32_t *values, int n);
+
+#ifdef __cplusplus
+}
+#endif
+#endif
diff --git a/obia_amd/_lib.py b/obia_amd/_lib.py
--- a/obia_amd/_lib.py
+++ b/obia_amd/_lib.py
@@ -149,6 +149,9 @@
     "obia_sharp_variance_dev": (_I, [_P, _P, _I, _I, _I, _P, _P]),
     "obia_sharp_stretch_f32_dev": (_I, [_P, _P, ctypes.c_int64, ctypes.c_double, ctypes.c_double, _P]),
 }
+_TEST_SIGNATURES = {
+    "obia_test_clear_ranges_dev": (_I, [_P, _P, _P, _P, _I]),
+}
 
 _lib = None
 
@@ -168,7 +171,7 @@
             raise ImportError(f"{LIB_PATH} not found: build it with `python -c 'import __graft_entry__ as g; g.build()'` "
                               "(hipcc, gfx950). obia_amd has no CPU fallback.")
         lib = ctypes.CDLL(LIB_PATH)
-        for name, (res, args) in list(_SIGNATURES.items()) + list(_IMAGE_SIGNATURES.items()) + list(_SHARPNESS_SIGNATURES.items()):
+        for name, (res, args) in list(_SIGNATURES.items()) + list(_IMAGE_SIGNATURES.items()) + list(_SHARPNESS_SIGNATURES.items()) + list(_TEST_SIGNATURES.items()):
             try:
                 fn = getattr(lib, name)
             except AttributeError:
@@ -232,7 +235,7 @@
         lib = load()
         names = ["assign_ms", "sweeps", "features_ms", "connectivity_ms", "zonal_ms", "total_ms", "prepass_ms", "assign_px",
                  "prepass_px", "assign_store_px", "assign_busy_ms", "prepass_busy_ms", "batch_repeats",
-                 "prepass_shared_px", "feature_fused_px", "prepass_group_launches"]
+                 "prepass_shared_px", "feature_fused_px", "prepass_group_launches", "fills", "uploads", "readbacks"]
         return {n: lib.obia_last_timing(self._h, i) for i, n in enumerate(names)}
 
     def workspace_bytes(self):
diff --git a/obia_amd/csrc/api.cpp b/obia_amd/csrc/api.cpp
--- a/obia_amd/csrc/api.cpp
+++ b/obia_amd/csrc/api.cpp
@@ -58,6 +58,8 @@
         A.rewind(sweeps_mk);
         b.d_mask4 = nullptr;
         OBIA_TRY(slic_rerun_storing(ctx, b));
+        OBIA_HIP_TRY(hipStreamSynchronize(ctx->stream));
+        OBIA_TRY(slic_sweeps_settle(ctx, nullptr));
     }
     return OBIA_OK;
 }
diff --git a/obia_amd/csrc/cc.hip b/obia_amd/csrc/cc.hip
--- a/obia_amd/csrc/cc.hip
+++ b/obia_amd/csrc/cc.hip
@@ -748,27 +748,30 @@
 
 int enforce_connectivity_batch(obia_ctx *ctx, const std::vector<CcProblem> &probs, const int32_t *labels_in,
                                long long total_pix, int start_label, int32_t *labels_out, int *h_n_labels_out,
-                               CcResolve *deferred) {
+                               CcResolve *deferred, const CcProblem *d_probs_in) {
     ScopedSpan span(ctx, T_CC);
     Arena &A = ctx->arena;
     const long long n = total_pix;
     const int np = (int)probs.size();
     if (np <= 0 || n <= 0 || n > 0x7fffffffLL) { set_error("label batch of %lld pixels not supported", n); return OBIA_E_INVALID; }
     const int mask_label = start_label - 1;
-    CcProblem *d_probs = A.get<CcProblem>(np);
+    const CcProblem *d_probs = d_probs_in ? d_probs_in : ctx->plan.add(ctx, probs.data(), (size_t)np);
     int *parent = A.get<int>(n), *size = A.get<int>(n), *newlab = A.get<int>(n);
     const int nb = cdiv(n, SCAN_CHUNK);
     int *block_sums = A.get<int>(3 * (size_t)nb);
     unsigned long long *rootbits = A.get<unsigned long long>((size_t)((n + 63) / 64));
     if (!rootbits) return OBIA_E_NOMEM;
-    unsigned long long *lrbits_block = A.get<unsigned long long>((size_t)((n + 63) / 64) + 4);
+    constexpr int RING = 64;
+    constexpr size_t LR_HEAD = 4 + RING / 2;
+    unsigned long long *lrbits_block = A.get<unsigned long long>((size_t)((n + 63) / 64) + LR_HEAD);
     if (!lrbits_block) return OBIA_E_NOMEM;
-    unsigned long long *lrbits = lrbits_block + 4;
+    unsigned long long *lrbits = lrbits_block + LR_HEAD;
+    int *const ring = reinterpret_cast<int *>(lrbits_block + 4);
     const unsigned long long *rb = rootbits;
     int *counters = reinterpret_cast<int *>(lrbits_block);
     if (!d_probs || !parent || !size || !newlab || !block_sums) return OBIA_E_NOMEM;
-    OBIA_TRY(upload_async(ctx, d_probs, probs.data(), sizeof(CcProblem) * np));
-    OBIA_HIP_TRY(hipMemsetAsync(lrbits_block, 0, sizeof(unsigned long long) * ((size_t)((n + 63) / 64) + 4), ctx->stream));
+    OBIA_TRY(ctx->plan.flush(ctx));
+    OBIA_TRY(fill_async(ctx, lrbits_block, 0, sizeof(unsigned long long) * ((size_t)((n + 63) / 64) + LR_HEAD)));
     int gs = cdiv(n, 256 * 4);
     if (gs > 65535 * 4) gs = 65535 * 4;
     {
@@ -796,7 +799,7 @@
         const int n_big = hc[6];
         int *big_root = A.get<int>(n_big), *big_qoff = A.get<int>(n_big), *big_box = A.get<int>(4 * (size_t)n_big);
         if (!big_root || !big_qoff || !big_box) return OBIA_E_NOMEM;
-        OBIA_HIP_TRY(hipMemsetAsync(counters, 0, sizeof(int) * 8, ctx->stream));
+        OBIA_TRY(fill_async(ctx, counters, 0, sizeof(int) * 8));
         hipLaunchKernelGGL(cc_flatten_all_kernel, dim3(gs), dim3(256), 0, ctx->stream, parent, n);
         hipLaunchKernelGGL(cc_big_list_kernel, dim3(cdiv(n, 256)), dim3(256), 0, ctx->stream, d_probs, np, parent, size, n, newlab,
                            big_root, big_qoff, big_box, counters);
@@ -807,7 +810,7 @@
         hipLaunchKernelGGL(cc_big_mark_kernel, dim3(cdiv(n, 256)), dim3(256), 0, ctx->stream, d_probs, np, parent, size, n, newlab, big_box);
         hipLaunchKernelGGL(cc_split_kernel, dim3(cdiv(n_big, 64)), dim3(64), 0, ctx->stream, d_probs, np, parent, size, big_root, big_qoff,
                            big_box, n_big, bqueue);
-        OBIA_HIP_TRY(hipMemsetAsync(counters, 0, sizeof(int) * 8, ctx->stream));
+        OBIA_TRY(fill_async(ctx, counters, 0, sizeof(int) * 8));
         rb = nullptr;
         hipLaunchKernelGGL(cc_rank_blocksum_kernel, dim3(nb), dim3(SCAN_NT), 0, ctx->stream, d_probs, np, parent, size, n, block_sums, counters, rb);
         hipLaunchKernelGGL(cc_rank_scan_kernel, dim3(3), dim3(1024), 0, ctx->stream, block_sums, nb, counters);
@@ -832,10 +835,6 @@
         int *settle = settle_arr = A.get<int>(n_small), *work_a = A.get<int>(n_small), *work_b = A.get<int>(n_small), *tag = A.get<int>(n_small);
         static const long long code_div = std::getenv("OBIA_CC_CODE_DIV") ? atoll(std::getenv("OBIA_CC_CODE_DIV")) : 64;
         const bool use_code = (long long)n_small * code_div >= n;
-        constexpr int RING = 64;
-        int *ring = A.get<int>(RING);
-        if (!ring) return OBIA_E_NOMEM;
-        OBIA_HIP_TRY(hipMemsetAsync(ring, 0, sizeof(int) * RING, ctx->stream));
         long long ring_pos = 0;
         int *code = use_code ? A.get<int>(n) : parent;
         if (!settle || !work_a || !work_b || !tag || !code) return OBIA_E_NOMEM;
@@ -848,7 +847,7 @@
                 if (hipMalloc(&ctx->cc_visited, want * sizeof(int32_t)) != hipSuccess) { (void)hipGetLastError(); set_error("out of device memory (visited map of %zu pixels)", want); return OBIA_E_NOMEM; }
                 ctx->cc_visited_px = want;
             }
-            OBIA_HIP_TRY(hipMemsetAsync(ctx->cc_visited, 0, sizeof(int32_t) * ctx->cc_visited_px, ctx->stream));
+            OBIA_TRY(fill_async(ctx, ctx->cc_visited, 0, sizeof(int32_t) * ctx->cc_visited_px));
         }
         ctx->cc_visited_dirty = true;
         visited = ctx->cc_visited;
@@ -862,10 +861,10 @@
             if (!px_g || !ccur || !px_cn) return OBIA_E_NOMEM;
             int maxh = 1;
             for (auto &P : probs) maxh = std::max(maxh, P.H);
-            OBIA_HIP_TRY(hipMemsetAsync(ccur, 0, sizeof(int) * (size_t)n_small, ctx->stream));
+            OBIA_TRY(fill_async(ctx, ccur, 0, sizeof(int) * (size_t)n_small));
             hipLaunchKernelGGL(cc_small_pixels_kernel, dim3(maxh, np), dim3(256), 0, ctx->stream, d_probs, code, small_qoff, ccur, px_g, px_cn, small_px);
             for (int side = (n_small > 8 * (long long)n_surv ? 1 : 0); side < 2 && !converged; ++side) {
-                OBIA_HIP_TRY(hipMemsetAsync(tag, 0, sizeof(int) * (size_t)n_small, ctx->stream));
+                OBIA_TRY(fill_async(ctx, tag, 0, sizeof(int) * (size_t)n_small));
                 hipLaunchKernelGGL(cc_settle_init_kernel, dim3(cdiv(n_small, 256)), dim3(256), 0, ctx->stream, small_list, n_small, settle, side);
                 int n_items = n_small;
                 const int *work_in = nullptr;
@@ -873,7 +872,7 @@
                 for (long long round = 0; round <= max_rounds; ++round) {
                     if (std::getenv("OBIA_DEBUG_CC")) fprintf(stderr, "[obia cc]   (lists) side %d round %lld: %d items\n", side, round, n_items);
                     int *cnt = ring + (ring_pos++ % RING);
-                    if (ring_pos > RING && (ring_pos - 1) % RING == 0) OBIA_HIP_TRY(hipMemsetAsync(ring, 0, sizeof(int) * RING, ctx->stream));
+                    if (ring_pos > RING && (ring_pos - 1) % RING == 0) OBIA_TRY(fill_async(ctx, ring, 0, sizeof(int) * RING));
                     hipLaunchKernelGGL(cc_settle_eval_kernel, dim3(cdiv(n_items, 64)), dim3(64), 0, ctx->stream, small_qoff, ccur, px_g, px_cn, small_px,
                                        settle, work_in, n_items, work_a, cnt, tag, (int)(round & 0x3fffffff));
                     int n_next = 0;
@@ -889,7 +888,7 @@
                                    small_qoff, settle, queue, visited, target, n_small);
         }
         for (int side = (n_small > 8 * (long long)n_surv ? 1 : 0); !dense && side < 2 && !converged; ++side) {
-            OBIA_HIP_TRY(hipMemsetAsync(tag, 0, sizeof(int) * (size_t)n_small, ctx->stream));
+            OBIA_TRY(fill_async(ctx, tag, 0, sizeof(int) * (size_t)n_small));
             hipLaunchKernelGGL(cc_settle_init_kernel, dim3(cdiv(n_small, 256)), dim3(256), 0, ctx->stream, small_list, n_small, settle, side);
             int n_items = n_small;
             const int *work_in = nullptr;
@@ -897,7 +896,7 @@
             for (long long round = 0; round <= max_rounds; ++round) {
                 if (std::getenv("OBIA_DEBUG_CC")) fprintf(stderr, "[obia cc]   side %d round %lld: %d items\n", side, round, n_items);
                 int *cnt = ring + (ring_pos++ % RING);
-                if (ring_pos > RING && (ring_pos - 1) % RING == 0) OBIA_HIP_TRY(hipMemsetAsync(ring, 0, sizeof(int) * RING, ctx->stream));
+                if (ring_pos > RING && (ring_pos - 1) % RING == 0) OBIA_TRY(fill_async(ctx, ring, 0, sizeof(int) * RING));
                 if (use_code)
                     hipLaunchKernelGGL(HIP_KERNEL_NAME(cc_small_bfs_kernel<true>), dim3(cdiv(n_items, 64)), dim3(64), 0, ctx->stream, d_probs, np, code,
                                        newlab, small_list, small_qoff, start_label, settle, queue, visited, target, work_in, n_items, work_a,
diff --git a/obia_amd/csrc/common.hpp b/obia_amd/csrc/common.hpp
--- a/obia_amd/csrc/common.hpp
+++ b/obia_amd/csrc/common.hpp
@@ -8,6 +8,8 @@
 #include <vector>
 
 #include "../../include/obia_hip.h"
+
+struct obia_ctx;
 
 namespace obia {
 
@@ -48,6 +50,17 @@
     bool failed_ = false;
 };
 
+class PlanBlob {
+  public:
+    template <typename T> T *add(obia_ctx *ctx, const T *host, size_t n) { return static_cast<T *>(add_bytes(ctx, host, n * sizeof(T))); }
+    int flush(obia_ctx *ctx);
+    void drop() { dev_ = host_ = nullptr; cap_ = used_ = 0; }
+  private:
+    void *add_bytes(obia_ctx *ctx, const void *host, size_t bytes);
+    char *dev_ = nullptr, *host_ = nullptr;
+    size_t cap_ = 0, used_ = 0;
+};
+
 struct Timing {
     double assign_ms = 0, prepass_ms = 0, feat_ms = 0, cc_ms = 0, zonal_ms = 0, total_ms = 0;
     double assign_px = 0, prepass_px = 0;
@@ -58,6 +71,7 @@
     int prepass_group_launches = 0;
     int batch_repeats = 0;
     double assign_busy_ms = 0, prepass_busy_ms = 0;
+    int fills = 0, uploads = 0, readbacks = 0;
 };
 
 }
@@ -77,6 +91,7 @@
     bool cc_visited_dirty = false;
     char *up_buf = nullptr;
     size_t up_bytes = 0, up_used = 0;
+    obia::PlanBlob plan;
     int profiling = 0;
     obia::Timing timing;
     struct Span { int kind; hipEvent_t a, b; };
@@ -107,6 +122,20 @@
 
 int read_back(obia_ctx *ctx, void *host_dst, const void *dev_src, size_t bytes);
 int upload_async(obia_ctx *ctx, void *dev_dst, const void *host_src, size_t bytes);
+int fill_async(obia_ctx *ctx, void *dev_dst, int byte, size_t bytes);
+
+struct ClearRange { void *p; unsigned long long bytes; unsigned value, pad; };
+struct ClearTable { ClearRange r[16]; int n; };
+class ClearSet {
+  public:
+    explicit ClearSet(obia_ctx *ctx) : ctx_(ctx) { t_.n = 0; }
+    int add(void *dev, int byte, size_t bytes);
+    int flush();
+  private:
+    obia_ctx *ctx_;
+    ClearTable t_;
+};
+
 int side_stream(obia_ctx *ctx);
 void debug_sync(obia_ctx *ctx, const char *stage);
 
diff --git a/obia_amd/csrc/context.cpp b/obia_amd/csrc/context.cpp
--- a/obia_amd/csrc/context.cpp
+++ b/obia_amd/csrc/context.cpp
@@ -1,4 +1,5 @@
 #include "common.hpp"
+#include "../../include/obia_testing.h"
 
 #include <algorithm>
 #include <cstdlib>
@@ -182,7 +183,9 @@
         OBIA_HIP_TRY(hipHostMalloc(&ctx->pinned, want, hipHostMallocDefault));
         ctx->pinned_bytes = want;
     }
+    OBIA_TRY(ctx->plan.flush(ctx));
     OBIA_HIP_TRY(hipMemcpyAsync(ctx->pinned, dev_src, bytes, hipMemcpyDeviceToHost, ctx->stream));
+    ctx->timing.readbacks += 1;
     OBIA_HIP_TRY(hipStreamSynchronize(ctx->stream));
     ctx->up_used = 0;
     memcpy(host_dst, ctx->pinned, bytes);
@@ -197,23 +200,127 @@
     fflush(stderr);
 }
 
+int fill_async(obia_ctx *ctx, void *dev_dst, int byte, size_t bytes) {
+    if (bytes == 0) return OBIA_OK;
+    OBIA_HIP_TRY(hipMemsetAsync(dev_dst, byte, bytes, ctx->stream));
+    ctx->timing.fills += 1;
+    return OBIA_OK;
+}
+
+template <bool RAGGED> __global__ __launch_bounds__(256) void clear_ranges_kernel(const ClearTable T) {
+    const size_t tid = (size_t)blockIdx.x * blockDim.x + threadIdx.x, stride = (size_t)gridDim.x * blockDim.x;
+    for (int k = 0; k < T.n; ++k) {
+        unsigned char *p = static_cast<unsigned char *>(T.r[k].p);
+        const size_t n = T.r[k].bytes;
+        const unsigned v = (T.r[k].value & 0xffu) * 0x01010101u;
+        size_t head = RAGGED ? (16 - (reinterpret_cast<uintptr_t>(p) & 15)) & 15 : 0;
+        if (head > n) head = n;
+        const size_t nvec = (n - head) / 16, tail0 = head + nvec * 16;
+        uint4 *pv = reinterpret_cast<uint4 *>(p + head);
+        for (size_t i = tid; i < nvec; i += stride) pv[i] = make_uint4(v, v, v, v);
+        if (RAGGED) {
+            if (tid < head) p[tid] = (unsigned char)v;
+            if (tid < n - tail0) p[tail0 + tid] = (unsigned char)v;
+        }
+    }
+}
+
+int ClearSet::add(void *dev, int byte, size_t bytes) {
+    if (bytes == 0) return OBIA_OK;
+    if (t_.n == 16) OBIA_TRY(flush());
+    t_.r[t_.n++] = ClearRange{dev, (unsigned long long)bytes, (unsigned)byte & 0xffu, 0u};
+    return OBIA_OK;
+}
+
+int ClearSet::flush() {
+    const int n = t_.n;
+    t_.n = 0;
+    if (n == 0) return OBIA_OK;
+    if (n == 1) return fill_async(ctx_, t_.r[0].p, (int)t_.r[0].value, (size_t)t_.r[0].bytes);
+    unsigned long long longest = 0;
+    bool ragged = false;
+    for (int k = 0; k < n; ++k) {
+        longest = std::max(longest, t_.r[k].bytes);
+        ragged = ragged || ((reinterpret_cast<uintptr_t>(t_.r[k].p) | (uintptr_t)t_.r[k].bytes) & 15) != 0;
+    }
+    ClearTable t = t_;
+    t.n = n;
+    const dim3 grid(flat_grid((long long)((longest + 15) / 16)));
+    if (ragged) hipLaunchKernelGGL(HIP_KERNEL_NAME(clear_ranges_kernel<true>), grid, dim3(256), 0, ctx_->stream, t);
+    else hipLaunchKernelGGL(HIP_KERNEL_NAME(clear_ranges_kernel<false>), grid, dim3(256), 0, ctx_->stream, t);
+    OBIA_HIP_TRY(hipGetLastError());
+    ctx_->timing.fills += 1;
+    return OBIA_OK;
+}
+
+constexpr size_t RING = 8u << 20;
+
+static int ring_ready(obia_ctx *ctx) {
+    if (ctx->up_buf) return OBIA_OK;
+    void *p = nullptr;
+    OBIA_HIP_TRY(hipHostMalloc(&p, RING, hipHostMallocDefault));
+    ctx->up_buf = static_cast<char *>(p);
+    ctx->up_bytes = RING;
+    ctx->up_used = 0;
+    return OBIA_OK;
+}
+
+void *PlanBlob::add_bytes(obia_ctx *ctx, const void *host, size_t bytes) {
+    constexpr size_t BLOCK = 64u << 10;
+    const size_t need = (bytes + 15) & ~size_t(15);
+    if (dev_ && used_ + need > cap_ && flush(ctx) != OBIA_OK) return nullptr;
+    if (ring_ready(ctx) != OBIA_OK) return nullptr;
+    if (need > ctx->up_bytes / 2) {
+        if (flush(ctx) != OBIA_OK) return nullptr;
+        void *d = ctx->arena.alloc(need);
+        return d && upload_async(ctx, d, host, bytes) == OBIA_OK ? d : nullptr;
+    }
+    if (!dev_) {
+        const size_t cap = (std::max(need, BLOCK) + 63) & ~size_t(63);
+        if (ctx->up_used + cap > ctx->up_bytes) {
+            if (hipStreamSynchronize(ctx->stream) != hipSuccess) { set_error("stream synchronisation failed (plan upload)"); return nullptr; }
+            ctx->up_used = 0;
+        }
+        char *d = static_cast<char *>(ctx->arena.alloc(cap));
+        if (!d) return nullptr;
+        dev_ = d;
+        host_ = ctx->up_buf + ctx->up_used;
+        ctx->up_used += cap;
+        cap_ = cap;
+        used_ = 0;
+    }
+    void *d = dev_ + used_;
+    if (bytes) memcpy(host_ + used_, host, bytes);
+    used_ += need;
+    return d;
+}
+
+int PlanBlob::flush(obia_ctx *ctx) {
+    if (!dev_) return OBIA_OK;
+    char *const dev = dev_, *const host = host_;
+    const size_t used = used_, cap = cap_;
+    dev_ = host_ = nullptr;
+    cap_ = used_ = 0;
+    if (ctx->up_buf && host + cap == ctx->up_buf + ctx->up_used) ctx->up_used -= cap - ((used + 63) & ~size_t(63));
+    if (used == 0) return OBIA_OK;
+    OBIA_HIP_TRY(hipMemcpyAsync(dev, host, used, hipMemcpyHostToDevice, ctx->stream));
+    ctx->timing.uploads += 1;
+    return OBIA_OK;
+}
+
 int upload_async(obia_ctx *ctx, void *dev_dst, const void *host_src, size_t bytes) {
     if (bytes == 0) return OBIA_OK;
-    constexpr size_t RING = 8u << 20;
-    if (!ctx->up_buf) {
-        void *p = nullptr;
-        OBIA_HIP_TRY(hipHostMalloc(&p, RING, hipHostMallocDefault));
-        ctx->up_buf = static_cast<char *>(p);
-        ctx->up_bytes = RING;
-        ctx->up_used = 0;
-    }
+    ctx->timing.uploads += 1;
+    OBIA_TRY(ring_ready(ctx));
     if (bytes > ctx->up_bytes) {
+        OBIA_TRY(ctx->plan.flush(ctx));
         OBIA_HIP_TRY(hipMemcpyAsync(dev_dst, host_src, bytes, hipMemcpyHostToDevice, ctx->stream));
         OBIA_HIP_TRY(hipStreamSynchronize(ctx->stream));
         ctx->up_used = 0;
         return OBIA_OK;
     }
     if (ctx->up_used + bytes > ctx->up_bytes) {
+        OBIA_TRY(ctx->plan.flush(ctx));
         OBIA_HIP_TRY(hipStreamSynchronize(ctx->stream));
         ctx->up_used = 0;
     }
@@ -237,12 +344,14 @@
 }
 
 void frame_begin(obia_ctx *ctx, unsigned opts) {
+    ctx->plan.drop();
     ctx->arena.reset();
     if (opts & FRAME_TIMING) begin_timing(ctx);
 }
 
 int frame_end(obia_ctx *ctx, unsigned opts, int rc) {
     if (rc != OBIA_OK) return quiesce(ctx, rc);
+    OBIA_TRY(ctx->plan.flush(ctx));
     OBIA_HIP_TRY(hipStreamSynchronize(ctx->stream));
     if (opts & FRAME_TIMING) resolve_timing(ctx);
     return OBIA_OK;
@@ -352,6 +461,18 @@
     if (!ctx) { set_error("null context"); return OBIA_E_INVALID; }
     OBIA_HIP_TRY(hipStreamSynchronize(ctx->stream));
     return OBIA_OK;
+}
+
+int obia_test_clear_ranges_dev(obia_ctx *ctx, void *const *dev_ptrs, const int64_t *bytes, const int32_t *values, int n) {
+    OBIA_TRY(enter(ctx));
+    if (!dev_ptrs || !bytes || !values || n < 0) { set_error("clear ranges: null array or negative count"); return OBIA_E_INVALID; }
+    for (int i = 0; i < n; ++i)
+        if (bytes[i] < 0 || (bytes[i] > 0 && !dev_ptrs[i])) { set_error("clear ranges: range %d is not a range", i); return OBIA_E_INVALID; }
+    return call_frame(ctx, FRAME_TIMING, [&] {
+        ClearSet clr(ctx);
+        for (int i = 0; i < n; ++i) OBIA_TRY(clr.add(dev_ptrs[i], values[i], (size_t)bytes[i]));
+        return clr.flush();
+    });
 }
 
 int64_t obia_workspace_bytes(obia_ctx *ctx) { return ctx ? (int64_t)ctx->arena.capacity() : 0; }
@@ -399,6 +520,9 @@
         case 13: return ctx->timing.prepass_shared_px;
         case 14: return ctx->timing.feat_fused_px;
         case 15: return (double)ctx->timing.prepass_group_launches;
+        case 16: return (double)ctx->timing.fills;
+        case 17: return (double)ctx->timing.uploads;
+        case 18: return (double)ctx->timing.readbacks;
         default: return -1.0;
     }
 }
diff --git a/obia_amd/csrc/slic.hip b/obia_amd/csrc/slic.hip
--- a/obia_amd/csrc/slic.hip
+++ b/obia_amd/csrc/slic.hip
@@ -718,17 +718,45 @@
     }
 }
 
-int slic_count_valid(obia_ctx *ctx, SlicBatch &b, std::vector<int> &nvalid) {
+int slic_plan_layout(obia_ctx *ctx, SlicBatch &b) {
+    if (b.d_tile_prob) return OBIA_OK;
+    const int np = b.nprob;
+    long long tiles_all = 0;
+    int tile_max = 0;
+    for (int p = 0; p < np; ++p) {
+        SlicProblem &P = b.probs[p];
+        P.tiles_x = cdiv(P.W, SWEEP_TW);
+        P.tiles_y = cdiv(P.H, SWEEP_TH);
+        const int nt = P.tiles_x * P.tiles_y;
+        if (tiles_all + nt > 0x7fff0000LL) { set_error("too many sweep tiles in one batch"); return OBIA_E_INVALID; }
+        P.tile_off = (int)tiles_all;
+        tiles_all += nt;
+        if (nt > tile_max) tile_max = nt;
+    }
+    b.total_tiles_all = tiles_all > 0 ? tiles_all : 1;
+    b.total_tiles = tile_max;
+    std::vector<int> tp((size_t)b.total_tiles_all, 0);
+    for (int p = 0; p < np; ++p)
+        for (int t = 0; t < b.probs[p].tiles_x * b.probs[p].tiles_y; ++t) tp[(size_t)b.probs[p].tile_off + t] = p;
+    b.d_probs = ctx->plan.add(ctx, b.probs.data(), (size_t)np);
+    b.d_tile_prob = ctx->plan.add(ctx, tp.data(), tp.size());
+    if (!b.d_probs || !b.d_tile_prob) return OBIA_E_NOMEM;
+    return OBIA_OK;
+}
+
+int slic_count_valid(obia_ctx *ctx, SlicBatch &b, std::vector<int> &nvalid, int *d_cnt_cleared) {
     const int np = b.nprob;
     Arena &A = ctx->arena;
     nvalid.assign(np, 0);
-    if (!b.d_probs) b.d_probs = A.get<SlicProblem>(np);
-    if (!b.d_probs) return OBIA_E_NOMEM;
+    OBIA_TRY(slic_plan_layout(ctx, b));
     if (b.masked) {
-        OBIA_TRY(upload_async(ctx, b.d_probs, b.probs.data(), sizeof(SlicProblem) * np));
-        int *d_cnt = A.get<int>(np);
-        if (!d_cnt) return OBIA_E_NOMEM;
-        OBIA_HIP_TRY(hipMemsetAsync(d_cnt, 0, sizeof(int) * np, ctx->stream));
+        OBIA_TRY(ctx->plan.flush(ctx));
+        int *d_cnt = d_cnt_cleared;
+        if (!d_cnt) {
+            d_cnt = A.get<int>(np);
+            if (!d_cnt) return OBIA_E_NOMEM;
+            OBIA_TRY(fill_async(ctx, d_cnt, 0, sizeof(int) * np));
+        }
         int blocks = cdiv(b.maxpix, 256 * 16 * 32);
         if (blocks < 1) blocks = 1;
         hipLaunchKernelGGL(count_valid_kernel, dim3(blocks, np), dim3(256), 0, ctx->stream, b.d_probs, b.d_mask, d_cnt);
@@ -746,8 +774,7 @@
         for (int p = 0; p < np; ++p)
             if (ext[p].n < 0 || (ext[p].n > 0 && !ext[p].yx && !ext[p].d_yx)) { set_error("external seeds of problem %d: bad set", p); return OBIA_E_INVALID; }
     Arena &A = ctx->arena;
-    if (!b.d_probs) b.d_probs = A.get<SlicProblem>(np);
-    if (!b.d_probs) return OBIA_E_NOMEM;
+    OBIA_TRY(slic_plan_layout(ctx, b));
     std::vector<int> nvalid;
     if (nvalid_in) nvalid = *nvalid_in;
     else OBIA_TRY(slic_count_valid(ctx, b, nvalid));
@@ -799,10 +826,9 @@
     b.total_cent = cent_off > 0 ? cent_off : 1;
     b.d_seed = A.get<float>((size_t)b.total_cent * 2);
     b.d_cent_prob = A.get<int>(b.total_cent);
-    SeedGrid *d_grids = A.get<SeedGrid>(np);
+    SeedGrid *d_grids = ctx->plan.add(ctx, grids.data(), (size_t)np);
     if (!b.d_seed || !b.d_cent_prob || !d_grids) return OBIA_E_NOMEM;
-    OBIA_HIP_TRY(hipMemsetAsync(b.d_cent_prob, 0xff, sizeof(int) * b.total_cent, ctx->stream));
-    OBIA_TRY(upload_async(ctx, d_grids, grids.data(), sizeof(SeedGrid) * np));
+    OBIA_TRY(fill_async(ctx, b.d_cent_prob, 0xff, sizeof(int) * b.total_cent));
     std::vector<int> K(np);
     if (ext) {
         std::vector<int> hp((size_t)b.total_cent, 0);
@@ -824,6 +850,7 @@
     } else if (b.masked) {
         int *d_K = A.get<int>(np);
         if (!d_K) return OBIA_E_NOMEM;
+        OBIA_TRY(ctx->plan.flush(ctx));
         hipLaunchKernelGGL(seed_masked_kernel, dim3(np), dim3(256), 0, ctx->stream, d_grids, b.d_probs, b.d_mask,
                            b.d_seed, b.d_cent_prob, d_K);
         OBIA_TRY(read_back(ctx, K.data(), d_K, sizeof(int) * np));
@@ -831,11 +858,11 @@
     } else {
         int maxK = 1;
         for (int p = 0; p < np; ++p) { K[p] = grids[p].ny * grids[p].nx; if (K[p] > maxK) maxK = K[p]; }
+        OBIA_TRY(ctx->plan.flush(ctx));
         hipLaunchKernelGGL(seed_grid_kernel, dim3(cdiv(maxK, 256), np), dim3(256), 0, ctx->stream, d_grids, np,
                            b.d_seed, b.d_cent_prob);
     }
-    int cell_off = 0, tile_max = 0;
-    long long tiles_all = 0;
+    int cell_off = 0;
     for (int p = 0; p < np; ++p) {
         SlicProblem &P = b.probs[p];
         P.K = K[p];
@@ -854,32 +881,16 @@
         long long nc = (long long)P.ncy * P.ncx;
         if (cell_off + nc > 0x7fff0000LL) { set_error("too many bins in one batch"); return OBIA_E_INVALID; }
         cell_off += (int)nc;
-        P.tiles_x = cdiv(P.W, SWEEP_TW);
-        P.tiles_y = cdiv(P.H, SWEEP_TH);
-        const int nt = P.tiles_x * P.tiles_y;
-        P.tile_off = (int)tiles_all;
-        tiles_all += nt;
-        if (nt > tile_max) tile_max = nt;
-    }
-    b.total_tiles_all = tiles_all > 0 ? tiles_all : 1;
-    {
-        std::vector<int> tp((size_t)b.total_tiles_all, 0);
-        for (int p = 0; p < np; ++p)
-            for (int t = 0; t < b.probs[p].tiles_x * b.probs[p].tiles_y; ++t) tp[(size_t)b.probs[p].tile_off + t] = p;
-        b.d_tile_prob = A.get<int>(tp.size());
-        if (!b.d_tile_prob) return OBIA_E_NOMEM;
-        OBIA_TRY(upload_async(ctx, b.d_tile_prob, tp.data(), sizeof(int) * tp.size()));
     }
     b.total_cells = cell_off > 0 ? cell_off : 1;
-    b.total_tiles = tile_max;
-    OBIA_TRY(upload_async(ctx, b.d_probs, b.probs.data(), sizeof(SlicProblem) * np));
+    b.d_probs = ctx->plan.add(ctx, b.probs.data(), (size_t)np);
+    if (!b.d_probs) return OBIA_E_NOMEM;
     const int RS = CENT_REC + b.CP;
     b.d_cent = A.get<float>((size_t)b.total_cent * RS);
     b.d_head = A.get<int>((size_t)b.total_cells * 2);
     const size_t acc_q = (size_t)b.total_cent * acc_record_qwords(b.CP);
     b.d_acc = A.get<unsigned long long>(acc_q);
     if (!b.d_cent || !b.d_head || !b.d_acc) return OBIA_E_NOMEM;
-    OBIA_HIP_TRY(hipMemsetAsync(b.d_acc, 0, sizeof(unsigned long long) * acc_q, ctx->stream));
     return OBIA_OK;
 }
 
diff --git a/obia_amd/csrc/slic.hpp b/obia_amd/csrc/slic.hpp
--- a/obia_amd/csrc/slic.hpp
+++ b/obia_amd/csrc/slic.hpp
@@ -157,7 +157,8 @@
 struct ExternalSeeds { const double *yx; int n; double step; const float *d_yx = nullptr; };
 int slic_plan_and_seed(obia_ctx *ctx, SlicBatch &b, const std::vector<int> &n_segments,
                        const std::vector<int> *nvalid = nullptr, const ExternalSeeds *ext = nullptr);
-int slic_count_valid(obia_ctx *ctx, SlicBatch &b, std::vector<int> &nvalid);
+int slic_count_valid(obia_ctx *ctx, SlicBatch &b, std::vector<int> &nvalid, int *d_cnt_cleared = nullptr);
+int slic_plan_layout(obia_ctx *ctx, SlicBatch &b);
 
 int slic_run_sweeps(obia_ctx *ctx, SlicBatch &b);
 int slic_sweeps_settle(obia_ctx *ctx, bool *repeat);
@@ -184,7 +185,7 @@
 #endif
 int enforce_connectivity_batch(obia_ctx *ctx, const std::vector<CcProblem> &probs, const int32_t *labels_in,
                                long long total_pix, int start_label, int32_t *labels_out, int *h_n_labels_out,
-                               CcResolve *deferred = nullptr);
+                               CcResolve *deferred = nullptr, const CcProblem *d_probs = nullptr);
 
 int enforce_connectivity_dev(obia_ctx *ctx, const int32_t *labels_in, int H, int W, int min_size,
                              int max_size, int start_label, int32_t *labels_out, int *d_n_labels_out);
diff --git a/obia_amd/csrc/slic_sweep.hip b/obia_amd/csrc/slic_sweep.hip
--- a/obia_amd/csrc/slic_sweep.hip
+++ b/obia_amd/csrc/slic_sweep.hip
@@ -1353,8 +1353,8 @@
         fp.cache_k = A.get<int>(nt * (MAXC + 1));
         fp.cache_q = A.get<unsigned long long>(nt * MAXC * (size_t)(b.CP + 3));
         if (!fp.bin_stamp || !fp.tile_lp || !fp.cache_k || !fp.cache_q) return OBIA_E_NOMEM;
-        OBIA_HIP_TRY(hipMemsetAsync(fp.bin_stamp, 0, sizeof(int) * (size_t)b.total_cells, ctx->stream));
-        OBIA_HIP_TRY(hipMemsetAsync(fp.tile_lp, 0, sizeof(int) * nt, ctx->stream));
+        OBIA_TRY(fill_async(ctx, fp.bin_stamp, 0, sizeof(int) * (size_t)b.total_cells));
+        OBIA_TRY(fill_async(ctx, fp.tile_lp, 0, sizeof(int) * nt));
     }
     {
         const size_t nt = (size_t)b.total_tiles_all;
@@ -1372,6 +1372,7 @@
         if (!b.d_mask4) return OBIA_E_NOMEM;
         int gq = (maxh_z + 3) / 4;
         if (gq > 16384) gq = 16384;
+        OBIA_TRY(ctx->plan.flush(ctx));
         hipLaunchKernelGGL(mask_pack4_kernel, dim3(gq, b.nprob), dim3(256), 0, ctx->stream, b.d_probs, b.d_mask, b.d_mask4);
     }
     if (maxh_z > 4096) maxh_z = 4096;
@@ -1381,7 +1382,6 @@
         fill_labels(ctx, b);
         debug_sync(ctx, "sweeps: label fill");
     }
-    if (repeat) OBIA_HIP_TRY(hipMemsetAsync(b.d_acc, 0, sizeof(unsigned long long) * (size_t)b.total_cent * RQ, ctx->stream));
     const bool prep_grouped = std::getenv("OBIA_PREP_GROUPED") != nullptr;
     const bool prepass_visits = std::getenv("OBIA_PREPASS_VISITS") != nullptr;
     std::vector<int> share_rep;
@@ -1415,18 +1415,14 @@
         n_act = (int)ap.size();
         act_p_base = ap.front();
         const bool span = ap.back() - ap.front() + 1 == n_act;
-        int *d_mr = A.get<int>(mr.size());
-        if (!d_mr) return OBIA_E_NOMEM;
-        OBIA_TRY(upload_async(ctx, d_mr, mr.data(), sizeof(int) * mr.size()));
-        d_member_rep = d_mr;
+        d_member_rep = ctx->plan.add(ctx, mr.data(), mr.size());
+        if (!d_member_rep) return OBIA_E_NOMEM;
         if (span) {
             act_tiles.base = b.probs[ap.front()].tile_off;
             act_tiles.end = b.probs[ap.back()].tile_off + b.probs[ap.back()].tiles_x * b.probs[ap.back()].tiles_y;
         } else {
-            int *d_ap = A.get<int>(ap.size()), *d_at = A.get<int>(at.size() ? at.size() : 1);
+            const int *d_ap = ctx->plan.add(ctx, ap.data(), ap.size()), *d_at = ctx->plan.add(ctx, at.data(), at.size());
             if (!d_ap || !d_at) return OBIA_E_NOMEM;
-            OBIA_TRY(upload_async(ctx, d_ap, ap.data(), sizeof(int) * ap.size()));
-            if (!at.empty()) OBIA_TRY(upload_async(ctx, d_at, at.data(), sizeof(int) * at.size()));
             d_act_probs = d_ap;
             act_tiles.table = d_at; act_tiles.base = 0; act_tiles.end = (int)at.size();
         }
@@ -1450,9 +1446,15 @@
             if (grp_split > 0) OBIA_TRY(side_stream(ctx));
         }
     }
-    OBIA_HIP_TRY(hipMemsetAsync(d_px, 0, sizeof(unsigned long long) * 513, ctx->stream));
-    OBIA_HIP_TRY(hipMemsetAsync(b.d_head, 0xff, sizeof(int) * (size_t)b.total_cells, ctx->stream));
-    OBIA_HIP_TRY(hipMemsetAsync(b.d_tl_meta, 0xff, sizeof(int) * 3 * (size_t)b.total_tiles_all, ctx->stream));
+    OBIA_TRY(ctx->plan.flush(ctx));
+    {
+        ClearSet clr(ctx);
+        OBIA_TRY(clr.add(b.d_acc, 0, sizeof(unsigned long long) * (size_t)b.total_cent * RQ));
+        OBIA_TRY(clr.add(d_px, 0, sizeof(unsigned long long) * 513));
+        OBIA_TRY(clr.add(b.d_head, 0xff, sizeof(int) * (size_t)b.total_cells));
+        OBIA_TRY(clr.add(b.d_tl_meta, 0xff, sizeof(int) * 3 * (size_t)b.total_tiles_all));
+        OBIA_TRY(clr.flush());
+    }
     debug_sync(ctx, "sweeps: memsets");
     bool first = true;
     int sweep_no = 0;
@@ -1461,7 +1463,7 @@
         const bool last_pass = (pass == passes - 1);
         if (pass > 0 && store_all) {
             fill_labels(ctx, b);
-            if (fp.tile_lp) OBIA_HIP_TRY(hipMemsetAsync(fp.tile_lp, 0, sizeof(int) * (size_t)b.total_tiles_all, ctx->stream));
+            if (fp.tile_lp) OBIA_TRY(fill_async(ctx, fp.tile_lp, 0, sizeof(int) * (size_t)b.total_tiles_all));
         }
         const int iters = ignore_color ? pre_iter : b.max_iter;
         for (int it = 0; it < iters; ++it) {
@@ -1590,38 +1592,39 @@
     return OBIA_OK;
 }
 
+static int defer_counters(obia_ctx *ctx, const unsigned long long *d_px) {
+    if (!ctx->defer_buf) OBIA_HIP_TRY(hipHostMalloc(reinterpret_cast<void **>(&ctx->defer_buf), sizeof(unsigned long long) * 513, hipHostMallocDefault));
+    OBIA_HIP_TRY(hipMemcpyAsync(ctx->defer_buf, d_px, sizeof(unsigned long long) * 513, hipMemcpyDeviceToHost, ctx->stream));
+    ctx->timing.readbacks += 1;
+    ctx->defer_pending = true;
+    return OBIA_OK;
+}
+
 int slic_run_sweeps(obia_ctx *ctx, SlicBatch &b) {
     ctx->defer_pending = false;
     unsigned long long *d_px = nullptr;
     ctx->defer_shared_px = 0.0;
     OBIA_TRY(queue_sweeps(ctx, b, false, &d_px, &ctx->defer_shared_px));
-    if (!d_px) return OBIA_OK;
-    if (!ctx->defer_buf) OBIA_HIP_TRY(hipHostMalloc(reinterpret_cast<void **>(&ctx->defer_buf), sizeof(unsigned long long) * 513, hipHostMallocDefault));
-    OBIA_HIP_TRY(hipMemcpyAsync(ctx->defer_buf, d_px, sizeof(unsigned long long) * 513, hipMemcpyDeviceToHost, ctx->stream));
-    ctx->defer_pending = true;
-    return OBIA_OK;
+    return d_px ? defer_counters(ctx, d_px) : OBIA_OK;
 }
 
 int slic_sweeps_settle(obia_ctx *ctx, bool *repeat) {
-    *repeat = false;
+    if (repeat) *repeat = false;
     if (!ctx->defer_pending) return OBIA_OK;
     ctx->defer_pending = false;
     const unsigned long long *h = ctx->defer_buf;
-    if ((h[512] & 0xffffffffull) != 0ull) { *repeat = true; return OBIA_OK; }
+    if (repeat && (h[512] & 0xffffffffull) != 0ull) { *repeat = true; return OBIA_OK; }
     fold_counters(ctx, h, ctx->defer_shared_px);
     return OBIA_OK;
 }
 
 int slic_rerun_storing(obia_ctx *ctx, SlicBatch &b) {
     ctx->timing.batch_repeats += 1;
+    ctx->defer_pending = false;
     unsigned long long *d_px = nullptr;
-    double shared_px = 0.0;
-    OBIA_TRY(queue_sweeps(ctx, b, true, &d_px, &shared_px));
-    if (!d_px) return OBIA_OK;
-    unsigned long long h[513];
-    OBIA_TRY(read_back(ctx, h, d_px, sizeof(h)));
-    fold_counters(ctx, h, shared_px);
-    return OBIA_OK;
-}
-
-}
+    ctx->defer_shared_px = 0.0;
+    OBIA_TRY(queue_sweeps(ctx, b, true, &d_px, &ctx->defer_shared_px));
+    return d_px ? defer_counters(ctx, d_px) : OBIA_OK;
+}
+
+}
diff --git a/obia_amd/csrc/tiling.hip b/obia_amd/csrc/tiling.hip
--- a/obia_amd/csrc/tiling.hip
+++ b/obia_amd/csrc/tiling.hip
@@ -323,7 +323,7 @@
     float *d_seeds = A.get<float>(2 * (size_t)total);
     double *d_steps = A.get<double>(2 * (size_t)np);
     if (!d_seeds || !d_steps) return OBIA_E_NOMEM;
-    OBIA_HIP_TRY(hipMemsetAsync(d_steps, 0, sizeof(double) * 2 * (size_t)np, ctx->stream));
+    OBIA_TRY(fill_async(ctx, d_steps, 0, sizeof(double) * 2 * (size_t)np));
     auto ascending_below = [](const int64_t *v, long long n, long long bound) {
         if (v[0] < 0 || v[n - 1] >= bound) return false;
         for (long long i = 1; i < n; ++i) if (v[i] <= v[i - 1]) return false;
@@ -371,8 +371,6 @@
     for (auto &t : wins) b.windows.push_back(SrcWindow{t.y0, t.x0, t.h, t.w, 0, 0, 0});
     OBIA_TRY(slic_batch_layout(b));
     for (int p = 0; p < np; ++p) { wins[p].pix_off = b.probs[p].pix_off; wins[p].m4_off = b.probs[p].m4_off; }
-    TileWin *d_wins = A.get<TileWin>(np);
-    b.d_windows = A.get<SrcWindow>(np);
     b.d_mask = A.get<uint8_t>((size_t)b.total_pix);
     unsigned *d_mask4 = A.get<unsigned>((size_t)b.total_m4);
     if (!d_mask4) return OBIA_E_NOMEM;
@@ -400,14 +398,24 @@
         }
     }
     b.d_labels = A.get<int32_t>((size_t)b.total_pix);
-    if (!d_wins || !b.d_windows || !b.d_mask || !b.d_feat || !b.d_labels) return OBIA_E_NOMEM;
-    OBIA_TRY(upload_async(ctx, d_wins, wins.data(), sizeof(TileWin) * np));
-    OBIA_TRY(upload_async(ctx, b.d_windows, b.windows.data(), sizeof(SrcWindow) * np));
-    int *d_tile_any = A.get<int>(np);
-    if (!d_tile_any) return OBIA_E_NOMEM;
+    if (!b.d_mask || !b.d_feat || !b.d_labels) return OBIA_E_NOMEM;
+    TileWin *d_wins = ctx->plan.add(ctx, wins.data(), (size_t)np);
+    b.d_windows = ctx->plan.add(ctx, b.windows.data(), (size_t)np);
+    if (!d_wins || !b.d_windows) return OBIA_E_NOMEM;
+    OBIA_TRY(slic_plan_layout(ctx, b));
+    OBIA_TRY(ctx->plan.flush(ctx));
+    int *d_tile_any = A.get<int>(np), *d_cnt = A.get<int>(np);
+    if (!d_tile_any || !d_cnt) return OBIA_E_NOMEM;
+    {
+        ClearSet clr(ctx);
+        if (white) {
+            OBIA_TRY(clr.add(S.inside, 0, sizeof(unsigned) * (size_t)S.next_id));
+            OBIA_TRY(clr.add(d_tile_any, 0, sizeof(int) * (size_t)np));
+        }
+        OBIA_TRY(clr.add(d_cnt, 0, sizeof(int) * (size_t)np));
+        OBIA_TRY(clr.flush());
+    }
     if (white) {
-        OBIA_HIP_TRY(hipMemsetAsync(S.inside, 0, sizeof(unsigned) * (size_t)S.next_id, ctx->stream));
-        OBIA_HIP_TRY(hipMemsetAsync(d_tile_any, 0, sizeof(int) * (size_t)np, ctx->stream));
         hipLaunchKernelGGL(tile_count_inside_kernel, dim3(grid_rows(wins), np), dim3(256), 0, ctx->stream, d_wins, S.G, S.W, S.inside, d_tile_any);
     }
     {
@@ -434,7 +442,7 @@
     }
     std::vector<int> nvalid;
     debug_sync(ctx, "tiler: mask + features");
-    OBIA_TRY(slic_count_valid(ctx, b, nvalid));
+    OBIA_TRY(slic_count_valid(ctx, b, nvalid, d_cnt));
     debug_sync(ctx, "tiler: count_valid");
     std::vector<int> nseg(np);
     const double pixel_area = S.tp.pixel_width * S.tp.pixel_height;
@@ -451,6 +459,14 @@
     if (S.seeding == OBIA_SEEDING_SKIMAGE) OBIA_TRY(seed_tiles_skimage(ctx, S, b, nvalid, nseg, ext));
     OBIA_TRY(slic_plan_and_seed(ctx, b, nseg, &nvalid, ext.empty() ? nullptr : ext.data()));
     debug_sync(ctx, "tiler: plan_and_seed");
+    std::vector<CcProblem> cps(np);
+    for (int p = 0; p < np; ++p) {
+        const SlicProblem &P = b.probs[p];
+        const auto [min_size, max_size] = slic_cc_sizes(S.sp.min_size_factor, S.sp.max_size_factor, P.n_valid, P.K);
+        cps[p] = CcProblem{P.H, P.W, P.pix_off, min_size, max_size};
+    }
+    const CcProblem *d_cps = S.sp.enforce_connectivity ? ctx->plan.add(ctx, cps.data(), (size_t)np) : nullptr;
+    if (S.sp.enforce_connectivity && !d_cps) return OBIA_E_NOMEM;
     if (!white && S.pf.planned && !S.pf.launched)
         OBIA_TRY(prefetch_white_launch(ctx, S, OBIA_PREFETCH_BESIDE != 0 || b.exit_on_fixed_point || b.slic_zero));
     const Arena::Mark sweeps_mk = A.mark();
@@ -460,20 +476,15 @@
     int n_new = 0;
     CcResolve resolve{};
     if (S.sp.enforce_connectivity) {
-        std::vector<CcProblem> cps(np);
-        for (int p = 0; p < np; ++p) {
-            const SlicProblem &P = b.probs[p];
-            const auto [min_size, max_size] = slic_cc_sizes(S.sp.min_size_factor, S.sp.max_size_factor, P.n_valid, P.K);
-            cps[p] = CcProblem{P.H, P.W, P.pix_off, min_size, max_size};
-        }
-        OBIA_TRY(enforce_connectivity_batch(ctx, cps, b.d_labels, b.total_pix, 1, nullptr, &n_new, &resolve));
+        OBIA_TRY(enforce_connectivity_batch(ctx, cps, b.d_labels, b.total_pix, 1, nullptr, &n_new, &resolve, d_cps));
         bool repeat = false;
         OBIA_TRY(slic_sweeps_settle(ctx, &repeat));
         if (repeat) {
             A.rewind(sweeps_mk);
             b.d_mask4 = mask4;
             OBIA_TRY(slic_rerun_storing(ctx, b));
-            OBIA_TRY(enforce_connectivity_batch(ctx, cps, b.d_labels, b.total_pix, 1, nullptr, &n_new, &resolve));
+            OBIA_TRY(enforce_connectivity_batch(ctx, cps, b.d_labels, b.total_pix, 1, nullptr, &n_new, &resolve, d_cps));
+            OBIA_TRY(slic_sweeps_settle(ctx, nullptr));
         }
         debug_sync(ctx, "tiler: connectivity");
     } else {
@@ -486,10 +497,11 @@
         for (auto &t : wins) sblocks = std::max(sblocks, cdiv(t.w, 64) * cdiv(t.h, 64));
         hipLaunchKernelGGL(tile_scatter_kernel, dim3(sblocks, np), dim3(64), 0, ctx->stream, d_wins, resolve, S.G, S.W,
                            S.next_id - 1, S.seg_size);
-        OBIA_HIP_TRY(hipMemsetAsync(S.alive + S.next_id, 1, (size_t)n_new, ctx->stream));
+        OBIA_TRY(fill_async(ctx, S.alive + S.next_id, 1, (size_t)n_new));
         S.next_id += n_new;
     }
     OBIA_HIP_TRY(hipGetLastError());
+    OBIA_TRY(ctx->plan.flush(ctx));
     A.rewind(mk);
     return OBIA_OK;
 }
@@ -610,8 +622,8 @@
     S.newid = A.get<int>((size_t)cap);
     S.d_total = A.get<long long>(1);
     if (!S.seg_size || !S.inside || !S.alive || !S.newid || !S.d_total) return OBIA_E_NOMEM;
-    OBIA_HIP_TRY(hipMemsetAsync(S.seg_size, 0, sizeof(unsigned) * (size_t)cap, ctx->stream));
-    OBIA_HIP_TRY(hipMemsetAsync(S.alive, 0, (size_t)cap, ctx->stream));
+    OBIA_TRY(fill_async(ctx, S.seg_size, 0, sizeof(unsigned) * (size_t)cap));
+    OBIA_TRY(fill_async(ctx, S.alive, 0, (size_t)cap));
     S.clx = S.cly = S.clx_in = S.cly_in = S.clx_any = S.cly_any = 0;
     if (B > 0) {
         const double cl = (double)B / 2.0;
@@ -773,7 +785,7 @@
     OBIA_TRY(check_seeding(seeding, picks));
     OBIA_TRY(tiler_init(ctx, S, img, mask, H, W, C, H, 0, tp, sp, labels_out, 0));
     S.seeding = seeding; S.pick_fn = picks; S.pick_user = picks_user;
-    OBIA_HIP_TRY(hipMemsetAsync(labels_out, 0, sizeof(int32_t) * (size_t)H * W, ctx->stream));
+    OBIA_TRY(fill_async(ctx, labels_out, 0, sizeof(int32_t) * (size_t)H * W));
     const int nty = cdiv(H, tp->tile_size);
     OBIA_TRY(prefetch_white_plan(ctx, S, tp->white_order));
     OBIA_TRY(tiler_run(ctx, S, false, 0, nty, -1));
@@ -853,7 +865,7 @@
     if (first_id + count > t->S.id_cap) { set_error("segment id capacity exceeded (%d + %d > %d)", first_id, count, t->S.id_cap); return OBIA_E_NOMEM; }
     if (count == 0) return OBIA_OK;
     OBIA_HIP_TRY(hipMemcpyAsync(t->S.seg_size + first_id, sizes_dev, sizeof(uint32_t) * (size_t)count, hipMemcpyDeviceToDevice, t->ctx->stream));
-    OBIA_HIP_TRY(hipMemsetAsync(t->S.alive + first_id, 1, (size_t)count, t->ctx->stream));
+    OBIA_TRY(fill_async(t->ctx, t->S.alive + first_id, 1, (size_t)count));
     if (first_id + count > t->S.next_id) t->S.next_id = first_id + count;
     OBIA_HIP_TRY(hipStreamSynchronize(t->ctx->stream));
     return OBIA_OK;
@@ -891,7 +903,7 @@
         t->seam_cap = (size_t)n + 2;
     }
     int *ctr = t->seam_buf, *new_list = t->seam_buf + 2;
-    OBIA_HIP_TRY(hipMemsetAsync(ctr, 0, sizeof(int) * 2, ctx->stream));
+    OBIA_TRY(fill_async(ctx, ctr, 0, sizeof(int) * 2));
     const int blocks = std::min(cdiv(n, 256), 2048);
     hipLaunchKernelGGL(seam_mark_kernel, dim3(blocks), dim3(256), 0, ctx->stream, codes_dev, n, my_rank, owner_rank, fmap_dev, fmap_cap, new_list, ctr,
                        ids_out_dev);
diff --git a/obia_amd/csrc/zonal.hip b/obia_amd/csrc/zonal.hip
--- a/obia_amd/csrc/zonal.hip
+++ b/obia_amd/csrc/zonal.hip
@@ -469,10 +469,14 @@
     unsigned *g_n = A.get<unsigned>(nlb);
     double *g_s2 = A.get<double>(nlb), *g_s3 = A.get<double>(nlb), *g_s4 = A.get<double>(nlb);
     if (!g_n || !g_s2 || !g_s3 || !g_s4) return OBIA_E_NOMEM;
-    OBIA_HIP_TRY(hipMemsetAsync(g_n, 0, sizeof(unsigned) * nlb, ctx->stream));
-    OBIA_HIP_TRY(hipMemsetAsync(g_s2, 0, sizeof(double) * nlb, ctx->stream));
-    OBIA_HIP_TRY(hipMemsetAsync(g_s3, 0, sizeof(double) * nlb, ctx->stream));
-    OBIA_HIP_TRY(hipMemsetAsync(g_s4, 0, sizeof(double) * nlb, ctx->stream));
+    {
+        ClearSet clr(ctx);
+        OBIA_TRY(clr.add(g_n, 0, sizeof(unsigned) * nlb));
+        OBIA_TRY(clr.add(g_s2, 0, sizeof(double) * nlb));
+        OBIA_TRY(clr.add(g_s3, 0, sizeof(double) * nlb));
+        OBIA_TRY(clr.add(g_s4, 0, sizeof(double) * nlb));
+        OBIA_TRY(clr.flush());
+    }
     if ((long long)W * C * 4 >= (1ll << 32)) { set_error("a raster row of %lld bytes is not supported (4 GB at most)", (long long)W * C * 4); return OBIA_E_UNSUPPORTED; }
     const int tiles = cdiv(W, ZTW) * cdiv(H, ZTH);
     const bool ident = bl.identity && bl.n == C;
```

After: 7546, median of 6. 1.01x the previous value.
